# jeuneS2/csolve

Hardware: AMD Instinct MI355X
Metric: constraint propagations/sec + nodes/sec, queens-N, 1/2/4/8 MI355X (higher is better)
Workload: dtype int32

## Files before the change

csolve_amd/_lib.py:

```python
from __future__ import annotations

import ctypes as C
import os
import re

_HERE = os.path.dirname(os.path.abspath(__file__))
LIB_PATH = os.environ.get("CSOLVE_HIP_LIB") or os.path.join(_HERE, "libcsolve_hip.so")
HEADER_PATH = os.path.join(os.path.dirname(_HERE), "include", "csolve_gpu.h")


class CsolveError(RuntimeError):
    def __init__(self, code: int, message: str):
        super().__init__(f"csolve_gpu error {code}: {message}")
        self.code = code


class Val(C.Structure):
    _fields_ = [("lo", C.c_int32), ("hi", C.c_int32)]


class Node(C.Structure):
    _fields_ = [("var", C.c_int32), ("lo", C.c_int32), ("hi", C.c_int32), ("parent", C.c_int32)]


class SearchStats(C.Structure):
    _fields_ = [("nodes", C.c_uint64), ("cuts", C.c_uint64), ("props", C.c_uint64), ("revisions", C.c_uint64),
                ("solutions", C.c_uint64), ("iterations", C.c_uint64), ("restarts", C.c_uint64), ("pool", C.c_int64), ("pool_peak", C.c_int64),
                ("best", C.c_int32), ("done", C.c_int32)]


SHARD_SOLUTION_FN = C.CFUNCTYPE(None, C.c_void_p, C.c_int, C.POINTER(C.c_int32), C.c_int64, C.c_int32)


class ShardOptions(C.Structure):
    _fields_ = [("slice_iterations", C.c_int64), ("poll_iterations", C.c_int64), ("seed_states_per_rank", C.c_int64),
                ("low_water", C.c_int64), ("time_limit", C.c_double), ("on_solution", SHARD_SOLUTION_FN),
                ("user", C.c_void_p)]


class Result(C.Structure):
    _fields_ = [("status", C.c_int32), ("props", C.c_int32), ("revisions", C.c_int32), ("rounds", C.c_int32)]


MANY_DONE, MANY_LIMIT, MANY_BAD_ROOT = 0, 1, 2
MANY_BAD_SLOT = 3


class ManyResult(C.Structure):
    _fields_ = [("status", C.c_int32), ("root_props", C.c_int32), ("nodes", C.c_int64), ("cuts", C.c_int64),
                ("props", C.c_int64), ("solutions", C.c_int64)]


class ManyOptions(C.Structure):
    _fields_ = [("objective", C.c_int32), ("reserved", C.c_int32), ("max_nodes", C.c_int64)]


class ManyUptoOptions(C.Structure):
    _fields_ = [("max_solutions", C.c_int32), ("reserved", C.c_int32), ("max_nodes", C.c_int64)]


MANY_ROTATE_FIRST = 1


class ManyRestartOptions(C.Structure):
    _fields_ = [("max_nodes", C.c_int64), ("restart_base", C.c_int64), ("seed", C.c_uint32), ("flags", C.c_int32)]


MANY_FULL = 4
MANY_SLOT_FRESH = -2


class ManyStream(C.Structure):
    _fields_ = [("d_rows", C.c_void_p), ("d_owner", C.c_void_p), ("d_count", C.c_void_p), ("capacity", C.c_int64)]


def declared_symbols(header: str = HEADER_PATH):
    text = re.sub(r"/\*.*?\*/", "", open(header).read(), flags=re.S)
    return sorted(set(re.findall(r"\b(csgpu_\w+)\s*\(", text)))


PLAN_FAMILIES = ("events", "traced", "rounds", "lds", "bitset", "regs0", "regs1", "regs2", "regs3", "packed",
                 "shave", "shave_trace", "server", "step_shave", "step_packed", "step_import")

_lib = None
_demangler = None


def demangle(symbol: str) -> str:
    global _demangler
    if _demangler is None:
        cxx = C.CDLL("libstdc++.so.6")
        cxx.__cxa_demangle.argtypes = [C.c_char_p, C.c_void_p, C.c_void_p, C.POINTER(C.c_int)]
        cxx.__cxa_demangle.restype = C.c_void_p
        libc = C.CDLL(None)
        libc.free.argtypes = [C.c_void_p]
        _demangler = (cxx.__cxa_demangle, libc.free)
    fn, free = _demangler
    status = C.c_int()
    p = fn(symbol.encode(), None, None, C.byref(status))
    if status.value != 0 or not p:
        raise ValueError(f"cannot demangle {symbol!r}")
    try:
        text = C.string_at(p).decode()
    finally:
        free(p)
    if text.startswith("void "):
        text = text[5:]
    depth = 0
    for i, ch in enumerate(text):
        depth += ch == "<"
        depth -= ch == ">"
        if ch == "(" and depth == 0:
            return text[:i]
    return text


def load_library():
    global _lib
    if _lib is not None:
        return _lib
    if not os.path.exists(LIB_PATH):
        raise ImportError(
            f"{LIB_PATH} is missing: build it with `python -c 'import __graft_entry__ as g; g.build()'` "
            "or `make -C csolve_amd/csrc` (hipcc --offload-arch=gfx950). There is no CPU fallback.")
    try:
        import torch
    except ImportError:
        pass
    L = C.CDLL(LIB_PATH)
    vp, i32, i64 = C.c_void_p, C.c_int32, C.c_int64
    L.csgpu_last_error.restype = C.c_char_p
    L.csgpu_device_count.restype = C.c_int
    L.csgpu_set_device.argtypes = [C.c_int]
    L.csgpu_model_from_text.argtypes = [C.c_char_p, C.c_int, C.POINTER(vp)]
    L.csgpu_model_from_file.argtypes = [C.c_char_p, C.c_int, C.POINTER(vp)]
    L.csgpu_model_from_dump.argtypes = [C.c_char_p, C.POINTER(vp)]
    L.csgpu_model_free.argtypes = [vp]
    L.csgpu_model_free.restype = None
    for f in ("csgpu_model_num_vars", "csgpu_model_num_clauses", "csgpu_model_objective",
              "csgpu_model_objective_var"):
        getattr(L, f).argtypes = [vp]
    L.csgpu_model_var_name.argtypes = [vp, C.c_int]
    L.csgpu_model_var_name.restype = C.c_char_p
    L.csgpu_model_get_domains.argtypes = [vp, vp]
    L.csgpu_model_set_domains.argtypes = [vp, vp]
    L.csgpu_model_device_info.argtypes = [vp, C.POINTER(i64)]
    L.csgpu_model_root_propagate.argtypes = [vp, C.POINTER(i32)]
    L.csgpu_model_finalize.argtypes = [vp]
    L.csgpu_model_normalize.argtypes = [vp]
    L.csgpu_model_specialize.argtypes = [vp, vp, C.POINTER(vp)]
    L.csgpu_model_build_tables.argtypes = [vp]
    L.csgpu_model_eval_clauses_host.argtypes = [vp, vp]
    L.csgpu_model_set_kernel.argtypes = [vp, C.c_int]
    L.csgpu_model_qualifies.argtypes = [vp, C.c_int]
    L.csgpu_set_linear_fast_paths.argtypes = [C.c_int]
    L.csgpu_sets_pack.argtypes = [vp, vp, vp, i64, vp]
    L.csgpu_sets_unpack.argtypes = [vp, vp, vp, i64, vp]
    L.csgpu_propagate_batch_sets.argtypes = [vp, vp, vp, vp, vp, i64, vp]
    L.csgpu_set_linear_fast_paths.restype = None
    L.csgpu_model_get_kernel.argtypes = [vp]
    L.csgpu_propagate_batch.argtypes = [vp, vp, vp, vp, vp, i64, vp]
    L.csgpu_propagate_batch_obj.argtypes = [vp, vp, vp, vp, vp, i64, i32, i32, vp]
    L.csgpu_internal_propagate_objdev.argtypes = [vp, vp, vp, vp, vp, i64, vp, i32, i32, vp, C.c_int, vp]
    L.csgpu_model_forbidden_words.argtypes = [vp]
    L.csgpu_propagate_batch_fb.argtypes = [vp, vp, vp, vp, vp, vp, vp, i64, vp]
    L.csgpu_eval_batch.argtypes = [vp, vp, vp, i64, vp]
    L.csgpu_eval_clauses.argtypes = [vp, vp, vp, vp]
    L.csgpu_search_create.argtypes = [vp, i64, i64, C.POINTER(vp)]
    L.csgpu_search_free.argtypes = [vp]
    L.csgpu_search_free.restype = None
    L.csgpu_search_reset.argtypes = [vp]
    L.csgpu_search_put.argtypes = [vp, vp, i64]
    L.csgpu_search_put_host.argtypes = [vp, vp, i64]
    L.csgpu_search_take.argtypes = [vp, vp, i64, C.POINTER(i64)]
    L.csgpu_search_take_host.argtypes = [vp, vp, i64, C.POINTER(i64)]
    L.csgpu_plan_transfers.argtypes = [vp, C.c_int, i64, i64, vp, C.POINTER(C.c_int)]
    L.csgpu_shard_region_size.argtypes = [C.c_int, C.c_int, i64, C.POINTER(C.c_size_t)]
    L.csgpu_shard_region_init.argtypes = [vp, C.c_size_t, C.c_int, C.c_int, i64]
    L.csgpu_shard_barrier.argtypes = [vp]
    L.csgpu_text_num_vars.argtypes = [C.c_char_p, C.c_int, C.POINTER(C.c_int)]
    L.csgpu_shard_default_options.argtypes = [C.POINTER(ShardOptions)]
    L.csgpu_shard_default_options.restype = None
    L.csgpu_shard_run.argtypes = [vp, vp, C.c_int, vp, C.POINTER(ShardOptions), C.POINTER(SearchStats),
                                  C.POINTER(SearchStats)]
    L.csgpu_search_set_best.argtypes = [vp, i32]
    L.csgpu_model_add_conflict.argtypes = [vp, i32, vp, vp]
    L.csgpu_search_put_cost.argtypes = [vp, C.POINTER(C.c_double), C.POINTER(i64)]
    L.csgpu_objective_better.argtypes = [C.c_int, Val, i32]
    L.csgpu_objective_bound.argtypes = [C.c_int, Val, i32]
    L.csgpu_objective_bound.restype = Val
    L.csgpu_objective_best.argtypes = [C.c_int, Val, i32]
    L.csgpu_objective_best.restype = i32
    L.csgpu_luby_next.argtypes = [C.POINTER(C.c_uint64), C.POINTER(C.c_uint64)]
    L.csgpu_luby_next.restype = None
    L.csgpu_step_check.argtypes = [Val, C.c_uint32]
    L.csgpu_step_val.argtypes = [Val, C.c_uint32, C.c_uint32]
    L.csgpu_step_val.restype = i32
    L.csgpu_search_share_incumbent.argtypes = [vp, vp]
    L.csgpu_search_set_parents.argtypes = [vp, i64]
    L.csgpu_search_set_restart.argtypes = [vp, i64]
    L.csgpu_search_run.argtypes = [vp, i64, C.POINTER(SearchStats)]
    L.csgpu_search_solutions.argtypes = [vp, vp, i64]
    L.csgpu_search_best_solution.argtypes = [vp, vp]
    L.csgpu_search_solutions.restype = i64
    L.csgpu_search_set_solution_stream.argtypes = [vp, i64]
    L.csgpu_search_drain_solutions.argtypes = [vp, vp, i64, C.POINTER(i64)]
    L.csgpu_search_drain_solutions_device.argtypes = [vp, vp, i64, C.POINTER(i64), vp]
    L.csgpu_search_pending_solutions.argtypes = [vp, C.POINTER(i64), C.POINTER(i64)]
    L.csgpu_propagate_one.argtypes = [vp, vp, Node, vp, C.POINTER(Result)]
    L.csgpu_propagate_one_traced.argtypes = [vp, vp, Node, vp, C.POINTER(Result), vp, i32, C.POINTER(i32)]
    L.csgpu_propagate_one_causes.argtypes = [vp, vp, Node, vp, C.POINTER(Result), vp, i32, C.POINTER(i32)]
    L.csgpu_propagate_values.argtypes = [vp, vp, i32, vp, i32, vp, vp]
    L.csgpu_model_root_propagate_limit.argtypes = [vp, i64, C.POINTER(i32), C.POINTER(i32)]
    L.csgpu_propagate_one_chain.argtypes = [vp, vp, Node, C.POINTER(i32), C.POINTER(i32), vp, i32, C.POINTER(i32)]
    L.csgpu_search_set_strategy.argtypes = [vp, C.c_int, C.c_int]
    L.csgpu_search_set_restart_on_improvement.argtypes = [vp, C.c_int]
    L.csgpu_internal_plan_symbol.argtypes = [vp, C.c_int, C.c_char_p, C.c_size_t]
    L.csgpu_solve_many.argtypes = [vp, vp, i64, C.POINTER(ManyOptions), vp, vp, vp]
    L.csgpu_internal_many_symbol.argtypes = [vp, C.c_char_p, C.c_size_t]
    L.csgpu_internal_many_waves.argtypes = [vp, i64]
    L.csgpu_internal_many_waves.restype = i64
    L.csgpu_internal_many_resume_symbol.argtypes = [vp, C.c_char_p, C.c_size_t]
    L.csgpu_many_checkpoint_bytes.argtypes = [vp]
    L.csgpu_many_checkpoint_bytes.restype = C.c_size_t
    L.csgpu_many_checkpoints_create.argtypes = [vp, i64, C.POINTER(vp)]
    L.csgpu_many_checkpoints_reset.argtypes = [vp, vp]
    L.csgpu_many_checkpoints_free.argtypes = [vp]
    L.csgpu_many_checkpoints_free.restype = None
    L.csgpu_solve_many_checkpointed.argtypes = [vp, vp, i64, C.POINTER(ManyOptions), vp, vp, vp, vp, vp]
    L.csgpu_solve_many_resume.argtypes = [vp, i64, C.POINTER(ManyOptions), vp, vp, vp, vp, vp]
    L.csgpu_many_checkpoint_states.argtypes = [vp, C.c_int32, vp, i64, C.POINTER(i64), vp]
    L.csgpu_many_checkpoint_children.argtypes = [vp, vp, i64, vp, vp]
    L.csgpu_many_checkpoint_fanout.argtypes = [vp, vp, i64, vp, vp, vp, i64, vp]
    L.csgpu_many_fold.argtypes = [vp, vp, i64, vp, vp]
    L.csgpu_solve_many_upto.argtypes = [vp, vp, i64, C.POINTER(ManyUptoOptions), vp, vp, vp]
    L.csgpu_solve_many_upto_checkpointed.argtypes = [vp, vp, i64, C.POINTER(ManyUptoOptions), vp, vp, vp, vp, vp]
    L.csgpu_solve_many_upto_resume.argtypes = [vp, i64, C.POINTER(ManyUptoOptions), vp, vp, vp, vp, vp]
    L.csgpu_internal_many_upto_symbol.argtypes = [vp, C.c_char_p, C.c_size_t]
    L.csgpu_model_qualifies_many_allowed.argtypes = [vp]
    L.csgpu_solve_many_allowed.argtypes = [vp, vp, i64, C.POINTER(ManyOptions), vp, vp, vp]
    L.csgpu_solve_many_allowed_upto.argtypes = [vp, vp, i64, C.POINTER(ManyUptoOptions), vp, vp, vp]
    L.csgpu_internal_many_allowed_symbol.argtypes = [vp, C.c_char_p, C.c_size_t]
    L.csgpu_internal_many_allowed_upto_symbol.argtypes = [vp, C.c_char_p, C.c_size_t]
    L.csgpu_solve_many_restarts.argtypes = [vp, vp, vp, i64, C.POINTER(ManyRestartOptions), vp, vp, vp, vp]
    L.csgpu_internal_many_restart_symbol.argtypes = [vp, C.c_char_p, C.c_size_t]
    L.csgpu_solve_many_stream.argtypes = [vp, vp, i64, C.POINTER(ManyOptions), vp, vp, vp, C.POINTER(ManyStream), vp]
    L.csgpu_internal_many_stream_symbol.argtypes = [vp, C.c_char_p, C.c_size_t]
    L.csgpu_solve_many_clauses.argtypes = [vp, vp, i64, C.POINTER(ManyOptions), vp, vp, vp, vp]
    L.csgpu_model_qualifies_many_clauses.argtypes = [vp]
    L.csgpu_internal_many_clauses_symbol.argtypes = [vp, C.c_char_p, C.c_size_t]
    L.csgpu_internal_many_clauses_waves.argtypes = [vp, i64]
    L.csgpu_internal_many_clauses_waves.restype = i64
    L.csgpu_internal_many_clauses_resume_symbol.argtypes = [vp, C.c_char_p, C.c_size_t]
    L.csgpu_many_clause_checkpoint_bytes.argtypes = [vp]
    L.csgpu_many_clause_checkpoint_bytes.restype = C.c_size_t
    L.csgpu_many_clause_checkpoints_create.argtypes = [vp, i64, C.POINTER(vp)]
    L.csgpu_solve_many_clauses_checkpointed.argtypes = [vp, vp, i64, C.POINTER(ManyOptions), vp, vp, vp, vp, vp, vp]
    L.csgpu_solve_many_clauses_resume.argtypes = [vp, i64, C.POINTER(ManyOptions), vp, vp, vp, vp, vp, vp]
    L.csgpu_many_clause_checkpoint_states.argtypes = [vp, C.c_int32, vp, i64, C.POINTER(i64), C.POINTER(C.c_int32),
                                                      C.POINTER(C.c_int32), vp]
    L.csgpu_many_clause_checkpoint_children.argtypes = [vp, vp, i64, vp, vp]
    L.csgpu_many_clause_checkpoint_fanout.argtypes = [vp, vp, i64, vp, vp, vp, i64, vp]
    L.csgpu_solve_many_clauses_upto.argtypes = [vp, vp, i64, C.POINTER(ManyUptoOptions), vp, vp, vp]
    L.csgpu_solve_many_clauses_upto_checkpointed.argtypes = [vp, vp, i64, C.POINTER(ManyUptoOptions), vp, vp, vp, vp, vp]
    L.csgpu_solve_many_clauses_upto_resume.argtypes = [vp, i64, C.POINTER(ManyUptoOptions), vp, vp, vp, vp, vp]
    L.csgpu_internal_many_clauses_upto_symbol.argtypes = [vp, C.c_char_p, C.c_size_t]
    L.csgpu_solve_many_clauses_restarts.argtypes = [vp, vp, vp, i64, C.POINTER(ManyRestartOptions), vp, vp, vp, vp]
    L.csgpu_internal_many_clauses_restart_symbol.argtypes = [vp, C.c_char_p, C.c_size_t]
    L.csgpu_solve_many_clauses_stream.argtypes = [vp, vp, i64, C.POINTER(ManyOptions), vp, vp, vp, C.POINTER(ManyStream), vp]
    L.csgpu_internal_many_clauses_stream_symbol.argtypes = [vp, C.c_char_p, C.c_size_t]
    L.csgpu_solve_many_clauses_from.argtypes = [vp, vp, vp, i64, C.POINTER(ManyOptions), vp, vp, vp, vp, vp, vp]
    L.csgpu_solve_many_clauses_from_resume.argtypes = [vp, i64, C.POINTER(ManyOptions), vp, vp, vp, vp, vp, vp]
    L.csgpu_many_clause_checkpoint_children_obj.argtypes = [vp, vp, i64, C.c_int, vp, vp]
    L.csgpu_many_clause_checkpoint_fanout_obj.argtypes = [vp, vp, i64, C.c_int, vp, vp, vp, vp, vp, i64, vp]
    L.csgpu_many_fold_best.argtypes = [vp, vp, vp, i64, C.c_int, vp, vp]
    L.csgpu_many_best_key.argtypes = [C.c_int, C.c_int32, C.c_uint32]
    L.csgpu_many_best_key.restype = C.c_uint64
    L.csgpu_many_key_decode.argtypes = [C.c_int, C.c_uint64, C.POINTER(C.c_int32), C.POINTER(C.c_uint32)]
    L.csgpu_internal_many_clauses_from_symbol.argtypes = [vp, C.c_char_p, C.c_size_t]
    L.csgpu_many_value.argtypes = [C.c_uint32, C.c_uint32, C.c_int32, Val, C.c_uint32, C.c_int32]
    L.csgpu_many_value.restype = C.c_int32
    L.csgpu_debug_one_timing.argtypes = [vp, C.POINTER(C.c_double), C.POINTER(C.c_uint64), C.POINTER(C.c_uint64)]
    _lib = L
    return L


def check(rc: int):
    if rc < 0:
        raise CsolveError(rc, load_library().csgpu_last_error().decode())
    return rc
```

csolve_amd/csrc/cs_capi.hip:

```cpp
#include <hip/hip_runtime.h>
#include <chrono>

#include <dlfcn.h>
#include <stdarg.h>
#include <stdio.h>
#include <stdlib.h>
#include <string.h>

#include <mutex>

#include "../../include/csolve_gpu.h"
#include "cs_kernels.hip.h"
#include "cs_shave.hip.h"
#include "cs_step.hip.h"
#include "cs_dive.hip.h"
#include "cs_walk.hip.h"
#include "cs_chain.hip.h"
#include "cs_internal.h"

static thread_local char g_err[512] = "";

static int set_err(int code, const char *fmt, ...) {
  va_list ap;
  va_start(ap, fmt);
// ... 980 lines not shown
  const char *force = getenv("CSGPU_K2_ADJ");
  const int want_global = force != NULL && force[0] == 'g';
  if (want_global && 8 * lds_slice <= CS_CU_LDS) {
    m->lds_adj_global = 1;
    waves = 8;
    bytes = 8 * lds_slice;
  }
  { const char *e = getenv("CSGPU_K2_CSZ"); m->k2_csz = e != NULL && atoi(e) >= 1 && atoi(e) <= CS_CHUNK ? atoi(e) : 0; }
  if (!waves) return CSGPU_OK;
  int rc;
  if ((rc = upload(m->img->adj_packed, (size_t)m->img->n_adj * (size_t)m->img->packed_width, (int **)&m->d_adj_packed)))
    return rc;
  if ((rc = plan_kernel(&m->plan.lds, ne_lds_kernel(m->img->packed_width, h->n_vars, m->lds_adj_global), bytes, waves)))
    return rc;
  if (m->plan.lds.per_cu < 1) m->plan.lds.per_cu = 1;
  return CSGPU_OK;
}

static int64_t widest_root_domain(const csgpu_model *m) {
  const cs_model *h = m->host;
  int64_t width = 1;
  for (int32_t v = 0; v < h->n_vars; v++) {
    const int64_t w = (int64_t)h->dom[v].hi - (int64_t)h->dom[v].lo + 1;
    if (w > width) width = w;
  }
  return width;
}

static int forbidden_sets_shape(const csgpu_model *m, int *fw_out, size_t *lds_out) {
  const cs_model *h = m->host;
  if (m->img->sym_width == 0 || m->not_root) return 0;
  const int64_t width = widest_root_domain(m);
  const int fw = width <= 64 ? 1 : (width <= 128 ? 2 : (width <= 256 ? 4 : 0));
  if (!fw) return 0;
  const size_t n_words = ((size_t)h->n_vars + 31) / 32;
  const size_t off_bytes = (((size_t)h->n_vars * 2 * sizeof(int)) + 15) & ~(size_t)15;
  const size_t base_bytes = (((size_t)h->n_vars * sizeof(int)) + 15) & ~(size_t)15;
  const size_t adj_bytes = (((size_t)m->img->sym_n_adj * (size_t)m->img->sym_width) + 15) & ~(size_t)15;
  const size_t sl = ((size_t)h->n_vars * sizeof(cs_val) + (size_t)h->n_vars * fw * 8 + (2 * n_words + 2) * sizeof(unsigned) + 15) &
                    ~(size_t)15;
  int waves = 16;
  for (; waves >= 1; waves--)
    if (off_bytes + base_bytes + adj_bytes + (size_t)waves * sl <= CS_CU_LDS) break;
  if (waves < 1) return 0;
  *fw_out = fw;
  *lds_out = off_bytes + base_bytes + adj_bytes + (size_t)waves * sl;
  return waves;
}

static int plan_forbidden_sets(csgpu_model *m) {
  const cs_model *h = m->host;
  int fw = 0;
  size_t lds = 0;
  const int waves = forbidden_sets_shape(m, &fw, &lds);
  if (!waves) return CSGPU_OK;
  m->fb_words = fw;
  int *lo = (int *)malloc((size_t)(h->n_vars ? h->n_vars : 1) * sizeof(int));
  for (int32_t v = 0; v < h->n_vars; v++) lo[v] = h->dom[v].lo;
  int rc = upload(lo, (size_t)h->n_vars * sizeof(int), &m->d_root_lo);
  free(lo);
  if (rc) return rc;
  if ((rc = upload(m->img->sym_off, ((size_t)h->n_vars + 1) * sizeof(int), &m->d_sym_off))) return rc;
  if ((rc = upload(m->img->sym_packed, (size_t)m->img->sym_n_adj * (size_t)m->img->sym_width, (int **)&m->d_sym_packed)))
    return rc;
  if ((rc = plan_kernel(&m->plan.bitset, ne_bitset_kernel(m->img->sym_width, fw, h->n_vars), lds, waves))) return rc;
  if (m->plan.bitset.per_cu < 1) m->plan.bitset.per_cu = 1;
  return CSGPU_OK;
}

static int dense_table_waves(const csgpu_model *m, size_t *bytes_out) {
  if (m->img->dense_width == 0) return 0;
  const size_t bytes = (size_t)m->host->n_vars * m->img->dense_slots * m->img->dense_cols * m->img->dense_width;
  int best = 0, waves = 0;
  for (int w = 4; w <= 16; w <<= 1)
    if (resident_per_cu(bytes, w) * w > best) { best = resident_per_cu(bytes, w) * w; waves = w; }
  *bytes_out = bytes;
  return waves;
}

static int plan_dense_table(csgpu_model *m) {
  const cs_model *h = m->host;
  if (!m->fb_words) return CSGPU_OK;
  const int n = h->n_vars, width = m->img->dense_width, slots = m->img->dense_slots;
  size_t bytes = 0;
  const int waves = dense_table_waves(m, &bytes);
  if (!waves) return CSGPU_OK;
  m->dense_bytes = bytes;
  int rc;
  if ((rc = upload(m->img->dense_tab, bytes, (int **)&m->d_dense_tab))) return rc;
  for (int variant = 0; variant < 4; variant++)
    if ((rc = plan_kernel(&m->plan.regs[variant], ne_regs_kernel(width, m->fb_words, n, variant & 1, variant >> 1), bytes, waves)))
      return rc;
  m->plan.full = n == cs_dense_strides(n) * CS_WAVE;
  if ((rc = plan_kernel(&m->plan.shave, ne_shave_kernel(width, n, slots, m->plan.full), bytes, waves))) return rc;
  const size_t table = (bytes + 15) & ~(size_t)15;
  if (table + (size_t)waves * 32 <= CS_CU_LDS &&
      (rc = plan_kernel(&m->plan.step_shave, step_shave_kernel(width, n, slots, m->plan.full), table + (size_t)waves * 32, waves)))
    return rc;
  if (table + CS_SHAVE_TRACE_LDS * 16 <= CS_CU_LDS) {
    if ((rc = plan_kernel(&m->plan.shave_trace, ne_shave_trace_kernel(width, n, slots), table + CS_SHAVE_TRACE_LDS * 16, waves)))
      return rc;
    m->plan.server = m->plan.shave_trace;
    m->plan.server.fn = shave_server_kernel(width, n, slots);
  }
  const int64_t widest = widest_root_domain(m);
  for (int family = 0; family < MANY_FAMILIES; family++) {
    const int by_allowed = family == MANY_ALLOWED || family == MANY_ALLOWED_UPTO;
    if (by_allowed && widest > CS_DIVE_ALLOWED_WIDTH) continue;
    if ((rc = plan_kernel(&m->plan.dive[family], dive_kernel(family, width, n, widest <= 32 ? 1 : 4), table, waves))) return rc;
  }
  {
    int *hi = (int *)malloc((size_t)n * sizeof(int));
    if (hi == NULL) return set_err(CSGPU_E_ARG, "out of memory");
    for (int32_t v = 0; v < n; v++) hi[v] = h->dom[v].hi;
    rc = upload(hi, (size_t)n * sizeof(int), &m->d_root_hi);
    free(hi);
    if (rc) return rc;
  }
  HIP_TRY(hipMalloc((void **)&m->d_tickets, (size_t)CS_TICKET_SLOTS * CS_TICKET_SLOT_WORDS * sizeof(unsigned)));
  HIP_TRY(hipMemset(m->d_tickets, 0, (size_t)CS_TICKET_SLOTS * CS_TICKET_SLOT_WORDS * sizeof(unsigned)));
  m->ticket_slots = CS_TICKET_SLOTS;
  m->shave_static = getenv("CSGPU_SHAVE_STATIC") != NULL;
  return CSGPU_OK;
}

static int plan_packed(csgpu_model *m) {
  const cs_model *h = m->host;
  if (m->plan.shave.fn == NULL) return CSGPU_OK;
  const int n = h->n_vars, s3 = m->img->dense_slots == 3;
  m->packed_nw = 1;
  for (int32_t v = 0; v < n; v++)
    if ((int64_t)h->dom[v].hi - (int64_t)h->dom[v].lo + 1 > 32) m->packed_nw = 2;
  m->packed_bias = 0;
  for (int32_t v = 0; v < n; v++)
    if (h->dom[v].lo - m->img->dense_dmin > m->packed_bias) m->packed_bias = h->dom[v].lo - m->img->dense_dmin;
  m->plan.packed_nodes = packed_nodes_per_wave(m->fb_words, n, m->img->dense_width);
  if (!m->plan.packed_nodes) return CSGPU_OK;
  const size_t bytes = m->dense_bytes;
  int rc;
  if ((rc = plan_kernel(&m->plan.packed, ne_packed_kernel(n, m->packed_nw, s3), 2 * bytes, m->plan.regs[0].waves))) return rc;
  m->plan.packed.per_cu = m->plan.regs[0].per_cu;
  const size_t per_row = (size_t)m->img->dense_slots * m->img->dense_cols, total = (size_t)n * per_row;
  uint16_t *rel = (uint16_t *)malloc(total * sizeof(uint16_t));
  const uint8_t *src = (const uint8_t *)m->img->dense_tab;
  for (size_t i = 0; i < total; i++) {
    const int32_t u = (int32_t)(i / per_row);
    rel[i] = src[i] == 0xffu ? (uint16_t)0xffffu : (uint16_t)((int)src[i] - (h->dom[u].lo - m->img->dense_dmin) + m->packed_bias);
  }
  rc = upload(rel, total * sizeof(uint16_t), (int **)&m->d_packed_tab);
  free(rel);
  if (rc) return rc;
  if (step_packed_lds(m, 16) <= 80u * 1024u &&
      ((rc = plan_kernel(&m->plan.step_packed, step_packed_kernel(n, m->packed_nw, s3), step_packed_lds(m, 16), 16)) ||
       (rc = plan_kernel(&m->plan.step_import, step_import_kernel(n, m->packed_nw, s3), (2 * bytes + 15) & ~(size_t)15, 4))))
    return rc;
  m->step_chunk_max = 128;
  { const char *e = getenv("CSGPU_STEP_CHUNK_MAX"); if (e != NULL && atoi(e) > 0) m->step_chunk_max = atoi(e); }
  return CSGPU_OK;
}

static int stage_single_node(csgpu_model *m) {
  int dev = 0;
  hipDeviceProp_t prop;
  HIP_TRY(hipGetDevice(&dev));
  HIP_TRY(hipGetDeviceProperties(&prop, dev));
  m->n_cus = prop.multiProcessorCount;
  const size_t nbytes = (size_t)(m->host->n_vars ? m->host->n_vars : 1) * sizeof(cs_val);
  const size_t part = (nbytes + 63) & ~(size_t)63;
  unsigned char *d = NULL;
  HIP_TRY(hipHostMalloc((void **)&m->h_one, 2 * part + 128, hipHostMallocMapped));
  HIP_TRY(hipHostGetDevicePointer((void **)&d, m->h_one, 0));
  m->d_one_in = (cs_val *)d;
  m->d_one_node = (cs_node_in *)(d + part);
  m->d_one_res = (cs_node_out *)(d + part + 64);
  m->d_one_out = (cs_val *)(d + part + 128);
  return CSGPU_OK;
}

extern "C" int csgpu_model_finalize(csgpu_model *m) {
  if (m == NULL) return set_err(CSGPU_E_ARG, "null argument");
  free_device(m);
  int rc;
  if ((rc = csgpu_model_build_tables(m)) || (rc = drop_entailed_clauses(m)) || (rc = plan_general(m)) ||
      (rc = plan_lds_resident(m)) || (rc = plan_forbidden_sets(m)) || (rc = plan_dense_table(m)) || (rc = plan_packed(m)) ||
      (rc = stage_single_node(m)))
    return rc;
  m->plan.step_kind = m->plan.step_packed.fn != NULL ? 1
                      : (m->plan.step_shave.fn != NULL && m->host->n_vars <= 256 && m->plan.max_width <= 256 ? 2 : 0);
  m->finalized = 1;
  return CSGPU_OK;
}

static int kernel_qualifies(const csgpu_model *m, int which) {
  if (!m->finalized) return 0;
  switch (which) {
  case 1: return 1;
  case 2: return m->plan.lds.fn != NULL;
  case 3: return m->plan.bitset.fn != NULL;
  case 4: return m->plan.regs[0].fn != NULL;
  case 5: return m->plan.packed.fn != NULL;
  case 6: return m->plan.rounds.fn != NULL;
  case 7: return m->plan.shave.fn != NULL;
  default: return 0;
  }
}

extern "C" int csgpu_model_set_kernel(csgpu_model *m, int which) {
  static const char *const kernel_name[8] = {
    NULL, NULL, "the LDS-resident kernel", "the forbidden-set kernel", "the register-resident forbidden-set kernel",
    "the several-nodes-per-wave kernel (at most 32 variables, 64 values)", "the clause-resident kernel (at most 512 clauses)",
    "the interval-only shaving kernel (dense pair table in LDS)" };
  if (m == NULL || which < 0 || which > 7) return set_err(CSGPU_E_ARG, "bad argument");
  if (which >= 2) {
    if (!m->finalized) return set_err(CSGPU_E_STATE, "model is not finalized");
    if (!kernel_qualifies(m, which)) return set_err(CSGPU_E_LIMIT, "model does not qualify for %s", kernel_name[which]);
  }
  m->kernel_choice = which;
  return CSGPU_OK;
}

extern "C" int csgpu_model_qualifies(const csgpu_model *m, int which) { return m != NULL && kernel_qualifies(m, which); }

extern "C" int csgpu_internal_plan_symbol(const csgpu_model *m, int family, char *buf, size_t len) {
  if (m == NULL || buf == NULL || len == 0) return set_err(CSGPU_E_ARG, "null argument");
  if (!m->finalized) return set_err(CSGPU_E_STATE, "model is not finalized");
  const cs_kernel_plan *p = &m->plan;
  const cs_planned *fam[] = { &p->events, &p->traced, &p->rounds, &p->lds, &p->bitset, &p->regs[0], &p->regs[1],
                              &p->regs[2], &p->regs[3], &p->packed, &p->shave, &p->shave_trace, &p->server,
                              &p->step_shave, &p->step_packed, &p->step_import };
  if (family < 0 || family >= (int)(sizeof fam / sizeof fam[0])) return set_err(CSGPU_E_ARG, "no plan family %d", family);
  buf[0] = '\0';
  const void *fn = fam[family]->fn;
  if (fn == NULL) return CSGPU_OK;
  Dl_info info;
  if (dladdr(fn, &info) == 0 || info.dli_sname == NULL || info.dli_saddr != fn)
    return set_err(CSGPU_E_STATE, "plan family %d: the kernel handle has no dynamic symbol", family);
  if (strlen(info.dli_sname) >= len) return set_err(CSGPU_E_LIMIT, "plan family %d: symbol longer than the buffer", family);
  strcpy(buf, info.dli_sname);
  return CSGPU_OK;
}

static int many_symbol(const csgpu_model *m, int family, char *buf, size_t len) {
  if (m == NULL || buf == NULL || len == 0) return set_err(CSGPU_E_ARG, "null argument");
  if (!m->finalized) return set_err(CSGPU_E_STATE, "model is not finalized");
  buf[0] = '\0';
  const void *fn = m->plan.dive[family].fn;
  const char *name = many_kernel_name[family];
  if (fn == NULL) return CSGPU_OK;
  Dl_info info;
  if (dladdr(fn, &info) == 0 || info.dli_sname == NULL || info.dli_saddr != fn)
    return set_err(CSGPU_E_STATE, "%s: the kernel handle has no dynamic symbol", name);
  if (strlen(info.dli_sname) >= len) return set_err(CSGPU_E_LIMIT, "%s: symbol longer than the buffer", name);
  strcpy(buf, info.dli_sname);
  return CSGPU_OK;
}

extern "C" int csgpu_internal_many_symbol(const csgpu_model *m, char *buf, size_t len) { return many_symbol(m, MANY_PLAIN, buf, len); }
extern "C" int csgpu_internal_many_resume_symbol(const csgpu_model *m, char *buf, size_t len) { return many_symbol(m, MANY_CK, buf, len); }
extern "C" int csgpu_internal_many_upto_symbol(const csgpu_model *m, char *buf, size_t len) { return many_symbol(m, MANY_UPTO, buf, len); }
extern "C" int csgpu_internal_many_restart_symbol(const csgpu_model *m, char *buf, size_t len) { return many_symbol(m, MANY_RESTART, buf, len); }
extern "C" int csgpu_internal_many_stream_symbol(const csgpu_model *m, char *buf, size_t len) { return many_symbol(m, MANY_STREAM, buf, len); }
extern "C" int csgpu_internal_many_allowed_symbol(const csgpu_model *m, char *buf, size_t len) { return many_symbol(m, MANY_ALLOWED, buf, len); }
extern "C" int csgpu_internal_many_allowed_upto_symbol(const csgpu_model *m, char *buf, size_t len) { return many_symbol(m, MANY_ALLOWED_UPTO, buf, len); }

extern "C" void csgpu_internal_engine_ref(const csgpu_model *m, int delta) {
  if (m != NULL) const_cast<csgpu_model *>(m)->engines += delta;
}

extern "C" const int32_t *csgpu_internal_root_lo(const csgpu_model *m) {
  return m != NULL && m->finalized && m->fb_words ? m->d_root_lo : NULL;
}

extern "C" int csgpu_model_forbidden_words(const csgpu_model *m) { return m && m->finalized ? m->fb_words : 0; }

extern "C" int csgpu_internal_step_kind(const csgpu_model *m) { return m == NULL || !m->finalized ? 0 : m->plan.step_kind; }

static int64_t step_shave_waves(const csgpu_model *m, int64_t stage_rows) {
  const cs_planned *k = &m->plan.step_shave;
  int64_t waves = (int64_t)m->n_cus * (int64_t)k->per_cu * k->waves;
  const int64_t by_stage = stage_rows / (4 * (int64_t)m->plan.max_width);
  if (waves > by_stage) waves = by_stage / k->waves * k->waves;
  return waves;
}

extern "C" int64_t csgpu_internal_step_parents_limit(const csgpu_model *m, int64_t stage_rows) {
  const int kind = csgpu_internal_step_kind(m);
  if (kind == 1) return 0x3fffffff;
  if (kind != 2) return 0;
  const int maxw = m->plan.max_width;
  const int64_t waves = step_shave_waves(m, stage_rows);
  if (waves < 1) return 0;
  return (stage_rows - waves * 2 * maxw) / maxw;
}

extern "C" int64_t csgpu_internal_step_stage_rows(const csgpu_model *m) {
  if (csgpu_internal_step_kind(m) != 2) return 0;
  return (int64_t)m->n_cus * 32 * 4 * m->plan.max_width;
}

extern "C" int64_t csgpu_internal_step_waves(const csgpu_model *m) { return m == NULL ? 0 : (int64_t)m->n_cus * 32; }

static int launch_step_shave(const csgpu_model *m, const csgpu_step_launch *L, void *stream) {
  const cs_planned *k = &m->plan.step_shave;
  const int n = m->host->n_vars, maxw = m->plan.max_width;
  int64_t waves = step_shave_waves(m, L->stage_rows);
  if (waves < k->waves || (int64_t)L->parents > csgpu_internal_step_parents_limit(m, L->stage_rows))
    return set_err(CSGPU_E_LIMIT, "step kernel: staging buffer too small for the frontier");
  const int64_t by_parents = ((int64_t)L->parents + k->waves - 1) / k->waves * k->waves;
  if (waves > by_parents) waves = by_parents;
  const int64_t grid = waves / k->waves;
  const int64_t K = L->stage_rows / waves;
  cs_step_io io;
  io.pool = (const uint2 *)L->pool;
  io.first_row = (long long)L->first_row;
  io.parents = L->parents;
  io.chunk = 1;
  io.maxw = maxw;
  io.stage = (uint2 *)L->stage;
  io.K = (int)(K > 0x7fffffff ? 0x7fffffff : K);
  io.fill = L->fill;
  io.wstat = (unsigned long long *)L->wstat;
  io.ticket = L->ticket;
  io.solutions = L->solutions;
  io.stored = (unsigned long long *)L->stored;
  io.max_solutions = (long long)L->max_solutions;
  io.store_open = L->store_open;
  io.stream_on = L->stream != NULL;
  int nn = n, slots = m->img->dense_slots, dmin_d = m->img->dense_dmin;
  const void *tab_d = m->d_dense_tab;
  const int *root_lo_d = m->d_root_lo, *sym_off = m->d_sym_off;
  size_t tab_bytes = m->dense_bytes;
  void *args[] = { &nn, &tab_d, &slots, &dmin_d, &root_lo_d, &sym_off, &tab_bytes, &io };
  HIP_TRY(hipLaunchKernel(k->fn, dim3((unsigned)grid), dim3((unsigned)(k->waves * CS_WAVE)), args, k->lds, (hipStream_t)stream));
  hipLaunchKernelGGL(cs_collect, dim3((unsigned)waves), dim3(256), 0, (hipStream_t)stream, (const unsigned *)L->fill, (int)waves,
                     (const uint2 *)L->stage, io.K, n, (uint2 *)L->pool, (long long)L->first_row, (int)L->parents,
                     0 , (const unsigned *)L->ticket, (const unsigned long long *)L->wstat,
                     (unsigned long long *)L->out, (const unsigned long long *)L->stored,
                     L->stream, (long long)L->stream_base, (long long)L->stream_limit, (long long)L->stream_cap,
                     (unsigned long long *)L->stream_err);
  HIP_TRY(hipGetLastError());
  return CSGPU_OK;
}

extern "C" int csgpu_internal_step(const csgpu_model *m, const csgpu_step_launch *L, void *stream) {
  const int kind = csgpu_internal_step_kind(m);
  if (kind == 0 || L == NULL || L->parents < 1) return set_err(CSGPU_E_ARG, "bad argument");
  if (kind == 2) return launch_step_shave(m, L, stream);
  const int n = m->host->n_vars;
  const int G = m->plan.packed_nodes, maxw = m->plan.max_width;
  if (G * maxw > CS_STEP_QN) return set_err(CSGPU_E_LIMIT, "step kernel: interval too wide for the child queue");
  int64_t waves = (int64_t)m->n_cus * 32;
  const int64_t by_stage = L->stage_rows / (2 * (int64_t)G * maxw);
  if (waves > by_stage) waves = by_stage;
  const int64_t by_parents = ((int64_t)L->parents + G - 1) / G;
  if (waves > by_parents) waves = by_parents;
  if (waves < 1) return set_err(CSGPU_E_LIMIT, "step kernel: staging buffer too small");
  int wg_waves = 16;
  while (wg_waves > waves) wg_waves >>= 1;
  const int64_t grid = waves / wg_waves;
  waves = grid * wg_waves;
  const int64_t K = L->stage_rows / waves;
  int64_t chunk = (int64_t)L->parents / (waves * 8);
  if (chunk > m->step_chunk_max) chunk = m->step_chunk_max;
  if (chunk * maxw > K / 2) chunk = K / (2 * maxw);
  chunk = chunk / G * G;
  if (chunk < G) chunk = G;
  cs_step_io io;
  io.pool = (const uint2 *)L->pool;
  io.first_row = (long long)L->first_row;
  io.parents = L->parents;
  io.chunk = (int)chunk;
  io.maxw = maxw;
  io.stage = (uint2 *)L->stage;
  io.K = (int)(K > 0x7fffffff ? 0x7fffffff : K);
  io.fill = L->fill;
  io.wstat = (unsigned long long *)L->wstat;
  io.ticket = L->ticket;
  io.solutions = L->solutions;
  io.stored = (unsigned long long *)L->stored;
  io.max_solutions = (long long)L->max_solutions;
  io.store_open = L->store_open;
  io.stream_on = L->stream != NULL;
  int nn = n, slots = m->img->dense_slots, bias = m->packed_bias;
  const void *tab_d = m->d_packed_tab;
  const int *root_lo_d = m->d_root_lo, *sym_off = m->d_sym_off;
  size_t tab_bytes = 2 * m->dense_bytes;
  void *args[] = { &nn, &tab_d, &slots, &root_lo_d, &sym_off, &bias, &tab_bytes, &io };
  HIP_TRY(hipLaunchKernel(m->plan.step_packed.fn, dim3((unsigned)grid), dim3((unsigned)(wg_waves * CS_WAVE)), args,
                          step_packed_lds(m, wg_waves), (hipStream_t)stream));
  hipLaunchKernelGGL(cs_collect, dim3((unsigned)waves), dim3(256), 0, (hipStream_t)stream, (const unsigned *)L->fill, (int)waves,
                     (const uint2 *)L->stage, io.K, n, (uint2 *)L->pool, (long long)L->first_row, (int)L->parents,
                     (int)chunk, (const unsigned *)L->ticket, (const unsigned long long *)L->wstat,
                     (unsigned long long *)L->out, (const unsigned long long *)L->stored,
                     L->stream, (long long)L->stream_base, (long long)L->stream_limit, (long long)L->stream_cap,
                     (unsigned long long *)L->stream_err);
  HIP_TRY(hipGetLastError());
  return CSGPU_OK;
}

extern "C" int csgpu_internal_step_import(const csgpu_model *m, csgpu_val *d_rows, int64_t first_row, int64_t count,
                                          void *stream) {
  const int kind = csgpu_internal_step_kind(m);
  if (kind == 2) return CSGPU_OK;
  if (kind != 1 || d_rows == NULL || count < 0) return set_err(CSGPU_E_ARG, "bad argument");
  if (count == 0) return CSGPU_OK;
  const cs_planned *k = &m->plan.step_import;
  const int n = m->host->n_vars, G = m->plan.packed_nodes;
  int nn = n, slots = m->img->dense_slots, bias = m->packed_bias;
  const void *tab_d = m->d_packed_tab;
  const int *root_lo_d = m->d_root_lo;
  size_t tab_bytes = 2 * m->dense_bytes;
  long long fr = first_row, cnt = count;
  int64_t grid = (count + (int64_t)G * k->waves - 1) / ((int64_t)G * k->waves);
  if (grid > (int64_t)m->n_cus * 8) grid = (int64_t)m->n_cus * 8;
  void *args[] = { &nn, &tab_d, &slots, &root_lo_d, &bias, &tab_bytes, &d_rows, &fr, &cnt };
  HIP_TRY(hipLaunchKernel(k->fn, dim3((unsigned)grid), dim3((unsigned)(k->waves * CS_WAVE)), args, k->lds, (hipStream_t)stream));
  return CSGPU_OK;
}

extern "C" int csgpu_internal_step_export(const csgpu_model *m, csgpu_val *d_rows, int64_t first_row, int64_t count,
                                          void *stream) {
  const int kind = csgpu_internal_step_kind(m);
  if (kind == 2) return CSGPU_OK;
  if (kind != 1 || d_rows == NULL || count < 0) return set_err(CSGPU_E_ARG, "bad argument");
  if (count == 0) return CSGPU_OK;
  const int n = m->host->n_vars;
  const long long elements = (long long)count * n;
  uint2 *rows = (uint2 *)d_rows + (size_t)first_row * n;
  const unsigned grid = (unsigned)((elements + 255) / 256);
  if (m->packed_nw == 1)
    hipLaunchKernelGGL(cs_step_export<1>, dim3(grid), dim3(256), 0, (hipStream_t)stream, n, (const int *)m->d_root_lo, rows, elements);
  else
    hipLaunchKernelGGL(cs_step_export<2>, dim3(grid), dim3(256), 0, (hipStream_t)stream, n, (const int *)m->d_root_lo, rows, elements);
  HIP_TRY(hipGetLastError());
  return CSGPU_OK;
}

static int launch_regs(const csgpu_model *m, const csgpu_val *d_states_in, const uint64_t *d_forb_in,
                       const csgpu_node *d_nodes, csgpu_val *d_states_out, uint64_t *d_forb_out, csgpu_result *d_results,
                       int64_t batch, const uint64_t *d_batch, int sets_only, int flags, void *stream) {
  int csz = shrink_chunk(CS_CHUNK, batch, (int64_t)m->n_cus * 32);
  int n = m->host->n_vars, slots = m->img->dense_slots, dmin_d = m->img->dense_dmin;
  const void *tab_d = m->d_dense_tab;
  const int *root_lo_d = m->d_root_lo, *sym_off = m->d_sym_off;
  long long nb_d = (long long)batch;
  void *args_d[] = { &n, &tab_d, &slots, &dmin_d, &root_lo_d, &sym_off, &d_states_in, &d_forb_in, &d_nodes,
                     &d_states_out, &d_forb_out, &d_results, &nb_d, &d_batch, &csz, &flags };
  if (!sets_only && m->kernel_choice != 4 && kernel_qualifies(m, 5)) {
    const cs_planned *k = &m->plan.packed;
    const int64_t groups = (batch + m->plan.packed_nodes - 1) / m->plan.packed_nodes;
    int64_t gp = (int64_t)m->n_cus * (int64_t)k->per_cu * 2;
    const int64_t need_gp = (groups + k->waves - 1) / k->waves;
    if (gp > need_gp) gp = need_gp;
    csz = m->packed_bias;
    tab_d = m->d_packed_tab;
    HIP_TRY(hipLaunchKernel(k->fn, dim3((unsigned)gp), dim3((unsigned)(k->waves * CS_WAVE)), args_d, k->lds, (hipStream_t)stream));
    return CSGPU_OK;
  }
  const int fast = m->plan.full && d_forb_in != NULL && d_forb_out != NULL && flags == 0;
  const cs_planned *k = &m->plan.regs[fast | sets_only << 1];
  const int64_t chunks = (batch + csz - 1) / csz;
  int64_t g = (int64_t)m->n_cus * (int64_t)k->per_cu;
  const int64_t need_wg = (chunks + k->waves - 1) / k->waves;
  g *= 2;
  if (g > need_wg) g = need_wg;
  HIP_TRY(hipLaunchKernel(k->fn, dim3((unsigned)g), dim3((unsigned)(k->waves * CS_WAVE)), args_d, k->lds, (hipStream_t)stream));
  return CSGPU_OK;
}

static std::mutex g_ticket_mutex;

static unsigned *ticket_slot(csgpu_model *m, void *stream) {
  if (m->d_tickets == NULL) return NULL;
  std::lock_guard<std::mutex> lock(g_ticket_mutex);
  hipStreamCaptureStatus cap = hipStreamCaptureStatusNone;
  if (stream != NULL && hipStreamIsCapturing((hipStream_t)stream, &cap) != hipSuccess) cap = hipStreamCaptureStatusNone;
  int slot = -1;
  if (cap == hipStreamCaptureStatusActive) {
    if (m->ticket_reserved < m->ticket_slots - CS_TICKET_STREAMS) slot = m->ticket_slots - 1 - m->ticket_reserved++;
  } else {
    for (int i = 0; i < m->ticket_streams; i++)
      if (m->ticket_stream[i] == stream) slot = i;
    if (slot < 0 && m->ticket_streams < CS_TICKET_STREAMS) {
      slot = m->ticket_streams++;
      m->ticket_stream[slot] = stream;
    }
  }
  return slot < 0 ? NULL : m->d_tickets + (size_t)slot * CS_TICKET_SLOT_WORDS;
}

static int launch_shave(const csgpu_model *m, const csgpu_val *d_states_in, const csgpu_node *d_nodes,
                        csgpu_val *d_states_out, csgpu_result *d_results, int64_t batch, const uint64_t *d_batch,
                        void *stream) {
  const cs_planned *k = &m->plan.shave;
  int csz = shrink_chunk(m->host->n_vars <= CS_WAVE ? 2 * CS_SHAVE_CHUNK : CS_SHAVE_CHUNK, batch, 4 * (int64_t)m->n_cus * 32);
  const int64_t chunks = (batch + csz - 1) / csz;
  int64_t g = (int64_t)m->n_cus * (int64_t)k->per_cu;
  const int64_t need_wg = (chunks + k->waves - 1) / k->waves;
  if (g > need_wg) g = need_wg;
  int n = m->host->n_vars, slots = m->img->dense_slots, dmin_d = m->img->dense_dmin;
  const void *tab_d = m->d_dense_tab;
  const int *root_lo_d = m->d_root_lo, *sym_off = m->d_sym_off;
  long long nb_d = (long long)batch;
  unsigned *tickets = m->shave_static ? NULL : ticket_slot((csgpu_model *)m, stream);
  int4 *no_trace = NULL;
  unsigned *no_trace_n = NULL;
  unsigned no_trace_cap = 0u;
  void *args[] = { &n, &tab_d, &slots, &dmin_d, &root_lo_d, &sym_off, &d_states_in, &d_nodes, &d_states_out, &d_results,
                   &nb_d, &d_batch, &csz, &tickets, &no_trace, &no_trace_n, &no_trace_cap };
  HIP_TRY(hipLaunchKernel(k->fn, dim3((unsigned)g), dim3((unsigned)(k->waves * CS_WAVE)), args, k->lds, (hipStream_t)stream));
  return CSGPU_OK;
}


static_assert(sizeof(csgpu_many_result) == sizeof(cs_dive_result) && sizeof(csgpu_many_result) == 40, "csgpu_many_result layout");
static_assert(sizeof(csgpu_many_restart_options) == 24, "csgpu_many_restart_options layout");

#define MANY_NOT_QUALIFIED "model does not qualify for the interval-only shaving kernel"

struct csgpu_many_checkpoints {
  const csgpu_model *m;
  int64_t capacity;
  size_t slot_bytes;
  cs_val *d_pool;
  unsigned long long *d_next;
  int counted;
  int kind;
  int *d_zero;
};
enum { MANY_POOL_DIVE, MANY_POOL_WALK };
#define MANY_POOL_KIND "the checkpoint pool is of the other kind: csgpu_many_checkpoints_create makes the pools of csgpu_solve_many, " \
                       "csgpu_many_clause_checkpoints_create those of csgpu_solve_many_clauses"

extern "C" int64_t csgpu_internal_many_waves(const csgpu_model *m, int64_t count) {
  if (m == NULL || !m->finalized || m->plan.dive[MANY_PLAIN].fn == NULL || count < 1) return 0;
  const cs_planned *k = &m->plan.dive[MANY_PLAIN];
  int64_t grid = (int64_t)m->n_cus * k->per_cu;
  const int64_t by_count = (count + k->waves - 1) / k->waves;
  if (grid > by_count) grid = by_count;
  return grid * k->waves;
}

static int many_workspace(csgpu_model *mm, int64_t waves, int frames) {
  const int n = mm->host->n_vars;
  const size_t bytes = (size_t)waves * (size_t)frames * ((size_t)n + 1) * sizeof(cs_val);
  if (mm->d_many_tickets == NULL) {
    quiesce_servers();
    HIP_TRY(hipMalloc((void **)&mm->d_many_tickets, (size_t)CS_DIVE_SHARDS * CS_DIVE_TICKET_STRIDE * sizeof(unsigned)));
    HIP_TRY(hipMemset(mm->d_many_tickets, 0, (size_t)CS_DIVE_SHARDS * CS_DIVE_TICKET_STRIDE * sizeof(unsigned)));
  }
  if (mm->many_stack_bytes < bytes) {
    quiesce_servers();
    if (mm->d_many_stack != NULL) (void)hipFree(mm->d_many_stack);
    mm->d_many_stack = NULL;
    mm->many_stack_bytes = 0;
    HIP_TRY(hipMalloc(&mm->d_many_stack, bytes));
    mm->many_stack_bytes = bytes;
  }
  return CSGPU_OK;
}

static int many_check_head(int null_arg, int64_t count, int64_t max_nodes, const char *budgeted) {
  if (null_arg) return set_err(CSGPU_E_ARG, "null argument");
  if (count < 0) return set_err(CSGPU_E_ARG, "negative instance count");
  if (max_nodes <= 0) return set_err(CSGPU_E_ARG, "max_nodes must be positive: every %s has a budget", budgeted);
  return CSGPU_OK;
}

static int many_check_objective(int objective) {
  if (objective == CS_OBJ_MIN || objective == CS_OBJ_MAX)
    return set_err(CSGPU_E_LIMIT, "csgpu_solve_many searches with ANY or ALL: MIN / MAX are not supported");
  if (objective != CS_OBJ_ANY && objective != CS_OBJ_ALL) return set_err(CSGPU_E_ARG, "no objective %d", objective);
  return CSGPU_OK;
}

static int many_check_tail(const csgpu_model *m, int family, const csgpu_many_checkpoints *ck, int64_t count) {
  if (!m->finalized) return set_err(CSGPU_E_STATE, "model is not finalized");
  if (m->plan.dive[family].fn == NULL)
    return set_err(CSGPU_E_LIMIT, MANY_NOT_QUALIFIED " (a pure != network of at most 256 variables whose dense pair table "
                                                     "fits LDS), which csgpu_solve_many is built on");
  if (ck != NULL && ck->m != m) return set_err(CSGPU_E_ARG, "the checkpoint pool was created for another model");
  if (ck != NULL && ck->kind != MANY_POOL_DIVE) return set_err(CSGPU_E_ARG, MANY_POOL_KIND);
  if (count > 0x7fffffff - CS_DIVE_SHARDS) return set_err(CSGPU_E_LIMIT, "more than 2^31 - 65 instances in one call");
  return CSGPU_OK;
}

static int many_launch(const csgpu_model *m, int family, const csgpu_val *d_roots, int64_t count, int64_t max_nodes, int all,
                       csgpu_many_result *d_results, int32_t *d_solutions, int resume, void *stream, void *tail0, void *tail1) {
  if (count == 0) return CSGPU_OK;
  csgpu_model *mm = const_cast<csgpu_model *>(m);
  const cs_planned *k = &m->plan.dive[family];
  const int n = m->host->n_vars;
  const int64_t waves = csgpu_internal_many_waves(m, count);
  const int frames = n;
  int rc;
  if ((rc = many_workspace(mm, resume ? 0 : waves, frames))) return rc;
  cs_dive_io io;
  io.roots = (const cs_val *)d_roots;
  io.count = (int)count;
  io.all = all;
  io.max_nodes = (long long)max_nodes;
  io.results = (cs_dive_result *)d_results;
  io.solutions = d_solutions;
  io.stack = resume ? NULL : (cs_val *)mm->d_many_stack;
  io.frames = frames;
  io.tickets = mm->d_many_tickets;
  int nn = n, slots = m->img->dense_slots, dmin_d = m->img->dense_dmin;
  const void *tab_d = m->d_dense_tab;
  const int *root_lo_d = m->d_root_lo, *root_hi_d = m->d_root_hi, *sym_off = m->d_sym_off;
  size_t tab_bytes = m->dense_bytes;
  void *args[] = { &nn, &tab_d, &slots, &dmin_d, &root_lo_d, &root_hi_d, &sym_off, &tab_bytes, &io, tail0, tail1 };
  HIP_TRY(hipLaunchKernel(k->fn, dim3((unsigned)(waves / k->waves)), dim3((unsigned)(k->waves * CS_WAVE)), args, k->lds, (hipStream_t)stream));
  return CSGPU_OK;
}

static cs_dive_ck many_ck_arg(const csgpu_many_checkpoints *ck, int32_t *d_slots, int resume) {
  cs_dive_ck dk;
  dk.pool = ck != NULL ? ck->d_pool : NULL;
  dk.next = ck != NULL ? ck->d_next : NULL;
  dk.capacity = ck != NULL ? (int)ck->capacity : 0;
  dk.resume = resume;
  dk.slots = ck != NULL ? d_slots : NULL;
  return dk;
}

extern "C" int csgpu_solve_many(const csgpu_model *m, const csgpu_val *d_roots, int64_t count, const csgpu_many_options *options,
                                csgpu_many_result *d_results, int32_t *d_solutions, void *stream) {
  const int null_arg = m == NULL || d_roots == NULL || d_results == NULL || options == NULL;
  int rc;
  if ((rc = many_check_head(null_arg, count, null_arg ? 0 : options->max_nodes, "instance")) ||
      (rc = many_check_objective(options->objective)) || (rc = many_check_tail(m, MANY_PLAIN, NULL, count)))
    return rc;
  return many_launch(m, MANY_PLAIN, d_roots, count, options->max_nodes, options->objective == CS_OBJ_ALL, d_results, d_solutions,
                     0, stream, NULL, NULL);
}


static int many_qualifies(const csgpu_model *m) {
  if (m->finalized) return m->plan.dive[MANY_PLAIN].fn != NULL;
  if (m->img == NULL) return 0;
  int fw = 0;
  size_t bytes = 0;
  return forbidden_sets_shape(m, &fw, &bytes) > 0 && dense_table_waves(m, &bytes) > 0 && ((bytes + 15) & ~(size_t)15) <= CS_CU_LDS;
}

extern "C" size_t csgpu_many_checkpoint_bytes(const csgpu_model *m) {
  if (m == NULL || !many_qualifies(m)) return 0;
  const size_t n = (size_t)m->host->n_vars;
  return (n + 1) * (n + 1) * sizeof(cs_val);
}

static int many_pool_create(const csgpu_model *m, int64_t capacity, int kind, int qualifies, const char *limit, size_t slot_bytes,
                            csgpu_many_checkpoints **out) {
  if (m == NULL || out == NULL) return set_err(CSGPU_E_ARG, "null argument");
  if (capacity < 1) return set_err(CSGPU_E_ARG, "a checkpoint pool has at least one slot");
  if (!m->finalized) return set_err(CSGPU_E_STATE, "model is not finalized");
  if (!qualifies) return set_err(CSGPU_E_LIMIT, "%s", limit);
  if (capacity > 0x7fffffff) return set_err(CSGPU_E_LIMIT, "more than 2^31 - 1 slots");
  csgpu_many_checkpoints *ck = (csgpu_many_checkpoints *)calloc(1, sizeof *ck);
  if (ck == NULL) return set_err(CSGPU_E_LIMIT, "out of memory");
  ck->m = m;
  ck->capacity = capacity;
  ck->slot_bytes = slot_bytes;
  ck->kind = kind;
  const size_t zero_bytes = (size_t)m->host->n_vars * sizeof(int);
  hipError_t e;
  if ((e = hipMalloc((void **)&ck->d_pool, (size_t)capacity * ck->slot_bytes)) != hipSuccess ||
      (e = hipMalloc((void **)&ck->d_next, sizeof *ck->d_next)) != hipSuccess ||
      (e = hipMemset(ck->d_pool, 0, (size_t)capacity * ck->slot_bytes)) != hipSuccess ||
      (e = hipMemset(ck->d_next, 0, sizeof *ck->d_next)) != hipSuccess ||
      (kind == MANY_POOL_WALK && ((e = hipMalloc((void **)&ck->d_zero, zero_bytes)) != hipSuccess ||
                                  (e = hipMemset(ck->d_zero, 0, zero_bytes)) != hipSuccess))) {
    csgpu_many_checkpoints_free(ck);
    return set_err(CSGPU_E_HIP, "checkpoint pool of %lld slots: %s", (long long)capacity, hipGetErrorString(e));
  }
  csgpu_internal_engine_ref(m, 1);
  ck->counted = 1;
  *out = ck;
  return CSGPU_OK;
}

extern "C" int csgpu_many_checkpoints_create(const csgpu_model *m, int64_t capacity, csgpu_many_checkpoints **out) {
  return many_pool_create(m, capacity, MANY_POOL_DIVE, m != NULL && m->finalized && m->plan.dive[MANY_CK].fn != NULL,
                          MANY_NOT_QUALIFIED ", which csgpu_solve_many is built on", csgpu_many_checkpoint_bytes(m), out);
}

extern "C" int csgpu_many_checkpoints_reset(csgpu_many_checkpoints *ck, void *stream) {
  if (ck == NULL) return set_err(CSGPU_E_ARG, "null argument");
  HIP_TRY(hipMemsetAsync(ck->d_next, 0, sizeof *ck->d_next, (hipStream_t)stream));
  return CSGPU_OK;
}

extern "C" void csgpu_many_checkpoints_free(csgpu_many_checkpoints *ck) {
  if (ck == NULL) return;
  if (ck->counted) csgpu_internal_engine_ref(ck->m, -1);
  (void)hipFree(ck->d_pool);
  (void)hipFree(ck->d_next);
  (void)hipFree(ck->d_zero);
  free(ck);
// ... 1245 lines not shown
```

csolve_amd/csrc/cs_internal.h:

```cpp
#ifndef CS_INTERNAL_H
#define CS_INTERNAL_H

#include "../../include/csolve_gpu.h"
#include "cs_model.h"

#ifdef __cplusplus
extern "C" {
#endif

int csgpu_model_from_host(cs_model *host, int lists_final, int domains_are_root, csgpu_model **out);
cs_model *csgpu_model_host(csgpu_model *m);

int csgpu_internal_propagate_fb(const csgpu_model *m, const csgpu_val *d_states_in, const uint64_t *d_forb_in,
                                const csgpu_node *d_nodes, csgpu_val *d_states_out, uint64_t *d_forb_out,
                                csgpu_result *d_results, int64_t batch, const uint64_t *d_batch, void *stream);
int csgpu_internal_propagate_obj(const csgpu_model *m, const csgpu_val *d_states_in, const csgpu_node *d_nodes,
                                 csgpu_val *d_states_out, csgpu_result *d_results, int64_t batch,
                                 const uint64_t *d_batch, int32_t obj_lo, int32_t obj_hi, void *stream);

int csgpu_internal_propagate_objdev(const csgpu_model *m, const csgpu_val *d_states_in, const csgpu_node *d_nodes,
                                    csgpu_val *d_states_out, csgpu_result *d_results, int64_t batch,
                                    const uint64_t *d_batch, int32_t obj_lo, int32_t obj_hi, const int32_t *d_best,
                                    int sense, void *stream);
const int32_t *csgpu_internal_root_lo(const csgpu_model *m);
void csgpu_internal_engine_ref(const csgpu_model *m, int delta);
int csgpu_internal_eval_list(const csgpu_model *m, const csgpu_val *d_states, const int32_t *d_list,
                             const uint64_t *d_count, int64_t bound, int32_t *d_truth, void *stream);

int csgpu_internal_set_error(int code, const char *msg);
int csgpu_internal_search_info(const csgpu_search *s, int *objective, int *obj_var, int *n_vars, int *restarts,
                               int64_t *stream_rows);

int csgpu_internal_server_warm(csgpu_model *m);

int csgpu_internal_plan_symbol(const csgpu_model *m, int family, char *buf, size_t len);
int csgpu_internal_many_symbol(const csgpu_model *m, char *buf, size_t len);
int csgpu_internal_many_resume_symbol(const csgpu_model *m, char *buf, size_t len);
int csgpu_internal_many_upto_symbol(const csgpu_model *m, char *buf, size_t len);
int csgpu_internal_many_restart_symbol(const csgpu_model *m, char *buf, size_t len);
int csgpu_internal_many_stream_symbol(const csgpu_model *m, char *buf, size_t len);
int csgpu_internal_many_allowed_symbol(const csgpu_model *m, char *buf, size_t len);
int csgpu_internal_many_allowed_upto_symbol(const csgpu_model *m, char *buf, size_t len);
int64_t csgpu_internal_many_waves(const csgpu_model *m, int64_t count);
int csgpu_internal_many_clauses_symbol(const csgpu_model *m, char *buf, size_t len);
int64_t csgpu_internal_many_clauses_waves(const csgpu_model *m, int64_t count);
int csgpu_internal_many_clauses_resume_symbol(const csgpu_model *m, char *buf, size_t len);
int csgpu_internal_many_clauses_upto_symbol(const csgpu_model *m, char *buf, size_t len);
int csgpu_internal_many_clauses_restart_symbol(const csgpu_model *m, char *buf, size_t len);
int csgpu_internal_many_clauses_stream_symbol(const csgpu_model *m, char *buf, size_t len);
int csgpu_internal_many_clauses_from_symbol(const csgpu_model *m, char *buf, size_t len);

typedef struct csgpu_step_launch {
  const csgpu_val *pool;
  int64_t first_row;
  int32_t parents;
  csgpu_val *stage;
  int64_t stage_rows;
  uint32_t *fill;
  uint64_t *wstat;
  uint32_t *ticket;
  uint64_t *out;
  int32_t *solutions;
  uint64_t *stored;
  int64_t max_solutions;
  int32_t store_open;
  int32_t *stream;
  int64_t stream_base;
  int64_t stream_limit;
  int64_t stream_cap;
  uint64_t *stream_err;
} csgpu_step_launch;
int csgpu_internal_step_kind(const csgpu_model *m);
int64_t csgpu_internal_step_parents_limit(const csgpu_model *m, int64_t stage_rows);
int64_t csgpu_internal_step_stage_rows(const csgpu_model *m);
int64_t csgpu_internal_step_waves(const csgpu_model *m);
int csgpu_internal_step(const csgpu_model *m, const csgpu_step_launch *L, void *stream);
int csgpu_internal_step_import(const csgpu_model *m, csgpu_val *d_rows, int64_t first_row, int64_t count, void *stream);
int csgpu_internal_step_export(const csgpu_model *m, csgpu_val *d_rows, int64_t first_row, int64_t count, void *stream);

#ifdef __cplusplus
}
#endif
#endif
```

csolve_amd/csrc/cs_search.hip:

```cpp
#include <hip/hip_runtime.h>
#include <chrono>
#include <type_traits>

#include <stdint.h>
#include <stdio.h>
#include <stdlib.h>
#include <string.h>

#include "../../include/csolve_gpu.h"
#include "cs_arith.h"
#include "cs_frontend.h"
#include "cs_internal.h"

#include "cs_search_kernels.hip.h"

struct cs_search_switches {
  int burst_off;
  int graph_off;
  int burst_split;
  int eval_always;
  int holes_off;
  int sets_off;
  int fused_off;
  int trace;
  int64_t parents_max;
  int64_t backlog_div;
  int64_t stage_mult;
};

static int env_is(const char *name, char c) {
  const char *e = getenv(name);
  return e != NULL && e[0] == c;
}
static int64_t env_count(const char *name, int64_t otherwise) {
  const char *e = getenv(name);
  return e != NULL && atoll(e) >= 1 ? atoll(e) : otherwise;
}

static cs_search_switches read_switches(void) {
  cs_search_switches w;
  w.burst_off = env_is("CSGPU_SEARCH_BURST", '0');
  w.graph_off = env_is("CSGPU_SEARCH_GRAPH", '0');
  w.burst_split = !env_is("CSGPU_SEARCH_BURST_SPLIT", '0');
  w.eval_always = env_is("CSGPU_SEARCH_EVAL", '1');
  w.holes_off = env_is("CSGPU_SEARCH_HOLES", '0');
  w.sets_off = env_is("CSGPU_SEARCH_SETS", '0');
  w.fused_off = env_is("CSGPU_SEARCH_FUSED", '0');
  w.trace = getenv("CSGPU_SEARCH_TRACE") != NULL;
  w.parents_max = env_count("CSGPU_SEARCH_PARENTS_MAX", 8192);
  w.backlog_div = env_count("CSGPU_SEARCH_BACKLOG_DIV", 4);
  w.stage_mult = env_count("CSGPU_STEP_STAGE_MULT", 2);
  return w;
}

enum cs_path {
  PATH_LEVELS,
  PATH_HOST,
  PATH_BURST_ONE,
  PATH_BURST_SPLIT,
};

struct csgpu_search {
  const csgpu_model *m;
  int n, objective, obj_var;
  int64_t cap, max_children, max_parents, max_width, parents_limit;
  int64_t parents_max;
  double avg_children;
  cs_val *pool;
  int64_t top, peak;
  int fw;
  unsigned long long *pool_forb, *d_child_forb;
  csgpu_node *d_rebuild_nodes;
  cs_choice *d_choice;
  int *d_child_off , *d_block_sum, *d_block_skip;
  csgpu_node *d_nodes;
  cs_val *d_child_states, *d_complete_states;
  csgpu_result *d_results;
  int *d_dest , *d_complete_list, *d_truth;
  int *d_block_surv, *d_block_comp, *d_block_cuts, *d_block_props, *d_block_revs, *d_surv_off, *d_comp_off;
  unsigned long long *d_counters;
  int *d_best;
  int64_t pending_complete;
  int32_t *d_solutions;
  int32_t *d_best_solution;
  int have_best_solution;
  int32_t best_solution_value;
  csgpu_search *lender;
  int borrowers, free_pending;
  double put_seconds;
  int64_t put_states;
  int device;
  int64_t max_solutions;
  csgpu_search_stats st;
  cs_val *seed;
  int64_t seed_count, seed_cap, restart_base, since_restart;
  uint64_t luby_threshold, luby_counter;
  unsigned long long *d_burst, *h_burst;
  hipStream_t burst_stream;
  hipGraphExec_t burst_exec;
  int64_t burst_limit;
  cs_holes holes;
  int counted;
  int64_t stage_rows;
  uint32_t *d_fill, *d_ticket;
  uint64_t *d_wstat, *d_step_out, *h_step_out;
  double surv_per_parent;
  uint64_t stored_seen;
  int order, prefer_failing, restart_on_improvement, fail_var_known;
  int *d_prio;
  int burst_no_eval;
  cs_search_switches sw;
  cs_path path;
  int32_t *d_stream;
  int64_t stream_cap, stream_rows, stream_head;
  int stream_failed;
};

extern "C" int csgpu_internal_set_error(int code, const char *msg);
static int fail(int code, const char *msg) { return csgpu_internal_set_error(code, msg); }
static int flush_accept_results(csgpu_search *s);

#define HIP_OK(expr)                                                           \
  do {                                                                         \
    hipError_t e_ = (expr);                                                    \
    if (e_ != hipSuccess) return fail(CSGPU_E_HIP, hipGetErrorString(e_));     \
  } while (0)
#define TRY(expr)                                                              \
  do {                                                                         \
    const int rc_ = (expr);                                                    \
    if (rc_ != CSGPU_OK) return rc_;                                           \
  } while (0)

static cs_path plan_path(const csgpu_search *s) {
  const int default_rule = s->order == 1 && !s->prefer_failing;
  if (s->objective == CS_OBJ_ALL)
    return csgpu_internal_step_kind(s->m) != 0 && !s->sw.fused_off && !s->sw.eval_always && default_rule ? PATH_LEVELS
                                                                                                          : PATH_HOST;
  const int split = s->sw.burst_split && s->objective != CS_OBJ_ANY;
  const int64_t most = split ? BURST_PARENTS_MAX : SMALL_PARENTS;
  if (s->sw.burst_off || s->parents_max > most || s->parents_max * s->max_width > s->max_children) return PATH_HOST;
  return split ? PATH_BURST_SPLIT : PATH_BURST_ONE;
}

static int burst_path(const csgpu_search *s) { return s->path == PATH_BURST_ONE || s->path == PATH_BURST_SPLIT; }

static int objective_sense(int objective) { return objective == CS_OBJ_MIN ? 1 : (objective == CS_OBJ_MAX ? 2 : 0); }

static int64_t pool_reserve(const csgpu_search *s) { return (int64_t)s->n * s->max_width; }
static int64_t pool_room_limit(const csgpu_search *s) { return s->cap > pool_reserve(s) ? s->cap - pool_reserve(s) : s->cap; }

static int scatter_cpb(int n, int64_t children) {
  int cpb = 4096 / n;
  cpb = cpb < 4 ? 4 : (cpb > SB ? SB : cpb);
  while (cpb > 4 && children / cpb < 2048) cpb >>= 1;
  return cpb;
}

template <typename F> static void launch_seg(int n, F launch) {
  if (n <= 16) launch(std::integral_constant<int, 16>());
  else if (n <= 32) launch(std::integral_constant<int, 32>());
  else launch(std::integral_constant<int, 64>());
}

static void drop_burst_graph(csgpu_search *s) {
  if (s->burst_exec != NULL) (void)hipGraphExecDestroy(s->burst_exec);
  s->burst_exec = NULL;
}

extern "C" void csgpu_search_free(csgpu_search *s) {
  if (s == NULL) return;
  if (s->borrowers > 0) {
    s->free_pending = 1;
    return;
  }
  if (s->lender != NULL) {
    csgpu_search *l = s->lender;
    s->lender = NULL;
    if (--l->borrowers == 0 && l->free_pending) csgpu_search_free(l);
  }
  (void)hipSetDevice(s->device);
  if (s->counted) csgpu_internal_engine_ref(s->m, -1);
  (void)hipFree(s->pool_forb); (void)hipFree(s->d_child_forb); (void)hipFree(s->d_rebuild_nodes);
  (void)hipFree(s->pool); (void)hipFree(s->d_choice); (void)hipFree(s->d_child_off); (void)hipFree(s->d_block_sum); (void)hipFree(s->d_block_skip);
  (void)hipFree(s->d_nodes); (void)hipFree(s->d_child_states); (void)hipFree(s->d_complete_states);
  (void)hipFree(s->d_results); (void)hipFree(s->d_dest); (void)hipFree(s->d_complete_list); (void)hipFree(s->d_truth);
  (void)hipFree(s->d_block_surv); (void)hipFree(s->d_block_comp); (void)hipFree(s->d_surv_off); (void)hipFree(s->d_comp_off);
  (void)hipFree(s->d_block_cuts); (void)hipFree(s->d_block_props); (void)hipFree(s->d_block_revs);
  (void)hipFree(s->d_counters); (void)hipFree(s->d_solutions);
  (void)hipFree(s->seed);
  (void)hipFree(s->d_best_solution);
  (void)hipFree(s->d_burst);
  (void)hipFree(s->d_prio);
  (void)hipFree(s->d_stream);
  (void)hipFree(s->d_fill); (void)hipFree(s->d_ticket); (void)hipFree(s->d_wstat); (void)hipFree(s->d_step_out);
  if (s->h_step_out) (void)hipHostFree(s->h_step_out);
  if (s->h_burst) (void)hipHostFree(s->h_burst);
  drop_burst_graph(s);
  if (s->burst_stream) (void)hipStreamDestroy(s->burst_stream);
  free(s);
}

static int search_init(csgpu_search *s) {
  const csgpu_model *m = s->m;
  const int n = s->n;
  const int64_t max_children = s->max_children;
  s->sw = read_switches();
  s->objective = csgpu_model_objective(m);
  s->obj_var = csgpu_model_objective_var(m);
  s->max_parents = max_children / s->max_width;
  s->avg_children = (double)s->max_width;
  s->parents_limit = s->objective == CS_OBJ_ALL ? s->max_parents : 64;
  if (s->parents_limit > s->max_parents) s->parents_limit = s->max_parents;
  s->parents_max = s->parents_limit;
  if (s->objective == CS_OBJ_MIN || s->objective == CS_OBJ_MAX) {
    int64_t want = s->sw.parents_max;
    const int64_t most = s->sw.burst_split ? BURST_PARENTS_MAX : SMALL_PARENTS;
    if (want > most) want = most;
    s->parents_max = want < s->max_parents ? want : s->max_parents;
    if (s->parents_max < s->parents_limit) s->parents_max = s->parents_limit;
  }
  s->max_solutions = 1024;
  s->restart_base = s->objective == CS_OBJ_ANY ? 64 : 0;
  s->order = 1;
  s->holes.order = 1;
  s->holes.prio = NULL;
  s->holes.pool_forb = NULL;
  s->holes.root_lo = csgpu_internal_root_lo(m);
  s->path = plan_path(s);
  const int levels = s->path == PATH_LEVELS;
  const size_t row = (size_t)n * sizeof(cs_val);
#define ALLOC(ptr, bytes) HIP_OK(hipMalloc((void **)&(ptr), (bytes)))
  ALLOC(s->pool, row * (size_t)s->cap);
  s->fw = s->obj_var < 0 && !s->sw.sets_off && !levels ? csgpu_model_forbidden_words(m) : 0;
  s->stage_rows = max_children;
  if (levels) {
    s->stage_rows = max_children * s->sw.stage_mult;
    if (s->stage_rows < csgpu_internal_step_stage_rows(m)) s->stage_rows = csgpu_internal_step_stage_rows(m);
    if (s->stage_rows > s->cap) s->stage_rows = s->cap;
  }
  if (levels) {
    const int64_t waves = csgpu_internal_step_waves(m);
    ALLOC(s->d_fill, sizeof(uint32_t) * (size_t)waves);
    ALLOC(s->d_wstat, sizeof(uint64_t) * 8 * (size_t)waves);
    ALLOC(s->d_ticket, 1024);
    ALLOC(s->d_step_out, sizeof(uint64_t) * 8);
    HIP_OK(hipHostMalloc((void **)&s->h_step_out, sizeof(uint64_t) * 8, 0));
  }
  if (s->fw > 0) {
    ALLOC(s->pool_forb, (size_t)n * s->fw * 8 * (size_t)s->cap);
    ALLOC(s->d_child_forb, (size_t)n * s->fw * 8 * (size_t)max_children);
    ALLOC(s->d_rebuild_nodes, sizeof(csgpu_node) * (size_t)max_children);
  }
  ALLOC(s->d_choice, sizeof(cs_choice) * (size_t)max_children);
  ALLOC(s->d_child_off, sizeof(int) * ((size_t)max_children + 1));
  ALLOC(s->d_block_sum, sizeof(int) * ((size_t)max_children + 1));
  ALLOC(s->d_block_skip, sizeof(int) * ((size_t)max_children + 1));
  ALLOC(s->d_nodes, sizeof(csgpu_node) * (size_t)max_children);
  ALLOC(s->d_child_states, row * (size_t)(levels ? s->stage_rows : max_children));
  if (!levels) ALLOC(s->d_complete_states, row * (size_t)max_children);
  ALLOC(s->d_results, sizeof(csgpu_result) * (size_t)max_children);
  ALLOC(s->d_dest, sizeof(int) * (size_t)max_children);
  ALLOC(s->d_complete_list, sizeof(int) * (size_t)max_children);
  ALLOC(s->d_truth, sizeof(int) * (size_t)max_children);
  {
    size_t blocks = ((size_t)max_children + SB - 1) / SB + 1;
    if (blocks < BURST_CLASS_WGS) blocks = BURST_CLASS_WGS;
    ALLOC(s->d_block_surv, sizeof(int) * blocks);
    ALLOC(s->d_block_comp, sizeof(int) * blocks);
    ALLOC(s->d_block_cuts, sizeof(int) * blocks);
    ALLOC(s->d_block_props, sizeof(int) * blocks);
    ALLOC(s->d_block_revs, sizeof(int) * blocks);
    ALLOC(s->d_surv_off, sizeof(int) * (blocks + 1));
    ALLOC(s->d_comp_off, sizeof(int) * (blocks + 1));
  }
  ALLOC(s->d_counters, sizeof(unsigned long long) * C_COUNT);
  s->d_best = (int *)(s->d_counters + C_BEST);
  ALLOC(s->d_solutions, sizeof(int32_t) * (size_t)n * (size_t)s->max_solutions);
  ALLOC(s->d_best_solution, sizeof(int32_t) * (size_t)n);
  if (s->fw == 1 && s->holes.root_lo != NULL && !s->sw.holes_off) s->holes.pool_forb = s->pool_forb;
  ALLOC(s->d_burst, sizeof(unsigned long long) * B_COUNT);
#undef ALLOC
  HIP_OK(hipHostMalloc((void **)&s->h_burst, sizeof(unsigned long long) * (B_COUNT + C_COUNT + 1), 0));
  HIP_OK(hipStreamCreate(&s->burst_stream));
  int64_t info[8];
  s->burst_no_eval = !s->sw.eval_always && csgpu_model_device_info(m, info) == CSGPU_OK && info[2] == 0;
  return csgpu_search_reset(s);
}

extern "C" int csgpu_search_create(const csgpu_model *m, int64_t pool_capacity, int64_t max_children,
                                   csgpu_search **out) {
  if (m == NULL || out == NULL || pool_capacity < 1 || max_children < 1) return fail(CSGPU_E_ARG, "bad argument");
  const int n = csgpu_model_num_vars(m);
  if (n <= 0) return fail(CSGPU_E_ARG, "model without variables");
  int device = 0;
  if (hipGetDevice(&device) != hipSuccess) return fail(CSGPU_E_HIP, "hipGetDevice");
  csgpu_val *dom = (csgpu_val *)malloc((size_t)n * sizeof *dom);
  if (dom == NULL) return fail(CSGPU_E_LIMIT, "out of memory");
  csgpu_model_get_domains(m, dom);
  int64_t max_width = 2;
  for (int v = 0; v < n; v++) {
    int64_t w = (int64_t)dom[v].hi - (int64_t)dom[v].lo + 1;
    if (w > SPLIT_WIDTH) w = SPLIT_WIDTH;
    if (w > max_width) max_width = w;
  }
  free(dom);
  if (max_children < max_width) max_children = max_width;
  if (max_children > 0x3fffffff) return fail(CSGPU_E_LIMIT, "max_children too large");
  if (pool_capacity < max_children + 1) pool_capacity = max_children + 1;
  if (pool_capacity > 0x7fffffff) return fail(CSGPU_E_LIMIT, "pool_capacity too large");
  csgpu_search *s = (csgpu_search *)calloc(1, sizeof *s);
  if (s == NULL) return fail(CSGPU_E_LIMIT, "out of memory");
  s->m = m;
  s->n = n;
  s->device = device;
  s->max_width = max_width;
  s->max_children = max_children;
  s->cap = pool_capacity;
  csgpu_internal_engine_ref(m, 1);
  s->counted = 1;
  const int rc = search_init(s);
  if (rc != CSGPU_OK) {
    csgpu_search_free(s);
    return rc;
  }
  *out = s;
  return CSGPU_OK;
}

static int search_put(csgpu_search *s, const csgpu_val *d_states, int64_t count);

extern "C" int csgpu_search_put(csgpu_search *s, const csgpu_val *d_states, int64_t count) {
  if (s == NULL || (count > 0 && d_states == NULL) || count < 0) return fail(CSGPU_E_ARG, "bad argument");
  if (hipSetDevice(s->device) != hipSuccess) return fail(CSGPU_E_HIP, "hipSetDevice");
  const auto t0 = std::chrono::steady_clock::now();
  int rc = search_put(s, d_states, count);
  if (rc == CSGPU_OK && count > 0) {
    HIP_OK(hipDeviceSynchronize());
    s->put_seconds += std::chrono::duration<double>(std::chrono::steady_clock::now() - t0).count();
    s->put_states += count;
  }
  return rc;
}

extern "C" int csgpu_search_put_cost(const csgpu_search *s, double *seconds, int64_t *states) {
  if (s == NULL || seconds == NULL || states == NULL) return fail(CSGPU_E_ARG, "bad argument");
  *seconds = s->put_seconds;
  *states = s->put_states;
  return CSGPU_OK;
}

static int search_put(csgpu_search *s, const csgpu_val *d_states, int64_t count) {
  if (s->top + count > s->cap) return fail(CSGPU_E_LIMIT, "state pool is full");
  if (count > 0)
    HIP_OK(hipMemcpy(s->pool + (size_t)s->top * s->n, d_states, (size_t)count * s->n * sizeof(cs_val),
                     hipMemcpyDeviceToDevice));
  if (count > 0 && s->path == PATH_LEVELS)
    TRY(csgpu_internal_step_import(s->m, (csgpu_val *)s->pool, s->top, count, NULL));
  if (count > 0 && s->fw > 0) {
    for (int64_t done = 0; done < count; done += s->max_children) {
      const int64_t k = count - done < s->max_children ? count - done : s->max_children;
      hipLaunchKernelGGL(cs_fill_rebuild, dim3((unsigned)((k + 255) / 256)), dim3(256), 0, 0, s->d_rebuild_nodes,
                         (long long)(s->top + done), (int)k);
      TRY(csgpu_propagate_batch_fb(s->m, (const csgpu_val *)s->pool, NULL, s->d_rebuild_nodes,
                                   (csgpu_val *)s->d_child_states, (uint64_t *)s->d_child_forb, s->d_results, k,
                                   NULL));
      HIP_OK(hipMemcpy(s->pool_forb + (size_t)(s->top + done) * s->n * s->fw, s->d_child_forb,
                       (size_t)k * s->n * s->fw * 8, hipMemcpyDeviceToDevice));
    }
  }
  if (count > 0 && (s->restart_base > 0 || s->restart_on_improvement) && !s->st.iterations) {
    if (s->seed_count + count > s->seed_cap) {
      const int64_t cap = (s->seed_count + count) * 2;
      cs_val *grown = NULL;
      HIP_OK(hipMalloc((void **)&grown, (size_t)cap * s->n * sizeof(cs_val)));
      if (s->seed_count > 0)
        HIP_OK(hipMemcpy(grown, s->seed, (size_t)s->seed_count * s->n * sizeof(cs_val), hipMemcpyDeviceToDevice));
      (void)hipFree(s->seed);
      s->seed = grown;
      s->seed_cap = cap;
    }
    HIP_OK(hipMemcpy(s->seed + (size_t)s->seed_count * s->n, d_states, (size_t)count * s->n * sizeof(cs_val),
                     hipMemcpyDeviceToDevice));
    s->seed_count += count;
  }
  s->top += count;
  if (s->top > s->peak) s->peak = s->top;
  return CSGPU_OK;
}

extern "C" int csgpu_search_reset(csgpu_search *s) {
  if (s == NULL) return fail(CSGPU_E_ARG, "bad argument");
  if (hipSetDevice(s->device) != hipSuccess) return fail(CSGPU_E_HIP, "hipSetDevice");
  s->top = 0;
  s->peak = 0;
  memset(&s->st, 0, sizeof s->st);
  s->st.best = s->objective == CS_OBJ_MIN ? CS_DOM_MAX : (s->objective == CS_OBJ_MAX ? CS_DOM_MIN : 0);
  s->seed_count = 0;
  s->since_restart = 0;
  s->luby_threshold = 1;
  s->luby_counter = 1;
  s->put_seconds = 0.0;
  s->put_states = 0;
  s->have_best_solution = 0;
  s->pending_complete = 0;
  s->surv_per_parent = (double)s->max_width;
  s->stored_seen = 0;
  s->stream_rows = 0;
  s->stream_head = 0;
  s->stream_failed = 0;
  if (s->d_prio != NULL) HIP_OK(hipMemset(s->d_prio, 0, sizeof(int) * (size_t)s->n));
  HIP_OK(hipMemset(s->d_counters, 0, sizeof(unsigned long long) * C_COUNT));
  HIP_OK(hipMemcpy(s->d_best, &s->st.best, sizeof(int), hipMemcpyHostToDevice));
  return CSGPU_OK;
}

extern "C" int csgpu_search_put_host(csgpu_search *s, const csgpu_val *states, int64_t count) {
  if (s == NULL || (count > 0 && states == NULL) || count < 0) return fail(CSGPU_E_ARG, "bad argument");
  if (hipSetDevice(s->device) != hipSuccess) return fail(CSGPU_E_HIP, "hipSetDevice");
  if (count == 0) return CSGPU_OK;
  cs_val *tmp = NULL;
  const size_t bytes = (size_t)count * s->n * sizeof(cs_val);
  HIP_OK(hipMalloc((void **)&tmp, bytes));
  hipError_t e = hipMemcpy(tmp, states, bytes, hipMemcpyHostToDevice);
  int rc = e == hipSuccess ? csgpu_search_put(s, (const csgpu_val *)tmp, count) : fail(CSGPU_E_HIP, hipGetErrorString(e));
  (void)hipFree(tmp);
  return rc;
}

extern "C" int csgpu_search_set_restart(csgpu_search *s, int64_t iterations) {
  if (s == NULL || iterations < 0) return fail(CSGPU_E_ARG, "bad argument");
  s->restart_base = s->objective == CS_OBJ_ANY ? iterations : 0;
  return CSGPU_OK;
}

extern "C" int csgpu_search_set_strategy(csgpu_search *s, int order, int prefer_failing) {
  if (s == NULL || order < 0 || order > 4) return fail(CSGPU_E_ARG, "bad argument");
  if (hipSetDevice(s->device) != hipSuccess) return fail(CSGPU_E_HIP, "hipSetDevice");
  if (s->top != 0 || s->st.iterations != 0) return fail(CSGPU_E_STATE, "the strategy is set before the first state is put");
  const int is_default = order == 1 && !prefer_failing;
  if (!is_default) {
    s->fw = 0;
    s->holes.pool_forb = NULL;
  }
  s->order = order;
  s->prefer_failing = prefer_failing != 0;
  s->path = plan_path(s);
  s->holes.order = order;
  s->holes.prio = NULL;
  if (s->prefer_failing) {
    if (s->d_prio == NULL) HIP_OK(hipMalloc((void **)&s->d_prio, sizeof(int) * (size_t)s->n));
    HIP_OK(hipMemset(s->d_prio, 0, sizeof(int) * (size_t)s->n));
    s->holes.prio = s->d_prio;
    const int k = csgpu_model_get_kernel(s->m);
    s->fail_var_known = k == 1 || k == 6 || k == 7;
  }
  drop_burst_graph(s);
  return CSGPU_OK;
}

extern "C" int csgpu_search_set_restart_on_improvement(csgpu_search *s, int on) {
  if (s == NULL) return fail(CSGPU_E_ARG, "bad argument");
  if (s->top != 0 || s->st.iterations != 0) return fail(CSGPU_E_STATE, "set before the first state is put");
  s->restart_on_improvement = on != 0 && (s->objective == CS_OBJ_MIN || s->objective == CS_OBJ_MAX);
  return CSGPU_OK;
}

extern "C" int csgpu_search_take(csgpu_search *s, csgpu_val *d_states, int64_t max, int64_t *count) {
  if (s == NULL || d_states == NULL || count == NULL || max < 0) return fail(CSGPU_E_ARG, "bad argument");
  if (hipSetDevice(s->device) != hipSuccess) return fail(CSGPU_E_HIP, "hipSetDevice");
  int64_t k = max < s->top ? max : s->top;
  *count = k;
  if (k == 0) return CSGPU_OK;
  HIP_OK(hipMemcpy(d_states, s->pool, (size_t)k * s->n * sizeof(cs_val), hipMemcpyDeviceToDevice));
  if (s->path == PATH_LEVELS) {
    TRY(csgpu_internal_step_export(s->m, d_states, 0, k, NULL));
    HIP_OK(hipDeviceSynchronize());
  }
  const int64_t rest = s->top - k, mv = rest < k ? rest : k;
  if (mv > 0) {
    hipLaunchKernelGGL(cs_move_rows, dim3((unsigned)((mv + 3) / 4)), dim3(SB), 0, 0, (unsigned long long *)s->pool,
                       (long long)(s->top - mv), 0ll, (int)mv, s->n);
    if (s->fw > 0)
      hipLaunchKernelGGL(cs_move_rows, dim3((unsigned)((mv + 3) / 4)), dim3(SB), 0, 0, s->pool_forb,
                         (long long)(s->top - mv), 0ll, (int)mv, s->n * s->fw);
    HIP_OK(hipGetLastError());
    HIP_OK(hipDeviceSynchronize());
  }
  s->top -= k;
  return CSGPU_OK;
}

extern "C" int csgpu_search_take_host(csgpu_search *s, csgpu_val *states, int64_t max, int64_t *count) {
  if (s == NULL || states == NULL || count == NULL || max < 0) return fail(CSGPU_E_ARG, "bad argument");
  if (hipSetDevice(s->device) != hipSuccess) return fail(CSGPU_E_HIP, "hipSetDevice");
  const int64_t k = max < s->top ? max : s->top;
  *count = 0;
  if (k == 0) return CSGPU_OK;
  cs_val *tmp = NULL;
  const size_t bytes = (size_t)k * s->n * sizeof(cs_val);
  HIP_OK(hipMalloc((void **)&tmp, bytes));
  int64_t got = 0;
  int rc = csgpu_search_take(s, (csgpu_val *)tmp, k, &got);
  if (rc == CSGPU_OK) {
    const hipError_t e = hipMemcpy(states, tmp, (size_t)got * s->n * sizeof(cs_val), hipMemcpyDeviceToHost);
    if (e == hipSuccess) *count = got;
    else rc = fail(CSGPU_E_HIP, hipGetErrorString(e));
  }
  (void)hipFree(tmp);
  return rc;
}

extern "C" int csgpu_internal_search_info(const csgpu_search *s, int *objective, int *obj_var, int *n_vars,
                                          int *restarts, int64_t *stream_rows) {
  if (s == NULL) return CSGPU_E_ARG;
  if (objective != NULL) *objective = s->objective;
  if (obj_var != NULL) *obj_var = s->obj_var;
  if (n_vars != NULL) *n_vars = s->n;
  if (restarts != NULL) *restarts = s->restart_base > 0 || s->restart_on_improvement;
  if (stream_rows != NULL) *stream_rows = s->d_stream != NULL ? s->stream_cap : 0;
  return CSGPU_OK;
}

extern "C" int csgpu_search_set_parents(csgpu_search *s, int64_t parents_per_iteration) {
  if (s == NULL || parents_per_iteration < 1) return fail(CSGPU_E_ARG, "bad argument");
  const int64_t limit = parents_per_iteration < s->max_parents ? parents_per_iteration : s->max_parents;
  if ((s->lender != NULL || s->borrowers > 0) && (limit > SMALL_PARENTS || limit * s->max_width > s->max_children))
    return fail(CSGPU_E_STATE, "engines that share an incumbent run device-driven iterations: at most 1,024 parents per iteration");
  s->parents_limit = limit;
  s->parents_max = s->parents_limit;
  s->path = plan_path(s);
  return CSGPU_OK;
}

extern "C" int csgpu_search_set_best(csgpu_search *s, int32_t best) {
  if (s == NULL) return fail(CSGPU_E_ARG, "bad argument");
  if (hipSetDevice(s->device) != hipSuccess) return fail(CSGPU_E_HIP, "hipSetDevice");
  TRY(flush_accept_results(s));
  int better = (s->objective == CS_OBJ_MIN && best < s->st.best) || (s->objective == CS_OBJ_MAX && best > s->st.best);
  if (better) {
    s->st.best = best;
    HIP_OK(hipMemcpy(s->d_best, &best, sizeof(int), hipMemcpyHostToDevice));
  }
  return CSGPU_OK;
}

extern "C" int csgpu_search_set_solution_stream(csgpu_search *s, int64_t rows) {
  if (s == NULL) return fail(CSGPU_E_ARG, "bad argument");
  if (hipSetDevice(s->device) != hipSuccess) return fail(CSGPU_E_HIP, "hipSetDevice");
  if (s->top != 0 || s->st.iterations != 0) return fail(CSGPU_E_STATE, "the solution stream is set before the first state is put");
  if (s->lender != NULL || s->borrowers > 0)
    return fail(CSGPU_E_STATE, "an engine that shares its incumbent has no solution stream");
  if (rows < s->max_width || rows > 0x7fffffff) return fail(CSGPU_E_ARG, "solution stream rows out of range");
  if (s->d_stream != NULL && s->stream_cap != rows) {
    (void)hipFree(s->d_stream);
    s->d_stream = NULL;
  }
  if (s->d_stream == NULL) HIP_OK(hipMalloc((void **)&s->d_stream, (size_t)rows * s->n * sizeof(int32_t)));
  s->stream_cap = rows;
  s->stream_rows = 0;
  s->stream_head = 0;
  s->stream_failed = 0;
  HIP_OK(hipMemset(s->d_counters + C_STREAM, 0, sizeof(unsigned long long) * 3));
  drop_burst_graph(s);
  return CSGPU_OK;
}

static int64_t stream_room(const csgpu_search *s) {
  const int64_t pending = s->objective == CS_OBJ_ALL ? s->pending_complete : (s->pending_complete > 0 ? 1 : 0);
  return s->stream_cap - s->stream_rows - pending;
}

extern "C" int csgpu_search_share_incumbent(csgpu_search *s, csgpu_search *with) {
  if (s == NULL || with == NULL || s->objective != with->objective || s->obj_var != with->obj_var)
    return fail(CSGPU_E_ARG, "bad argument");
  if (hipSetDevice(s->device) != hipSuccess) return fail(CSGPU_E_HIP, "hipSetDevice");
  if (s->d_stream != NULL || with->d_stream != NULL)
    return fail(CSGPU_E_STATE, "an engine with a solution stream does not share its incumbent");
  if (s->objective != CS_OBJ_MIN && s->objective != CS_OBJ_MAX) return CSGPU_OK;
  if (!burst_path(s) || !burst_path(with))
    return fail(CSGPU_E_STATE, "a shared incumbent needs the device-driven iterations");
  TRY(flush_accept_results(s));
  int mine = 0, theirs = 0;
  HIP_OK(hipMemcpy(&mine, s->d_best, sizeof(int), hipMemcpyDeviceToHost));
  HIP_OK(hipMemcpy(&theirs, with->d_best, sizeof(int), hipMemcpyDeviceToHost));
  const int best = s->objective == CS_OBJ_MIN ? (mine < theirs ? mine : theirs) : (mine > theirs ? mine : theirs);
  HIP_OK(hipMemcpy(with->d_best, &best, sizeof(int), hipMemcpyHostToDevice));
  if (s == with || s->lender == with) return CSGPU_OK;
  if (s->borrowers > 0) return fail(CSGPU_E_STATE, "an engine whose incumbent word is shared by others cannot borrow one itself");
  csgpu_search *owner = with->lender != NULL ? with->lender : with;
  if (s->lender != NULL && --s->lender->borrowers == 0 && s->lender->free_pending) csgpu_search_free(s->lender);
  s->lender = owner;
  owner->borrowers++;
  s->d_best = owner->d_best;
  s->st.best = best;
  s->path = plan_path(s);
  drop_burst_graph(s);
  return CSGPU_OK;
}

static int apply_accept_results(csgpu_search *s, unsigned long long solutions_total, int best) {
  if (s->pending_complete == 0) return CSGPU_OK;
  const int improved = (s->objective == CS_OBJ_MIN || s->objective == CS_OBJ_MAX) && solutions_total > s->st.solutions &&
                       best != s->st.best;
  if (s->d_stream != NULL && (s->objective == CS_OBJ_ALL || s->objective == CS_OBJ_ANY))
    s->stream_rows += (int64_t)(solutions_total - s->st.solutions);
  s->st.solutions = solutions_total;
  if (improved) {
    hipLaunchKernelGGL(cs_pick_best, dim3(1), dim3(64), 0, 0, s->d_complete_states, s->d_truth, (int)s->pending_complete,
                       s->n, s->objective, s->obj_var, best, s->d_best_solution, s->d_stream, (long long)s->stream_cap,
                       s->d_counters);
    if (s->d_stream != NULL) s->stream_rows++;
    s->have_best_solution = 1;
    s->best_solution_value = best;
  }
  if (s->objective == CS_OBJ_MIN || s->objective == CS_OBJ_MAX) s->st.best = best;
  s->pending_complete = 0;
  HIP_OK(hipGetLastError());
  return CSGPU_OK;
}

static int flush_accept_results(csgpu_search *s) {
  if (s->pending_complete == 0) return CSGPU_OK;
  unsigned long long tail[C_COUNT - C_SOLUTIONS];
  HIP_OK(hipMemcpy(tail, s->d_counters + C_SOLUTIONS, sizeof tail, hipMemcpyDeviceToHost));
  return apply_accept_results(s, tail[0], (int)(unsigned)tail[C_BEST - C_SOLUTIONS]);
}

static int one_iteration_fused(csgpu_search *s) {
  const int64_t reserve = pool_reserve(s);
  const double spp = s->surv_per_parent < 0.25 ? 0.25 : s->surv_per_parent;
  int64_t parents = s->top;
  const int64_t by_stage = (int64_t)((double)s->stage_rows / (2.0 * spp));
  if (parents > by_stage) parents = by_stage;
  const int64_t room = s->cap - s->top - reserve;
  const int64_t by_pool = room > 0 ? (int64_t)((double)room / (spp * (double)s->n)) : 0;
  if (parents > by_pool) parents = by_pool;
  if (parents > 0x3fffffff) parents = 0x3fffffff;
  if (parents < 1) parents = 1;
  if (s->d_stream != NULL && parents > stream_room(s) / s->max_width) parents = stream_room(s) / s->max_width;
  if (s->top - 1 + s->max_width > s->cap) return fail(CSGPU_E_LIMIT, "state pool is full");
  csgpu_step_launch L;
  L.pool = (const csgpu_val *)s->pool;
  L.first_row = s->top - parents;
  L.parents = (int32_t)parents;
  L.stage = (csgpu_val *)s->d_child_states;
  L.stage_rows = s->stage_rows;
  if (L.stage_rows > s->cap - s->top) L.stage_rows = s->cap - s->top;
  {
    const int64_t limit = csgpu_internal_step_parents_limit(s->m, L.stage_rows);
    if (limit < 1) return fail(CSGPU_E_LIMIT, "state pool is full");
    if (parents > limit) {
      parents = limit;
      L.first_row = s->top - parents;
      L.parents = (int32_t)parents;
    }
  }
  L.fill = s->d_fill;
  L.wstat = s->d_wstat;
  L.ticket = s->d_ticket;
  L.out = s->d_step_out;
  L.solutions = s->d_solutions;
  L.stored = (uint64_t *)(s->d_counters + C_STORED);
  L.max_solutions = s->max_solutions;
  L.store_open = s->stored_seen < (uint64_t)s->max_solutions;
  L.stream = s->d_stream;
  L.stream_base = s->stream_head + s->stream_rows;
  L.stream_limit = s->stream_head + s->stream_cap;
  L.stream_cap = s->stream_cap;
  L.stream_err = (uint64_t *)(s->d_counters + C_STREAM_ERR);
  HIP_OK(hipMemsetAsync(s->d_ticket, 0, 1024, 0));
  TRY(csgpu_internal_step(s->m, &L, NULL));
  HIP_OK(hipMemcpyAsync(s->h_step_out, s->d_step_out, sizeof(uint64_t) * 8, hipMemcpyDeviceToHost, 0));
  HIP_OK(hipStreamSynchronize(0));
  const uint64_t *h = s->h_step_out;
  const int64_t consumed = (int64_t)h[0], survivors = (int64_t)h[1];
  if (consumed < 1) return fail(CSGPU_E_LIMIT, "internal: a frontier of the fused search consumed no parent");
  s->top += survivors - consumed;
  if (s->top > s->peak) s->peak = s->top;
  s->st.iterations++;
  s->st.nodes += h[2];
  s->st.cuts += h[3];
  s->st.props += h[4];
  s->st.revisions += h[5];
  s->st.solutions += h[6];
  if (s->d_stream != NULL) s->stream_rows += (int64_t)h[6];
  s->stored_seen = h[7];
  s->surv_per_parent = 0.5 * s->surv_per_parent + 0.5 * ((double)survivors / (double)consumed);
  if (s->sw.trace)
    fprintf(stderr, "fused: parents %lld consumed %lld survivors %lld top %lld nodes %llu cuts %llu solutions %llu\n",
            (long long)parents, (long long)consumed, (long long)survivors, (long long)s->top, (unsigned long long)h[2],
            (unsigned long long)h[3], (unsigned long long)h[6]);
  return CSGPU_OK;
}

static int one_iteration(csgpu_search *s) {
  if (s->path == PATH_LEVELS) return one_iteration_fused(s);
  const int n = s->n;
  int64_t parents = s->top < s->parents_limit ? s->top : s->parents_limit;
  const int64_t room_limit = pool_room_limit(s);
  const int adaptive = s->objective == CS_OBJ_ALL && s->parents_limit == s->max_parents;
  if (adaptive) {
    int64_t guess = (int64_t)((double)s->max_children / (s->avg_children * 1.25));
    if (guess > s->max_children / 2) guess = s->max_children / 2;
    const double per_parent = s->avg_children > 1.5 ? s->avg_children - 1.0 : 0.5;
    const int64_t room = (int64_t)((double)(room_limit - s->top) / (per_parent * 1.25));
    if (guess > room) guess = room;
    if (guess > parents) parents = guess < s->top ? guess : s->top;
  }
  if (!adaptive || parents <= s->max_parents) {
    if (s->top - parents + parents * s->max_width > room_limit) {
      const int64_t fit = s->max_width > 1 ? (room_limit - s->top) / (s->max_width - 1) : parents;
      parents = s->top < 1 ? 0 : (fit < 1 ? 1 : (fit < parents ? fit : parents));
      if (s->top - parents + parents * s->max_width > s->cap) return fail(CSGPU_E_LIMIT, "state pool is full");
    }
  }
  if (s->d_stream != NULL && s->objective == CS_OBJ_ALL && parents > stream_room(s) / s->max_width)
    parents = stream_room(s) / s->max_width;
  long long first_row = s->top - parents;
  if (parents == 0) return CSGPU_OK;
  const int small = parents <= SMALL_PARENTS && parents <= s->max_parents;
  const int low_last = s->objective == CS_OBJ_MAX ? 0 : 1;
  const unsigned scramble =
      s->objective == CS_OBJ_ANY ? (unsigned)(s->st.iterations * 2654435761ull + 0x9e3779b9u) | 1u : 0u;
  unsigned long long skipped_now = 0;
  int64_t children;
  const uint64_t *d_children;
  if (small) {
    hipLaunchKernelGGL(cs_expand_small, dim3(1), dim3(1024), 0, 0, s->pool, first_row, (int)parents, n, s->d_nodes,
                       s->d_counters, low_last, scramble, s->holes);
    children = parents * s->max_width;
    d_children = (const uint64_t *)(s->d_counters + C_TOTAL_CHILDREN);
  } else {
    unsigned pb;
    for (;;) {
      HIP_OK(hipMemsetAsync(s->d_counters, 0, sizeof(unsigned long long) * C_PER_ITERATION, 0));
      launch_seg(n, [&](auto S) {
        constexpr int ppb = SB / decltype(S)::value;
        pb = (unsigned)((parents + ppb - 1) / ppb);
        hipLaunchKernelGGL(cs_branch<decltype(S)::value>, dim3(pb), dim3(SB), 0, 0, s->pool, first_row, (int)parents, n,
                           s->d_choice, s->d_block_sum, s->holes, s->d_block_skip);
      });
      hipLaunchKernelGGL(cs_scan, dim3(1), dim3(1024), 0, 0, s->d_block_sum, (int)pb, s->d_child_off, s->d_counters,
                         (int)C_TOTAL_CHILDREN, (const int *)s->d_block_skip, (int)C_SKIPPED);
      unsigned long long head[C_COUNT - C_TOTAL_CHILDREN];
      HIP_OK(hipMemcpy(head, s->d_counters + C_TOTAL_CHILDREN, sizeof head, hipMemcpyDeviceToHost));
      children = (int64_t)head[0];
      skipped_now = head[C_SKIPPED - C_TOTAL_CHILDREN];
      TRY(apply_accept_results(s, head[C_SOLUTIONS - C_TOTAL_CHILDREN], (int)(unsigned)head[C_BEST - C_TOTAL_CHILDREN]));
      if (adaptive) s->avg_children = 0.5 * s->avg_children + 0.5 * ((double)children / (double)parents);
      const int fits = children <= s->max_children &&
                       (s->top - parents + children <= room_limit || (parents == 1 && s->top - 1 + children <= s->cap));
      if (fits) break;
      if (parents == 1) return fail(CSGPU_E_LIMIT, "state pool is full");
      parents = parents / 2 > 0 ? parents / 2 : 1;
      first_row = s->top - parents;
    }
    d_children = NULL;
    if (children > s->max_children) return fail(CSGPU_E_LIMIT, "internal: more children than the batch buffers hold");
    launch_seg(n, [&](auto S) {
      hipLaunchKernelGGL(cs_emit<decltype(S)::value>, dim3(pb), dim3(SB), 0, 0, first_row, (int)parents,
                         (const cs_choice *)s->d_choice, (const int *)s->d_child_off, s->d_nodes, low_last, scramble);
    });
  }
  s->top -= parents;
  s->st.iterations++;
  if (children == 0) {
    s->st.nodes += skipped_now;
    s->st.cuts += skipped_now;
    return CSGPU_OK;
  }

  const cs_val lim = cs_objective_bound(objective_sense(s->objective), cs_interval(CS_DOM_MIN, CS_DOM_MAX), s->st.best);
  if (s->fw > 0)
    TRY(csgpu_internal_propagate_fb(s->m, (const csgpu_val *)s->pool, (const uint64_t *)s->pool_forb, s->d_nodes,
                                    (csgpu_val *)s->d_child_states, (uint64_t *)s->d_child_forb, s->d_results, children,
                                    d_children, NULL));
  else
    TRY(csgpu_internal_propagate_obj(s->m, (const csgpu_val *)s->pool, s->d_nodes, (csgpu_val *)s->d_child_states,
                                     s->d_results, children, d_children, lim.lo, lim.hi, NULL));
  const unsigned cb = (unsigned)((children + SB - 1) / SB);
  if (s->prefer_failing)
    hipLaunchKernelGGL(cs_prio_update, dim3(cb), dim3(SB), 0, 0, (const csgpu_result *)s->d_results, (const csgpu_node *)s->d_nodes,
                       (int)children, (const unsigned long long *)d_children, n, s->fail_var_known, s->d_prio);
  if (small) {
    hipLaunchKernelGGL(cs_classify_small, dim3(1), dim3(1024), 0, 0, s->d_results, s->d_dest, s->d_complete_list,
                       s->d_counters, (unsigned long long *)NULL);
  } else {
    hipLaunchKernelGGL(cs_classify_count, dim3(cb), dim3(SB), 0, 0, s->d_results, (int)children, s->d_block_surv,
                       s->d_block_comp, s->d_block_cuts, s->d_block_props, s->d_block_revs);
    hipLaunchKernelGGL(cs_scan_classes, dim3(1), dim3(1024), 0, 0, s->d_block_surv, s->d_block_comp, s->d_block_cuts,
                       s->d_block_props, s->d_block_revs, (int)cb, s->d_surv_off, s->d_comp_off, s->d_counters);
    hipLaunchKernelGGL(cs_classify_assign, dim3(cb), dim3(SB), 0, 0, s->d_results, (int)children, s->d_surv_off,
                       s->d_comp_off, s->d_dest, s->d_complete_list);
  }
  {
    const int cpb = scatter_cpb(n, children);
    hipLaunchKernelGGL(cs_scatter, dim3((unsigned)((children + cpb - 1) / cpb)), dim3(SB), 0, 0, s->d_child_states, s->d_dest,
                       s->d_counters, (long long)s->top, n, s->pool, s->d_child_forb, s->pool_forb, s->fw, cpb,
                       (const unsigned long long *)NULL);
  }
  unsigned long long c[C_COUNT];
  HIP_OK(hipMemcpy(c, s->d_counters, sizeof c, hipMemcpyDeviceToHost));
  if (small) {
    children = (int64_t)c[C_TOTAL_CHILDREN];
    TRY(apply_accept_results(s, c[C_SOLUTIONS], (int)(unsigned)c[C_BEST]));
  }
  s->top += (int64_t)c[C_SURVIVORS];
  if (s->top > s->peak) s->peak = s->top;
  s->st.nodes += (uint64_t)children + c[C_SKIPPED];
  s->st.cuts += c[C_CUTS] + c[C_SKIPPED];
  s->st.props += c[C_PROPS];
  s->st.revisions += c[C_REVS];

  const int64_t complete = (int64_t)c[C_COMPLETE];
  if (complete > 0) {
    if (s->objective == CS_OBJ_ALL) {
      const int *truth = s->fw > 0 && !s->sw.eval_always ? (const int *)NULL : (const int *)s->d_truth;
      if (truth != NULL)
        TRY(csgpu_internal_eval_list(s->m, (const csgpu_val *)s->d_child_states, s->d_complete_list,
                                     (const uint64_t *)(s->d_counters + C_COMPLETE), complete, s->d_truth, NULL));
      hipLaunchKernelGGL(cs_accept, dim3((unsigned)((complete + SB - 1) / SB)), dim3(SB), 0, 0, s->d_child_states,
                         truth, (int)complete, n, s->objective, s->obj_var, s->d_counters, s->d_solutions,
                         (long long)s->max_solutions, (const int *)s->d_complete_list, s->d_stream, (long long)s->stream_cap);
    } else {
      const unsigned gw = (unsigned)((complete + 3) / 4);
      hipLaunchKernelGGL(cs_gather_complete, dim3(gw), dim3(SB), 0, 0, s->d_child_states, s->d_complete_list,
                         (int)complete, n, s->d_complete_states);
      TRY(csgpu_eval_batch(s->m, (const csgpu_val *)s->d_complete_states, s->d_truth, complete, NULL));
      hipLaunchKernelGGL(cs_accept, dim3((unsigned)((complete + SB - 1) / SB)), dim3(SB), 0, 0, s->d_complete_states,
                         s->d_truth, (int)complete, n, s->objective, s->obj_var, s->d_counters, s->d_solutions,
                         (long long)s->max_solutions, (const int *)NULL,
                         s->objective == CS_OBJ_ANY ? s->d_stream : (int32_t *)NULL, (long long)s->stream_cap);
    }
    s->pending_complete = complete;
    if (s->objective == CS_OBJ_ANY) TRY(flush_accept_results(s));
  }
  HIP_OK(hipGetLastError());
  return CSGPU_OK;
}


static int enqueue_burst(csgpu_search *s, hipStream_t st) {
  const int n = s->n;
  const int64_t bound = s->parents_max * s->max_width;
  const long long room_limit = pool_room_limit(s);
  const uint64_t *d_children = (const uint64_t *)(s->d_counters + C_TOTAL_CHILDREN);
  const int sense = objective_sense(s->objective);
  const int cpb = scatter_cpb(n, bound);
  const int split = s->path == PATH_BURST_SPLIT;
  const unsigned burst_wgs = (unsigned)((s->parents_max + BURST_PPW - 1) / BURST_PPW);
  const int *truth = s->burst_no_eval ? (const int *)NULL : (const int *)s->d_truth;
  for (int it = 0; it < BURST_ITERATIONS; it++) {
    if (split) {
      hipLaunchKernelGGL(cs_burst_branch, dim3(burst_wgs), dim3(1024), 0, st, s->pool, n, s->d_counters, s->d_burst,
                         s->objective, (long long)s->max_width, (long long)s->cap, room_limit, s->holes, s->d_choice,
                         s->d_block_sum, s->d_block_skip, (const cs_val *)s->d_child_states,
                         (const int *)s->d_complete_list, truth, s->obj_var, s->d_solutions,
                         (long long)s->max_solutions, s->d_best_solution, s->d_best, s->d_stream, (long long)s->stream_cap);
      hipLaunchKernelGGL(cs_burst_emit, dim3(burst_wgs), dim3(1024), 0, st, s->d_nodes, s->d_counters, s->d_burst,
                         s->objective, (const cs_choice *)s->d_choice, (const int *)s->d_block_sum,
                         (const int *)s->d_block_skip);
    } else
      hipLaunchKernelGGL(cs_expand_burst, dim3(1), dim3(1024), 0, st, s->pool, n, s->d_nodes, s->d_counters, s->d_burst,
                         s->objective, (long long)s->max_width, (long long)s->cap, room_limit, s->holes,
                         (const cs_val *)s->d_child_states, (const int *)s->d_complete_list, truth,
                         s->obj_var, s->d_solutions, (long long)s->max_solutions, s->d_best_solution, s->d_best,
                         s->d_stream, (long long)s->stream_cap);
    if (s->fw > 0)
      TRY(csgpu_internal_propagate_fb(s->m, (const csgpu_val *)s->pool, (const uint64_t *)s->pool_forb, s->d_nodes,
                                      (csgpu_val *)s->d_child_states, (uint64_t *)s->d_child_forb, s->d_results, bound,
                                      d_children, st));
    else
      TRY(csgpu_internal_propagate_objdev(s->m, (const csgpu_val *)s->pool, s->d_nodes, (csgpu_val *)s->d_child_states,
                                          s->d_results, bound, d_children, CS_DOM_MIN, CS_DOM_MAX,
                                          sense ? (const int32_t *)s->d_best : NULL, sense, st));
    if (s->prefer_failing)
      hipLaunchKernelGGL(cs_prio_update, dim3((unsigned)((bound + SB - 1) / SB)), dim3(SB), 0, st, (const csgpu_result *)s->d_results,
                         (const csgpu_node *)s->d_nodes, (int)bound, (const unsigned long long *)d_children, n, s->fail_var_known,
                         s->d_prio);
    if (split) {
      hipLaunchKernelGGL(cs_burst_count, dim3(BURST_CLASS_WGS), dim3(1024), 0, st, (const csgpu_result *)s->d_results,
                         (const unsigned long long *)s->d_counters, s->d_block_surv, s->d_block_comp, s->d_block_cuts,
                         s->d_block_props, s->d_block_revs);
      hipLaunchKernelGGL(cs_burst_assign, dim3(BURST_CLASS_WGS), dim3(1024), 0, st, (const csgpu_result *)s->d_results,
                         s->d_dest, s->d_complete_list, s->d_counters, s->d_burst, (const int *)s->d_block_surv,
                         (const int *)s->d_block_comp, (const int *)s->d_block_cuts, (const int *)s->d_block_props,
                         (const int *)s->d_block_revs, (const cs_val *)s->d_child_states, s->pool, n,
                         (const unsigned long long *)s->d_child_forb, s->pool_forb, s->fw);
    } else {
      hipLaunchKernelGGL(cs_classify_small, dim3(1), dim3(1024), 0, st, s->d_results, s->d_dest, s->d_complete_list,
                         s->d_counters, s->d_burst);
      hipLaunchKernelGGL(cs_scatter, dim3((unsigned)((bound + cpb - 1) / cpb)), dim3(SB), 0, st, s->d_child_states, s->d_dest,
                         s->d_counters, 0ll, n, s->pool, s->d_child_forb, s->pool_forb, s->fw, cpb,
                         (const unsigned long long *)(s->d_burst + B_SCATTER_BASE));
    }
    if (truth != NULL)
      TRY(csgpu_internal_eval_list(s->m, (const csgpu_val *)s->d_child_states, s->d_complete_list,
                                   (const uint64_t *)(s->d_counters + C_COMPLETE), bound, s->d_truth, st));
  }
  hipLaunchKernelGGL(cs_accept_burst, dim3(1), dim3(256), 0, st, s->d_child_states, s->d_complete_list, truth, n,
                     s->objective, s->obj_var, s->d_counters, s->d_burst, s->d_solutions, (long long)s->max_solutions,
                     s->d_best_solution, s->d_best, s->d_stream, (long long)s->stream_cap);
  HIP_OK(hipGetLastError());
  return CSGPU_OK;
}

static int run_burst(csgpu_search *s, int64_t budget, int64_t *done) {
  TRY(flush_accept_results(s));
  if (!s->sw.graph_off && (s->burst_exec == NULL || s->burst_limit != s->parents_max)) {
    drop_burst_graph(s);
    hipGraph_t graph = NULL;
    if (hipStreamBeginCapture(s->burst_stream, hipStreamCaptureModeThreadLocal) == hipSuccess) {
      const int rc = enqueue_burst(s, s->burst_stream);
      const hipError_t e = hipStreamEndCapture(s->burst_stream, &graph);
      if (rc != CSGPU_OK) {
        if (graph != NULL) (void)hipGraphDestroy(graph);
        return rc;
      }
      if (e == hipSuccess && graph != NULL && hipGraphInstantiate(&s->burst_exec, graph, NULL, NULL, 0) != hipSuccess)
        s->burst_exec = NULL;
      if (graph != NULL) (void)hipGraphDestroy(graph);
    }
    (void)hipGetLastError();
    s->burst_limit = s->parents_max;
  }
  unsigned long long *h = s->h_burst;
  memset(h, 0, sizeof(unsigned long long) * B_COUNT);
  h[B_TOP] = (unsigned long long)s->top;
  h[B_BUDGET] = (unsigned long long)(budget < BURST_ITERATIONS ? budget : BURST_ITERATIONS);
  h[B_LIMIT] = (unsigned long long)s->parents_limit;
  h[B_LIMIT_MAX] = (unsigned long long)s->parents_max;
  h[B_BACKLOG_DIV] = (unsigned long long)s->sw.backlog_div;
  h[B_ITER_BASE] = (unsigned long long)s->st.iterations;
  h[B_PEAK] = (unsigned long long)s->peak;
  HIP_OK(hipMemcpyAsync(s->d_burst, h, sizeof(unsigned long long) * B_COUNT, hipMemcpyHostToDevice, s->burst_stream));
  if (s->burst_exec != NULL)
    HIP_OK(hipGraphLaunch(s->burst_exec, s->burst_stream));
  else
    TRY(enqueue_burst(s, s->burst_stream));
  HIP_OK(hipMemcpyAsync(h, s->d_burst, sizeof(unsigned long long) * B_COUNT, hipMemcpyDeviceToHost, s->burst_stream));
  HIP_OK(hipMemcpyAsync(h + B_COUNT, s->d_counters, sizeof(unsigned long long) * C_COUNT, hipMemcpyDeviceToHost,
                        s->burst_stream));
  HIP_OK(hipMemcpyAsync(h + B_COUNT + C_COUNT, s->d_best, sizeof(int), hipMemcpyDeviceToHost, s->burst_stream));
  HIP_OK(hipStreamSynchronize(s->burst_stream));
  if (s->sw.trace)
    fprintf(stderr, "burst: iters %llu top %llu nodes %llu cuts %llu | surv %llu complete %llu children %llu solutions %llu stored %llu best %d\n",
            h[B_ITERS], h[B_TOP], h[B_NODES], h[B_CUTS], h[B_COUNT + C_SURVIVORS], h[B_COUNT + C_COMPLETE],
            h[B_COUNT + C_TOTAL_CHILDREN], h[B_COUNT + C_SOLUTIONS], h[B_COUNT + C_STORED], (int)(unsigned)h[B_COUNT + C_BEST]);
  if (h[B_ERROR] != 0ull) return fail(CSGPU_E_LIMIT, "state pool is full");
  *done = (int64_t)h[B_ITERS];
  s->top = (int64_t)h[B_TOP];
  s->peak = (int64_t)h[B_PEAK];
  s->st.iterations += h[B_ITERS];
  s->st.nodes += h[B_NODES];
  s->st.cuts += h[B_CUTS];
  s->st.props += h[B_PROPS];
  s->st.revisions += h[B_REVS];
  s->st.solutions = h[B_COUNT + C_SOLUTIONS];
  if (s->d_stream != NULL) s->stream_rows = (int64_t)h[B_COUNT + C_STREAM] - s->stream_head;
  if (s->objective == CS_OBJ_MIN || s->objective == CS_OBJ_MAX) s->st.best = *(const int *)(h + B_COUNT + C_COUNT);
  if (h[B_IMPROVED] != 0ull) {
    s->have_best_solution = 1;
    s->best_solution_value = (int32_t)(uint32_t)h[B_IMPROVED];
  }
  return CSGPU_OK;
}

static int restart_from_seeds(csgpu_search *s) {
  s->st.restarts++;
  s->top = 0;
  const int keep_flag = s->restart_on_improvement;
  const int64_t keep = s->restart_base;
  s->restart_on_improvement = 0;
  s->restart_base = 0;
  const int rc = csgpu_search_put(s, (const csgpu_val *)s->seed, s->seed_count);
  s->restart_base = keep;
  s->restart_on_improvement = keep_flag;
  return rc;
}

extern "C" int csgpu_search_run(csgpu_search *s, int64_t max_iterations, csgpu_search_stats *stats) {
  if (s == NULL || stats == NULL) return fail(CSGPU_E_ARG, "bad argument");
  if (hipSetDevice(s->device) != hipSuccess) return fail(CSGPU_E_HIP, "hipSetDevice");
  if (s->stream_failed) return fail(CSGPU_E_STATE, "the solution stream overflowed: reset the engine");
  for (int64_t it = 0; it < max_iterations; it++) {
    if (s->top == 0) break;
    if (s->objective == CS_OBJ_ANY && s->st.solutions > 0) break;
    if (s->d_stream != NULL && stream_room(s) < (s->objective == CS_OBJ_ALL ? s->max_width : 1)) break;
    int64_t steps = 1;
    const int32_t best_before = s->st.best;
    const int restarts_on = s->restart_base > 0 && s->seed_count > 0 && s->st.solutions == 0;
    if (burst_path(s)) {
      int64_t budget = max_iterations - it;
      if (s->d_stream != NULL && budget > stream_room(s)) budget = stream_room(s);
      if (restarts_on) {
        const int64_t until = (int64_t)s->luby_threshold * s->restart_base + 1 - s->since_restart;
        if (until < budget) budget = until < 1 ? 1 : until;
      }
      TRY(run_burst(s, budget, &steps));
      if (steps == 0) break;
      it += steps - 1;
    } else {
      TRY(one_iteration(s));
    }
    if (s->restart_on_improvement && s->seed_count > 0 && s->top > 0) {
      TRY(flush_accept_results(s));
      if (s->st.best != best_before) TRY(restart_from_seeds(s));
    }
    if (restarts_on && s->st.solutions == 0 &&
        (s->since_restart += steps) > (int64_t)s->luby_threshold * s->restart_base) {
      s->since_restart = 0;
      cs_luby_next(&s->luby_threshold, &s->luby_counter);
      TRY(restart_from_seeds(s));
    }
  }
  TRY(flush_accept_results(s));
  if (s->d_stream != NULL) {
    unsigned long long err = 0ull;
    HIP_OK(hipMemcpy(&err, s->d_counters + C_STREAM_ERR, sizeof err, hipMemcpyDeviceToHost));
    if (err != 0ull) {
      s->stream_failed = 1;
      return fail(CSGPU_E_LIMIT, "solution stream overflow");
    }
  }
  s->st.pool = s->top;
  s->st.pool_peak = s->peak;
  s->st.done = s->top == 0 || (s->objective == CS_OBJ_ANY && s->st.solutions > 0);
  *stats = s->st;
  return CSGPU_OK;
}

extern "C" int64_t csgpu_search_solutions(const csgpu_search *s, int32_t *values, int64_t max) {
  if (s == NULL || values == NULL || max < 0) return CSGPU_E_ARG;
  if (hipSetDevice(s->device) != hipSuccess) return fail(CSGPU_E_HIP, "hipSetDevice");
  unsigned long long stored = 0;
  if (hipMemcpy(&stored, s->d_counters + C_STORED, sizeof stored, hipMemcpyDeviceToHost) != hipSuccess) return CSGPU_E_HIP;
  int64_t k = (int64_t)stored;
  if (k > s->max_solutions) k = s->max_solutions;
  if (k > max) k = max;
  if (k > 0 && hipMemcpy(values, s->d_solutions, (size_t)k * s->n * sizeof(int32_t), hipMemcpyDeviceToHost) != hipSuccess)
    return CSGPU_E_HIP;
  return k;
}

extern "C" int csgpu_search_best_solution(const csgpu_search *s, int32_t *values) {
  if (s == NULL || values == NULL) return CSGPU_E_ARG;
  if (hipSetDevice(s->device) != hipSuccess) return fail(CSGPU_E_HIP, "hipSetDevice");
  if (!s->have_best_solution || s->best_solution_value != s->st.best) return 0;
  if (hipMemcpy(values, s->d_best_solution, (size_t)s->n * sizeof(int32_t), hipMemcpyDeviceToHost) != hipSuccess)
    return CSGPU_E_HIP;
  return 1;
}

static int stream_drain(csgpu_search *s, int32_t *values, int64_t max, int64_t *count, hipMemcpyKind kind, hipStream_t st) {
  if (s == NULL || values == NULL || count == NULL || max < 0) return fail(CSGPU_E_ARG, "bad argument");
  if (hipSetDevice(s->device) != hipSuccess) return fail(CSGPU_E_HIP, "hipSetDevice");
  if (s->d_stream == NULL) return fail(CSGPU_E_STATE, "no solution stream");
  if (s->stream_failed) return fail(CSGPU_E_STATE, "the solution stream overflowed: reset the engine");
  TRY(flush_accept_results(s));
  *count = 0;
  const int64_t k = max < s->stream_rows ? max : s->stream_rows;
  if (k == 0) return CSGPU_OK;
  HIP_OK(hipDeviceSynchronize());
  const size_t row = (size_t)s->n * sizeof(int32_t);
  const int64_t first = s->stream_head % s->stream_cap, part = k < s->stream_cap - first ? k : s->stream_cap - first;
  HIP_OK(hipMemcpyAsync(values, s->d_stream + (size_t)first * s->n, (size_t)part * row, kind, st));
  if (k > part) HIP_OK(hipMemcpyAsync(values + (size_t)part * s->n, s->d_stream, (size_t)(k - part) * row, kind, st));
  HIP_OK(hipStreamSynchronize(st));
  s->stream_head += k;
  s->stream_rows -= k;
  const unsigned long long head = (unsigned long long)s->stream_head;
  HIP_OK(hipMemcpy(s->d_counters + C_STREAM_HEAD, &head, sizeof head, hipMemcpyHostToDevice));
  *count = k;
  return CSGPU_OK;
}

extern "C" int csgpu_search_drain_solutions(csgpu_search *s, int32_t *values, int64_t max, int64_t *count) {
  return stream_drain(s, values, max, count, hipMemcpyDeviceToHost, (hipStream_t)0);
}

extern "C" int csgpu_search_drain_solutions_device(csgpu_search *s, int32_t *d_values, int64_t max, int64_t *count,
                                                   void *stream) {
  return stream_drain(s, d_values, max, count, hipMemcpyDeviceToDevice, (hipStream_t)stream);
}

extern "C" int csgpu_search_pending_solutions(const csgpu_search *s, int64_t *rows, int64_t *room) {
  if (s == NULL || rows == NULL || room == NULL) return fail(CSGPU_E_ARG, "bad argument");
  if (s->d_stream == NULL) return fail(CSGPU_E_STATE, "no solution stream");
  if (s->stream_failed) return fail(CSGPU_E_STATE, "the solution stream overflowed: reset the engine");
  *rows = s->stream_rows;
  *room = s->stream_cap - s->stream_rows;
  return CSGPU_OK;
}
```

csolve_amd/csrc/cs_step.hip.h:

```cpp
#ifndef CS_STEP_HIP_H
#define CS_STEP_HIP_H

#include "cs_kernels.hip.h"
#include "cs_shave.hip.h"

#define CS_STEP_QN 256
#define CS_STEP_SHARDS 16
#define CS_STEP_STATS 8

struct cs_step_io {
  const uint2 *pool;
  long long first_row;
  int parents;
  int chunk;
  int maxw;
  uint2 *stage;
  int K;
  unsigned *fill;
  unsigned long long *wstat;
  unsigned *ticket;
  int32_t *solutions;
  unsigned long long *stored;
  long long max_solutions;
  int store_open;
  int stream_on;
};

template <int S>
__device__ __forceinline__ unsigned cs_seg_bcast(unsigned x, int src, int lane) {
  return (unsigned)__builtin_amdgcn_ds_bpermute(((lane & ~(S - 1)) + src) << 2, (int)x);
}

template <int G, int NW, bool S3>
struct cs_packed {
  static constexpr int S = CS_WAVE / G;
  static constexpr int W = CS_WAVE;
  static constexpr unsigned KEY_VALUE = (1u << 26) - 1u;
  const unsigned short *s_tab;
  int n, slots, v, row_stride;
  unsigned key_base;
  __device__ __forceinline__ void push_pending(bool &pending, int rl, unsigned *fb) const {
    while (__ballot(pending) != 0ull) {
      const unsigned key = cs_segment_min<S>(pending ? key_base + (unsigned)rl : 0xffffffffu);
      const int ul = (int)(key >> 26);
      const int cd = (int)(key & KEY_VALUE);
      pending = pending && v != ul;
      const int ulc = ul < n ? ul : n - 1;
      const unsigned char *row = (const unsigned char *)s_tab + ulc * row_stride + v * 2;
      if (S3) {
        const int e0 = (int)*(const unsigned short *)(row), e1 = (int)*(const unsigned short *)(row + W * 2),
                  e2 = (int)*(const unsigned short *)(row + 2 * W * 2);
        const unsigned b0_ = (unsigned)(cd - e0), b1_ = (unsigned)(cd - e1), b2_ = (unsigned)(cd - e2);
        fb[0] |= (b0_ < 32u ? 1u << b0_ : 0u) | (b1_ < 32u ? 1u << b1_ : 0u) | (b2_ < 32u ? 1u << b2_ : 0u);
        if (NW == 2)
          fb[1] |= ((b0_ >> 5) == 1u ? 1u << (b0_ & 31u) : 0u) | ((b1_ >> 5) == 1u ? 1u << (b1_ & 31u) : 0u) |
                   ((b2_ >> 5) == 1u ? 1u << (b2_ & 31u) : 0u);
      } else {
        for (int k = 0; k < slots; k++) {
          const unsigned bit = (unsigned)(cd - (int)*(const unsigned short *)(row + (size_t)k * W * 2));
          fb[0] |= bit < 32u ? 1u << bit : 0u;
          if (NW == 2) fb[1] |= (bit >> 5) == 1u ? 1u << (bit & 31u) : 0u;
        }
      }
    }
  }
  __device__ __forceinline__ void decode(uint2 e, bool live, int &rl, int &rh, unsigned *fb) const {
    if (NW == 1) {
      fb[0] = live ? e.x : 0xfffffffeu;
      fb[1] = 0xffffffffu;
      rl = live ? (int)(e.y & 0xffu) : 0;
      rh = live ? (int)((e.y >> 8) & 0xffu) : 0;
    } else {
      fb[0] = live ? e.x : 0xfffffffeu;
      fb[1] = live ? e.y : 0xffffffffu;
      cs_set_bounds_all<2>(fb, &rl, &rh);
      rl = rl > 63 ? 0 : rl;
      rh = rh < 0 ? 0 : rh;
    }
  }
  __device__ __forceinline__ uint2 encode(int rl, int rh, unsigned *fb) const {
    if (NW == 1) return make_uint2(fb[0], (unsigned)rl | ((unsigned)rh << 8));
    cs_set_restrict<2>(fb, rl, rh);
    return make_uint2(fb[0], fb[1]);
  }
};

template <int G, int NW, bool S3>
__global__ __launch_bounds__(1024, 8) void cs_step_packed(int n, const unsigned short *__restrict__ tab_g, int slots,
                                                          const int *__restrict__ root_lo, const int *__restrict__ sym_off,
                                                          int bias, size_t tab_bytes, cs_step_io io) {
  extern __shared__ __attribute__((aligned(16))) unsigned char cs_lds[];
  typedef unsigned long long u64;
  constexpr int S = CS_WAVE / G;
  constexpr int W = CS_WAVE;
  constexpr int LOG_S = G == 4 ? 4 : 5;
  constexpr int WORDS = 1 + NW;
  const int lane = threadIdx.x & (CS_WAVE - 1);
  const int wave_in_block = __builtin_amdgcn_readfirstlane(threadIdx.x >> 6);
  const int waves_per_block = blockDim.x >> 6;
  const int wave_global = (int)blockIdx.x * waves_per_block + wave_in_block;
  {
    const int vecs = (int)(tab_bytes / 16);
    const uint4 *src = (const uint4 *)tab_g;
    uint4 *dst = (uint4 *)cs_lds;
    for (int i = threadIdx.x; i < vecs; i += blockDim.x) dst[i] = src[i];
  }
  unsigned *s_wave = (unsigned *)(cs_lds + ((tab_bytes + 15) & ~(size_t)15)) + (size_t)wave_in_block * (WORDS * 256 + CS_STEP_QN);
  unsigned *s_prl = s_wave;
  unsigned *s_pf = s_wave + 256;
  unsigned *s_q = s_wave + WORDS * 256;
  __syncthreads();

  const int g = lane >> LOG_S, v = lane & (S - 1);
  const bool live = v < n;
  const int vcl = live ? v : n - 1;
  const int b0 = live ? root_lo[vcl] : 0;
  const int deg = live ? sym_off[vcl + 1] - sym_off[vcl] : 0;
  cs_packed<G, NW, S3> P;
  P.s_tab = (const unsigned short *)cs_lds;
  P.n = n; P.slots = slots; P.v = v; P.row_stride = slots * W * 2;
  P.key_base = ((unsigned)v << 26) + (unsigned)bias;

  int c_cur = 0, c_end = 0;
  int exhausted = 0;
  int tk_pending = 0;
  unsigned tk_v = 0u;
  int qhead = 0, qlen = 0;
  int grp_tail = 0;
  int fill = 0;
  int sfill = 0;
  int store_open = io.store_open;
  int acc_fail = 0, acc_sol = 0, acc_parents = 0;
  int acc_nodes = 0, acc_skip = 0, acc_props = 0, acc_revs = 0;
  const size_t region = (size_t)wave_global * (size_t)io.K;
  uint2 pre = make_uint2(0u, 0u);

  auto load_group = [&](int first, int end) -> uint2 {
    const int pidx = first + g < end ? first + g : end - 1;
    const long long prow = io.first_row + (long long)io.parents - 1 - (long long)pidx;
    return io.pool[(size_t)prow * n + vcl];
  };
#define CS_STEP_ASK_TICKET()                                                                                        \
  do {                                                                                                              \
    if (!exhausted && !tk_pending) {                                                                                \
      if (fill + sfill + qlen + (c_end - c_cur + io.chunk) * io.maxw <= io.K) {                                     \
        tk_v = 0u;                                                                                                  \
        if (lane == 0) tk_v = __hip_atomic_fetch_add(io.ticket, 1u, __ATOMIC_RELAXED, __HIP_MEMORY_SCOPE_AGENT);    \
        tk_pending = 1;                                                                                             \
      } else {                                                                                                      \
        exhausted = 1;                           \
      }                                                                                                             \
    }                                                                                                               \
  } while (0)
  CS_STEP_ASK_TICKET();

  for (;;) {
    c_cur = __builtin_amdgcn_readfirstlane(c_cur);
    c_end = __builtin_amdgcn_readfirstlane(c_end);
    exhausted = __builtin_amdgcn_readfirstlane(exhausted);
    tk_pending = __builtin_amdgcn_readfirstlane(tk_pending);
    qhead = __builtin_amdgcn_readfirstlane(qhead);
    qlen = __builtin_amdgcn_readfirstlane(qlen);
    grp_tail = __builtin_amdgcn_readfirstlane(grp_tail);
    fill = __builtin_amdgcn_readfirstlane(fill);
    sfill = __builtin_amdgcn_readfirstlane(sfill);
    store_open = __builtin_amdgcn_readfirstlane(store_open);
    acc_fail = __builtin_amdgcn_readfirstlane(acc_fail);
    acc_sol = __builtin_amdgcn_readfirstlane(acc_sol);
    acc_parents = __builtin_amdgcn_readfirstlane(acc_parents);
    int grp_live = 0;
    if (qlen > 0) {
      const unsigned d0 = s_q[qhead];
      const int grp_head = (int)((__builtin_amdgcn_readfirstlane((int)d0) & 0xff) >> (G == 4 ? 2 : 1));
      grp_live = (grp_tail - grp_head) & 3;
      if (grp_live == 0) grp_live = 4;
    }
    if (grp_live < 4 && qlen + G * io.maxw <= CS_STEP_QN) {
      if (c_cur == c_end && tk_pending) {
        tk_pending = 0;
        const long long first = (long long)__builtin_amdgcn_readfirstlane((int)tk_v) * io.chunk;
        if (first < (long long)io.parents) {
          c_cur = (int)first;
          c_end = first + io.chunk < (long long)io.parents ? (int)first + io.chunk : io.parents;
          pre = load_group(c_cur, c_end);
        } else {
          exhausted = 1;
        }
      }
      if (c_cur < c_end) {
        const bool pvalid = c_cur + g < c_end;
        const int had = c_end - c_cur < G ? c_end - c_cur : G;
        const uint2 e = pre;
        c_cur += had;
        acc_parents += had;
        if (c_cur < c_end) pre = load_group(c_cur, c_end);
        else CS_STEP_ASK_TICKET();
        int rl, rh;
        unsigned fb[2];
        P.decode(e, live, rl, rh, fb);
        const bool open = live && pvalid && rl != rh;
        const unsigned kmin = cs_segment_min<S>(open ? ((unsigned)(rh - rl) << 8) | (unsigned)v : 0xffffffffu);
        const int bv = (int)(kmin & 0xffu);
        const bool any_open = kmin != 0xffffffffu;
        const unsigned prl = (unsigned)rl | ((unsigned)rh << 8);
        const unsigned prl_b = cs_seg_bcast<S>(prl, bv & (S - 1), lane);
        const unsigned f0_b = cs_seg_bcast<S>(fb[0], bv & (S - 1), lane);
        const unsigned f1_b = NW == 2 ? cs_seg_bcast<S>(fb[1], bv & (S - 1), lane) : 0u;
        const int rlb = (int)(prl_b & 0xffu), rhb = (int)((prl_b >> 8) & 0xffu);
        unsigned a0, a1 = 0u;
        if (NW == 1) {
          a0 = ~f0_b & (~0u << rlb) & (~0u >> (31 - rhb));
        } else {
          const unsigned lo_m0 = rlb < 32 ? ~0u << rlb : 0u, lo_m1 = rlb < 32 ? ~0u : ~0u << (rlb - 32);
          const unsigned hi_m0 = rhb < 32 ? ~0u >> (31 - rhb) : ~0u, hi_m1 = rhb < 32 ? 0u : ~0u >> (63 - rhb);
          a0 = ~f0_b & lo_m0 & hi_m0;
          a1 = ~f1_b & lo_m1 & hi_m1;
        }
        if (!any_open) { a0 = 0u; a1 = 0u; }
        const int width = any_open ? rhb - rlb + 1 : 0;
        const int cnt = __popc(a0) + (NW == 2 ? __popc(a1) : 0);
        if (v == 0) { acc_nodes += width; acc_skip += width - cnt; }
        const int slot_lane = grp_tail * 64 + lane;
        s_prl[slot_lane] = prl;
        s_pf[slot_lane] = fb[0];
        if (NW == 2) s_pf[256 + slot_lane] = fb[1];
        int off = 0, total = 0;
#pragma unroll
        for (int gg = 0; gg < G; gg++) {
          const int c = __builtin_amdgcn_readlane(cnt, gg * S);
          off += g > gg ? c : 0;
          total += c;
        }
        const unsigned desc_base = (unsigned)(grp_tail * G + g) | ((unsigned)bv << 8);
        const int qbase = qhead + qlen + off;
#pragma unroll
        for (int p = 0; p < (32 * NW) / S; p++) {
          const int bit = v + p * S;
          const unsigned word = (NW == 2 && bit >= 32) ? a1 : a0;
          const int b5 = bit & 31;
          if ((word >> b5) & 1u) {
            int rank = __popc(word & ((1u << b5) - 1u));
            if (NW == 2 && bit >= 32) rank += __popc(a0);
            s_q[(qbase + rank) & (CS_STEP_QN - 1)] = desc_base | ((unsigned)bit << 16);
          }
        }
        if (total > 0) {
          qlen += total;
          grp_tail = (grp_tail + 1) & 3;
        }
        continue;
      }
    }
    if (qlen == 0) break;

    const int take = qlen < G ? qlen : G;
    const bool valid = g < take;
    const unsigned d = s_q[(qhead + (valid ? g : 0)) & (CS_STEP_QN - 1)];
    qhead = (qhead + take) & (CS_STEP_QN - 1);
    qlen -= take;
    const int slot = (int)(d & 0xffu), nvar = (int)((d >> 8) & 0xffu), nval = (int)(d >> 16);
    const int src = slot * S + v;
    const unsigned prl = s_prl[src];
    unsigned fb[2];
    fb[0] = s_pf[src];
    fb[1] = NW == 2 ? s_pf[256 + src] : 0xffffffffu;
    int rl = (int)(prl & 0xffu), rh = (int)((prl >> 8) & 0xffu);
    const bool mine = v == nvar;
    if (mine) { rl = nval; rh = nval; }
    const int rl0 = rl, rh0 = rh;
    bool pending = mine && valid;
    const unsigned valid_lo = G == 2 ? 0xffffffffu : (take >= 2 ? 0xffffffffu : 0x0000ffffu);
    const unsigned valid_hi = G == 2 ? (take >= 2 ? 0xffffffffu : 0u) : (take >= 4 ? 0xffffffffu : (take == 3 ? 0x0000ffffu : 0u));
    const u64 validm = ((u64)valid_hi << 32) | (u64)valid_lo;
    u64 failedm = 0ull, pushedm = __ballot(pending);
    for (;;) {
      P.push_pending(pending, rl, fb);
      int first, last;
      bool bad;
      if (NW == 1) {
        const unsigned a = ~fb[0] & (~0u << rl) & (~0u >> (31 - rh));
        bad = a == 0u;
        first = __builtin_ctz(a | 0x80000000u);
        last = 31 - __builtin_clz(a | 1u);
      } else {
        cs_set_bounds<2>(fb, rl, rh, &first, &last);
        bad = last < 0;
      }
      const bool newly = !bad && first == last && rl != rh;
      rl = bad ? rl : first;
      rh = bad ? rh : last;
      const u64 badm = __ballot(bad);
      if (badm != 0ull) failedm |= cs_segments_any<G>(badm);
      const u64 newm = __ballot(newly) & ~failedm & validm;
      if (newm == 0ull) break;
      pending = __builtin_amdgcn_inverse_ballot_w64(newm);
      pushedm |= newm;
    }
    failedm &= validm;
    const u64 openm = cs_segments_any<G>(__ballot(live && rl != rh)) & validm;
    const u64 survm = openm & ~failedm, complm = validm & ~failedm & ~openm;
    acc_fail += __popcll(failedm) >> LOG_S;
    acc_props += __builtin_amdgcn_inverse_ballot_w64(validm & ~failedm) ? (rl - rl0) + (rh0 - rh) : 0;
    acc_revs += __builtin_amdgcn_inverse_ballot_w64(pushedm) ? deg : 0;
    if (survm != 0ull) {
      const int rank = (int)__builtin_amdgcn_mbcnt_hi((unsigned)(survm >> 32), __builtin_amdgcn_mbcnt_lo((unsigned)survm, 0u)) >> LOG_S;
      const uint2 e = P.encode(rl, rh, fb);
      if (__builtin_amdgcn_inverse_ballot_w64(survm) && live) io.stage[(region + (size_t)(fill + rank)) * n + v] = e;
      fill += __popcll(survm) >> LOG_S;
    }
    if (complm != 0ull) {
      const int ns = __popcll(complm) >> LOG_S;
      acc_sol += ns;
      if (io.stream_on) {
        const int rank = (int)__builtin_amdgcn_mbcnt_hi((unsigned)(complm >> 32), __builtin_amdgcn_mbcnt_lo((unsigned)complm, 0u)) >> LOG_S;
        if (__builtin_amdgcn_inverse_ballot_w64(complm) && live)
          io.stage[(region + (size_t)(io.K - 1 - (sfill + rank))) * n + v] = make_uint2((unsigned)(b0 + rl), 0u);
        sfill += ns;
      }
      if (store_open) {
        unsigned long long s0 = 0ull;
        if (lane == 0) s0 = atomicAdd(io.stored, (unsigned long long)ns);
        const long long slot0 = (long long)(((u64)(unsigned)__builtin_amdgcn_readfirstlane((int)(s0 >> 32)) << 32) |
                                            (u64)(unsigned)__builtin_amdgcn_readfirstlane((int)s0));
        const int rank = (int)__builtin_amdgcn_mbcnt_hi((unsigned)(complm >> 32), __builtin_amdgcn_mbcnt_lo((unsigned)complm, 0u)) >> LOG_S;
        if (__builtin_amdgcn_inverse_ballot_w64(complm) && live && slot0 + rank < io.max_solutions)
          io.solutions[(size_t)(slot0 + rank) * n + v] = b0 + rl;
        if (slot0 + ns >= io.max_solutions) store_open = 0;
      }
    }
  }
  const int nodes = cs_wave_sum(acc_nodes), skip = cs_wave_sum(acc_skip), props = cs_wave_sum(acc_props),
            revs = cs_wave_sum(acc_revs);
  if (lane == 0) {
    io.fill[wave_global] = (unsigned)fill;
    unsigned long long *st = io.wstat + (size_t)wave_global * CS_STEP_STATS;
    st[0] = (unsigned long long)nodes;
    st[1] = (unsigned long long)(skip + acc_fail);
    st[2] = (unsigned long long)props;
    st[3] = (unsigned long long)revs;
    st[4] = (unsigned long long)acc_sol;
    st[5] = (unsigned long long)acc_parents;
  }
#undef CS_STEP_ASK_TICKET
}

template <int G, int NW, bool S3>
__global__ __launch_bounds__(256) void cs_step_import(int n, const unsigned short *__restrict__ tab_g, int slots,
                                                      const int *__restrict__ root_lo, int bias, size_t tab_bytes,
                                                      uint2 *__restrict__ rows, long long first_row, long long count) {
  extern __shared__ __attribute__((aligned(16))) unsigned char cs_lds[];
  constexpr int S = CS_WAVE / G;
  constexpr int TOP = 32 * NW - 1;
  {
    const int vecs = (int)(tab_bytes / 16);
    const uint4 *src = (const uint4 *)tab_g;
    uint4 *dst = (uint4 *)cs_lds;
    for (int i = threadIdx.x; i < vecs; i += blockDim.x) dst[i] = src[i];
  }
  __syncthreads();
  const int lane = threadIdx.x & (CS_WAVE - 1);
  const int v = lane & (S - 1);
  const bool live = v < n;
  const int vcl = live ? v : n - 1;
  const int b0 = live ? root_lo[vcl] : 0;
  cs_packed<G, NW, S3> P;
  P.s_tab = (const unsigned short *)cs_lds;
  P.n = n; P.slots = slots; P.v = v; P.row_stride = slots * CS_WAVE * 2;
  P.key_base = ((unsigned)v << 26) + (unsigned)bias;
  const long long segs = (long long)gridDim.x * (blockDim.x / S);
  const long long groups = (count + G - 1) / G;
  for (long long q = (long long)blockIdx.x * (blockDim.x >> 6) + (threadIdx.x >> 6); q < groups; q += segs / G) {
    const long long r = q * G + lane / S;
    const bool valid = r < count;
    const size_t at = (size_t)(first_row + (valid ? r : count - 1)) * n + vcl;
    const cs_val d = ((const cs_val *)rows)[at];
    int rl = live ? d.lo - b0 : 0, rh = live ? d.hi - b0 : 0;
    rl = rl < 0 ? 0 : (rl > TOP ? TOP : rl);
    rh = rh < 0 ? 0 : (rh > TOP ? TOP : rh);
    unsigned fb[2];
    fb[0] = live ? 0u : 0xfffffffeu;
    fb[1] = live ? 0u : 0xffffffffu;
    bool pending = live && valid && rl == rh;
    P.push_pending(pending, rl, fb);
    const uint2 e = P.encode(rl, rh, fb);
    if (valid && live) rows[at] = e;
  }
}

template <int NW>
__global__ __launch_bounds__(256) void cs_step_export(int n, const int *__restrict__ root_lo, uint2 *__restrict__ rows,
                                                      long long elements) {
  const long long i = (long long)blockIdx.x * blockDim.x + threadIdx.x;
  if (i >= elements) return;
  const uint2 e = rows[i];
  const int b0 = root_lo[(int)(i % n)];
  int rl, rh;
  if (NW == 1) {
    rl = (int)(e.y & 0xffu);
    rh = (int)((e.y >> 8) & 0xffu);
  } else {
    unsigned fb[2] = { e.x, e.y };
    cs_set_bounds_all<2>(fb, &rl, &rh);
  }
  ((cs_val *)rows)[i] = cs_interval(b0 + rl, b0 + rh);
}

__device__ __forceinline__ unsigned cs_wave_min_u32(unsigned x) {
  unsigned y;
  y = (unsigned)__builtin_amdgcn_update_dpp((int)0xffffffffu, (int)x, 0x111, 0xf, 0xf, false); x = y < x ? y : x;
  y = (unsigned)__builtin_amdgcn_update_dpp((int)0xffffffffu, (int)x, 0x112, 0xf, 0xf, false); x = y < x ? y : x;
  y = (unsigned)__builtin_amdgcn_update_dpp((int)0xffffffffu, (int)x, 0x114, 0xf, 0xf, false); x = y < x ? y : x;
  y = (unsigned)__builtin_amdgcn_update_dpp((int)0xffffffffu, (int)x, 0x118, 0xf, 0xf, false); x = y < x ? y : x;
  y = (unsigned)__builtin_amdgcn_update_dpp((int)0xffffffffu, (int)x, 0x142, 0xa, 0xf, false); x = y < x ? y : x;
  y = (unsigned)__builtin_amdgcn_update_dpp((int)0xffffffffu, (int)x, 0x143, 0xc, 0xf, false); x = y < x ? y : x;
  return (unsigned)__builtin_amdgcn_readlane((int)x, 63);
}

template <typename E, int R, int SL, bool FULL>
__global__ __launch_bounds__(1024, (R <= 2 ? 8 : 4)) void cs_step_shave(int n, const E *__restrict__ tab_g, int slots, int dmin,
                                                                        const int *__restrict__ root_lo,
                                                                        const int *__restrict__ sym_off, size_t tab_bytes,
                                                                        cs_step_io io) {
  extern __shared__ __attribute__((aligned(16))) unsigned char cs_lds[];
  typedef unsigned long long u64;
  const int lane = threadIdx.x & (CS_WAVE - 1);
  const int wave_in_block = __builtin_amdgcn_readfirstlane(threadIdx.x >> 6);
  const int waves_per_block = blockDim.x >> 6;
  const int wave_global = (int)blockIdx.x * waves_per_block + wave_in_block;
  if (SL != 0) slots = SL;
  {
    const int vecs = (int)(tab_bytes / 16);
    const uint4 *src = (const uint4 *)tab_g;
    uint4 *dst = (uint4 *)cs_lds;
    for (int i = threadIdx.x; i < vecs; i += blockDim.x) dst[i] = src[i];
  }
  unsigned *s_mask = (unsigned *)(cs_lds + ((tab_bytes + 15) & ~(size_t)15)) + (size_t)wave_in_block * 8;
  __syncthreads();
  const cs_val *pool = (const cs_val *)io.pool;
  cs_val *stage = (cs_val *)io.stage;

  cs_shave_core<E, R, SL, false> C;
  C.s_tab = (const E *)cs_lds; C.slots = slots; C.lane = lane; C.s_trace = nullptr; C.tcount = 0u;
  int b0[R], vcl[R];
  bool live[R];
#pragma unroll
  for (int r = 0; r < R; r++) {
    const int v = lane + r * CS_WAVE;
    live[r] = FULL || v < n;
    vcl[r] = live[r] ? v : n - 1;
    b0[r] = live[r] ? root_lo[vcl[r]] : 0;
    C.b0[r] = b0[r];
    C.kb[r] = b0[r] - dmin;
    C.deg[r] = live[r] ? sym_off[vcl[r] + 1] - sym_off[vcl[r]] : 0;
    C.livemask[r] = FULL ? ~0ull : __ballot(live[r]);
  }
  constexpr int W = CS_WAVE * R;

  int fill = 0, sfill = 0 , store_open = io.store_open;
  int acc_nodes = 0, acc_cuts = 0, acc_sol = 0, acc_parents = 0, acc_revs = 0;
  int acc_props = 0;
  const size_t region = (size_t)wave_global * (size_t)io.K;
  int shard = wave_global % CS_STEP_SHARDS, tried = 0;

#define CS_STEP_DRAW(OUT)                                                                                            \
  do {                                                                                                               \
    (OUT) = -1;                                                                                                      \
    while (tried < CS_STEP_SHARDS) {                                                                                 \
      const int count_s_ = (io.parents - shard + CS_STEP_SHARDS - 1) / CS_STEP_SHARDS;                               \
      unsigned t_ = 0u;                                                                                              \
      if (count_s_ > 0) {                                                                                            \
        if (lane == 0) t_ = __hip_atomic_fetch_add(io.ticket + shard * 16, 1u, __ATOMIC_RELAXED, __HIP_MEMORY_SCOPE_AGENT); \
        t_ = (unsigned)__builtin_amdgcn_readfirstlane((int)t_);                                                      \
      }                                                                                                              \
      if (count_s_ > 0 && t_ < (unsigned)count_s_) { (OUT) = (int)t_ * CS_STEP_SHARDS + shard; break; }              \
      shard = (shard + 1) % CS_STEP_SHARDS;                                                                          \
      tried++;                                                                                                       \
    }                                                                                                                \
  } while (0)
  auto load_parent = [&](int p, cs_val *pd) {
    const size_t prow = (size_t)(io.first_row + (long long)io.parents - 1 - (long long)p) * n;
#pragma unroll
    for (int r = 0; r < R; r++) pd[r] = pool[prow + vcl[r]];
  };

  int p_cur = -1;
  if (io.maxw <= io.K) CS_STEP_DRAW(p_cur);
  cs_val pd[R];
  if (p_cur >= 0) load_parent(p_cur, pd);
  while (p_cur >= 0) {
    p_cur = __builtin_amdgcn_readfirstlane(p_cur);
    fill = __builtin_amdgcn_readfirstlane(fill);
    sfill = __builtin_amdgcn_readfirstlane(sfill);
    shard = __builtin_amdgcn_readfirstlane(shard);
    tried = __builtin_amdgcn_readfirstlane(tried);
    store_open = __builtin_amdgcn_readfirstlane(store_open);
    int plo[R], phi[R];
#pragma unroll
    for (int r = 0; r < R; r++) {
      plo[r] = live[r] ? pd[r].lo - b0[r] : 0;
      phi[r] = live[r] ? pd[r].hi - b0[r] : 0;
    }
    acc_parents++;
    int p_next = -1;
    if (fill + sfill + 2 * io.maxw <= io.K) CS_STEP_DRAW(p_next);
    if (p_next >= 0) load_parent(p_next, pd);
    u64 pval[R];
    unsigned key = 0xffffffffu;
#pragma unroll
    for (int r = R - 1; r >= 0; r--) {
      pval[r] = __ballot(plo[r] == phi[r]) & C.livemask[r];
      const bool open = live[r] && plo[r] != phi[r];
      const unsigned k = ((unsigned)(phi[r] - plo[r]) << 8) | (unsigned)(lane + r * CS_WAVE);
      key = open && k < key ? k : key;
    }
    const unsigned kmin = cs_wave_min_u32(key);
    if (kmin != 0xffffffffu) {
      const int bv = (int)(kmin & 0xffu), br = bv >> 6, bl = bv & 63;
      int blo = 0, bhi = 0, kbw = 0;
#pragma unroll
      for (int r = 0; r < R; r++)
        if (r == br) {
          blo = __builtin_amdgcn_readlane(plo[r], bl);
          bhi = __builtin_amdgcn_readlane(phi[r], bl);
          kbw = __builtin_amdgcn_readlane(C.kb[r], bl);
        }
      const int width = bhi - blo + 1;
      if (lane < 8) s_mask[lane] = 0u;
      {
        const E *row = (const E *)cs_lds + (size_t)bv * slots * W + lane;
        for (int k = 0; k < slots; k++) {
#pragma unroll
          for (int r2 = 0; r2 < R; r2++) {
            const int c = (int)row[k * W + r2 * CS_WAVE] + plo[r2] - kbw - blo;
            if (__builtin_amdgcn_inverse_ballot_w64(pval[r2]) && c >= 0 && c < width) atomicOr(&s_mask[c >> 5], 1u << (c & 31));
          }
        }
      }
      acc_nodes += width;
      for (int wd = 0; wd * 32 < width; wd++) {
        unsigned m = (unsigned)__builtin_amdgcn_readfirstlane((int)s_mask[wd]);
        const int bits = width - wd * 32 < 32 ? width - wd * 32 : 32;
        unsigned todo = ~m & (bits == 32 ? 0xffffffffu : (1u << bits) - 1u);
        acc_cuts += bits - __builtin_popcount(todo);
        while (todo != 0u) {
          const int j = __builtin_ctz(todo);
          todo &= todo - 1u;
          const int value = blo + wd * 32 + j;
          int rlo[R], rhi[R], lo0[R], hi0[R];
          u64 pushed[R], push[R], dl[R], dh[R], val[R];
#pragma unroll
          for (int r = 0; r < R; r++) {
            rlo[r] = plo[r]; rhi[r] = phi[r];
            pushed[r] = pval[r] | ~C.livemask[r];
            push[r] = 0ull; dl[r] = 0ull; dh[r] = 0ull;
            val[r] = pval[r];
            if (r == br) {
              if (lane == bl) { rlo[r] = value; rhi[r] = value; }
              push[r] = 1ull << bl;
              val[r] |= push[r];
            }
            lo0[r] = rlo[r]; hi0[r] = rhi[r];
          }
          int rounds = 0, revisions = 0;
          const int fail_var = C.fixpoint(rlo, rhi, pushed, push, dl, dh, val, rounds, revisions);
          if (rounds != 0) __builtin_amdgcn_s_setprio(0);
          acc_revs += revisions;
          int open_vars = 0;
#pragma unroll
          for (int r = 0; r < R; r++) {
            open_vars += __popcll(__ballot(rlo[r] != rhi[r]));
            if (fail_var < 0) acc_props += (rlo[r] - lo0[r]) + (hi0[r] - rhi[r]);
          }
          if (fail_var >= 0) {
            acc_cuts++;
          } else if (open_vars > 0) {
            const size_t orow = (region + (size_t)fill) * n;
#pragma unroll
            for (int r = 0; r < R; r++)
              if (live[r]) stage[orow + lane + r * CS_WAVE] = cs_interval(rlo[r] + b0[r], rhi[r] + b0[r]);
            fill++;
          } else {
            acc_sol++;
            if (io.stream_on) {
              const size_t orow = (region + (size_t)(io.K - 1 - sfill)) * n;
#pragma unroll
              for (int r = 0; r < R; r++)
                if (live[r]) stage[orow + lane + r * CS_WAVE] = cs_value(rlo[r] + b0[r]);
              sfill++;
            }
            if (store_open) {
              unsigned long long s0 = 0ull;
              if (lane == 0) s0 = atomicAdd(io.stored, 1ull);
              const long long slot0 = (long long)(((u64)(unsigned)__builtin_amdgcn_readfirstlane((int)(s0 >> 32)) << 32) |
                                                  (u64)(unsigned)__builtin_amdgcn_readfirstlane((int)s0));
              if (slot0 < io.max_solutions) {
#pragma unroll
                for (int r = 0; r < R; r++)
                  if (live[r]) io.solutions[(size_t)slot0 * n + lane + r * CS_WAVE] = rlo[r] + b0[r];
              }
              if (slot0 + 1 >= io.max_solutions) store_open = 0;
            }
          }
        }
      }
    }
    p_cur = p_next;
  }
  const int props = cs_wave_sum(acc_props);
  if (lane == 0) {
    io.fill[wave_global] = (unsigned)fill;
    unsigned long long *st = io.wstat + (size_t)wave_global * CS_STEP_STATS;
    st[0] = (unsigned long long)acc_nodes;
    st[1] = (unsigned long long)acc_cuts;
    st[2] = (unsigned long long)props;
    st[3] = (unsigned long long)acc_revs;
    st[4] = (unsigned long long)acc_sol;
    st[5] = (unsigned long long)acc_parents;
  }
#undef CS_STEP_DRAW
}

__global__ __launch_bounds__(256) void cs_collect(const unsigned *__restrict__ fill, int waves, const uint2 *__restrict__ stage,
                                                  int K, int n, uint2 *__restrict__ pool, long long first_row, int parents,
                                                  int chunk, const unsigned *__restrict__ ticket,
                                                  const unsigned long long *__restrict__ wstat,
                                                  unsigned long long *__restrict__ out,
                                                  const unsigned long long *__restrict__ stored,
                                                  int32_t *__restrict__ stream, long long stream_base, long long stream_limit,
                                                  long long stream_cap, unsigned long long *__restrict__ stream_err) {
  __shared__ unsigned long long s_red[256];
  const int w = blockIdx.x, t = threadIdx.x;
  const unsigned long long drawn = chunk == 0 ? (unsigned long long)parents : (unsigned long long)*ticket * (unsigned long long)chunk;
  const long long consumed = drawn < (unsigned long long)parents ? (long long)drawn : (long long)parents;
  unsigned long long before = 0ull;
  for (int i = t; i < w; i += 256) before += fill[i];
  s_red[t] = before;
  __syncthreads();
  for (int d = 128; d > 0; d >>= 1) {
    if (t < d) s_red[t] += s_red[t + d];
    __syncthreads();
  }
  before = s_red[0];
  __syncthreads();
  const size_t count = (size_t)fill[w] * n;
  const uint2 *src = stage + (size_t)w * K * n;
  uint2 *dst = pool + (size_t)(first_row + parents - consumed + (long long)before) * n;
  size_t e = t;
  for (; e + 768 < count; e += 1024) {
    const uint2 a = src[e], b = src[e + 256], c = src[e + 512], d = src[e + 768];
    dst[e] = a; dst[e + 256] = b; dst[e + 512] = c; dst[e + 768] = d;
  }
  for (; e < count; e += 256) dst[e] = src[e];
  if (stream != nullptr) {
    unsigned long long sb = 0ull;
    for (int i = t; i < w; i += 256) sb += wstat[(size_t)i * CS_STEP_STATS + 4];
    __syncthreads();
    s_red[t] = sb;
    __syncthreads();
    for (int d = 128; d > 0; d >>= 1) {
      if (t < d) s_red[t] += s_red[t + d];
      __syncthreads();
    }
    const long long sbefore = (long long)s_red[0];
    __syncthreads();
    const int rows = (int)wstat[(size_t)w * CS_STEP_STATS + 4];
    const long long at = stream_base + sbefore;
    if (rows > 0 && at + rows > stream_limit) {
      if (t == 0) *stream_err = 1ull;
    } else {
      const uint2 *rsrc = stage + (size_t)w * K * n;
      const long long r0 = at % stream_cap;
      const int total = rows * n;
      for (int f = t; f < total; f += 256) {
        const int j = f / n, v = f - j * n;
        long long r = r0 + j;
        r = r >= stream_cap ? r - stream_cap : r;
        stream[(size_t)r * n + v] = (int32_t)rsrc[(size_t)(K - 1 - j) * n + v].x;
      }
    }
  }
  if (w == 0) {
    for (int k = 0; k < 6; k++) {
      unsigned long long x = 0ull;
      for (int i = t; i < waves; i += 256) x += k < 5 ? wstat[(size_t)i * CS_STEP_STATS + k] : (unsigned long long)fill[i];
      s_red[t] = x;
      __syncthreads();
      for (int d = 128; d > 0; d >>= 1) {
        if (t < d) s_red[t] += s_red[t + d];
        __syncthreads();
      }
      if (t == 0) out[k < 5 ? 2 + k : 1] = s_red[0];
      __syncthreads();
    }
    if (t == 0) {
      out[0] = (unsigned long long)consumed;
      out[7] = *stored;
    }
  }
}

#endif
```

csolve_amd/solver.py:

```python
from __future__ import annotations

import contextlib
import ctypes as C

import numpy as np
import torch

from ._lib import (MANY_ROTATE_FIRST, MANY_SLOT_FRESH, PLAN_FAMILIES, CsolveError, ManyOptions, ManyRestartOptions, ManyResult,
                   ManyStream, ManyUptoOptions, Node, Result, SearchStats, Val, check, demangle, load_library)

STATUS_FAIL = -1


def _stream_ptr(stream) -> int:
    if stream is None:
        stream = torch.cuda.current_stream()
    return int(stream.cuda_stream)


class Model:

    def __init__(self, handle):
        self._h = handle
        self.finalized = False
# ... 950 lines not shown
                            if p is not None:
                                p.close()
        assert obj == 1, "solve_many_clauses_spread walks under ALL, or under the model's MIN / MAX"
        family = dict(solve=self.solve_many_clauses, resume=self.resume_many_clauses, children=self.clause_checkpoint_children,
                      fanout=self.clause_checkpoint_fanout, make_pool=self.many_clause_checkpoints,
                      slot_bytes=self.clause_checkpoint_bytes(), qualifies=self.qualifies_many_clauses())
        return self._spread_call(family, roots, budgets, max_rounds, max_rows, solutions, stream, pool_bytes, pools)

    def _solve_many_clauses_spread_best(self, roots, obj, budgets, max_rounds, max_rows, solutions, stream, pool_bytes, pools,
                                        own_pools) -> dict:
        slot_bytes = max(self.clause_checkpoint_bytes(), 1)
        minimise = obj == 2

        def pool_for(rnd, batch):
            k = rnd % 2
            need = max(1, min(batch, pool_bytes // slot_bytes))
            if own_pools and (pools[k] is None or pools[k].capacity < need):
                if pools[k] is not None:
                    pools[k].close()
                pools[k] = self.many_clause_checkpoints(need)
            else:
                pools[k].reset(stream)
            return pools[k]

        def budget(rnd):
            return budgets[min(rnd, len(budgets) - 1)]

        if not self.qualifies_many_clauses() or self.objective != obj:
            self.solve_many_clauses(roots, obj, max_nodes=budget(0), solutions=solutions, stream=stream)
        pool = pool_for(0, int(roots.shape[0]))
        main = self.solve_many_clauses(roots, obj, max_nodes=budget(0), solutions=solutions, stream=stream, checkpoints=pool)
        K = main["status"].shape[0]
        dev = main["status"].device
        limited = torch.zeros((max(K, 1),), dtype=torch.int32, device=dev)
        has = None
        batch, owner = main, None
        rounds, round_rows = 1, []

        def owners_of(index):
            return index if owner is None else owner.long()[index]

        def leave(last):
            nonlocal has
            T = batch["status"].shape[0]
            rows = torch.arange(T, dtype=torch.int64, device=dev)
            stopped = batch["status"] == 1
            if not last:
                stopped = stopped & (batch["slot"] < 0)
            stopped = stopped | (batch["status"] == 3)
            limited.index_add_(0, owners_of(rows), stopped.to(torch.int32))
            if owner is None:
                has = batch["solutions"] > 0
                return
            self.fold_many(batch, owner, main, stream)
            found, value, row = self.fold_many_best(batch, owner, K, obj, stream)
            mine = main["best"]
            take = found & (~has | (value < mine if minimise else value > mine))
            if solutions:
                main["first"].copy_(torch.where(take[:, None], batch["first"][row.clamp(max=max(T - 1, 0))], main["first"]))
            mine.copy_(torch.where(take, value, mine))
            has = has | found

        while rounds < max_rounds and K > 0:
            index = torch.nonzero((batch["status"] == 1) & (batch["slot"] >= 0)).flatten()
            S = int(index.shape[0])
            if S == 0:
                break
            slots = batch["slot"][index].contiguous()
            children = self.clause_checkpoint_children(pool, slots, stream, objective=obj)
            offsets = torch.zeros((S + 1,), dtype=torch.int64, device=dev)
            torch.cumsum(children.clamp(min=0), 0, out=offsets[1:])
            total = int(offsets[-1].item())
            if total > max_rows:
                self.resume_many_clauses(batch, max_nodes=budget(rounds), stream=stream, own_solutions=owner is not None)
                round_rows.append(0)
                rounds += 1
                continue
            limited.index_add_(0, owners_of(index), (children < 0).to(torch.int32))
            if total == 0:
                break
            leave(False)
            whose = owners_of(index)
            owner_start = torch.stack([main["best"][whose], has[whose].to(torch.int32)], 1).contiguous()
            rows, came_from, start = self.clause_checkpoint_fanout(pool, slots, offsets, total, stream=stream, objective=obj,
                                                                   owner_start=owner_start)
            owner = whose[came_from.long()].to(torch.int32).contiguous()
            pool = pool_for(rounds, total)
            batch = self.solve_many_clauses(rows, obj, max_nodes=budget(rounds), solutions=solutions, stream=stream,
                                            checkpoints=pool, start=start)
            round_rows.append(total)
            rounds += 1
        leave(True)
        status = main["status"]
        status.copy_(torch.where(status == 2, status, (limited[:K] > 0).to(status.dtype)))
        if own_pools:
            torch.cuda.current_stream().synchronize()
        out = {k: v for k, v in main.items() if not k.startswith("_") and k != "slot"}
        out["rounds"], out["sub_instances"], out["round_rows"] = rounds, sum(round_rows), round_rows
        return out

    def _many_symbol(self, export: str):
        buf = C.create_string_buffer(1024)
        check(getattr(load_library(), export)(self._h, buf, len(buf)))
        return demangle(buf.value.decode()) if buf.value else None

    def many_kernel(self):
        return self._many_symbol("csgpu_internal_many_symbol")

    def many_resume_kernel(self):
        return self._many_symbol("csgpu_internal_many_resume_symbol")

    def many_upto_kernel(self):
        return self._many_symbol("csgpu_internal_many_upto_symbol")

    def many_allowed_kernel(self):
        return self._many_symbol("csgpu_internal_many_allowed_symbol")

    def many_allowed_upto_kernel(self):
        return self._many_symbol("csgpu_internal_many_allowed_upto_symbol")

    def many_restart_kernel(self):
        return self._many_symbol("csgpu_internal_many_restart_symbol")

    def many_waves(self, count: int) -> int:
        return int(load_library().csgpu_internal_many_waves(self._h, int(count)))

    def forbidden_words(self) -> int:
        return load_library().csgpu_model_forbidden_words(self._h)

    def propagate_fb(self, states_in, nodes, forb_in=None, states_out=None, forb_out=None, results=None,
                     want_forb=True, stream=None):
        n, fw = self.n_vars, self.forbidden_words()
        assert fw > 0, "model does not qualify for the forbidden-set kernel"
        assert states_in.is_cuda and states_in.dtype == torch.int32 and states_in.is_contiguous()
        assert nodes.is_cuda and nodes.dtype == torch.int32 and nodes.is_contiguous()
        B = nodes.shape[0]
        if states_out is None:
            states_out = torch.empty((B, n, 2), dtype=torch.int32, device=nodes.device)
        if results is None:
            results = torch.empty((B, 4), dtype=torch.int32, device=nodes.device)
        if forb_out is None and want_forb:
            forb_out = torch.empty((B, n, fw), dtype=torch.int64, device=nodes.device)
        if forb_in is not None:
            assert forb_in.dtype == torch.int64 and forb_in.is_contiguous() and forb_in.shape[-2:] == (n, fw)
            assert forb_in.shape[0] == states_in.shape[0]
        check(load_library().csgpu_propagate_batch_fb(
            self._h, states_in.data_ptr(), 0 if forb_in is None else forb_in.data_ptr(), nodes.data_ptr(),
            states_out.data_ptr(), 0 if forb_out is None else forb_out.data_ptr(), results.data_ptr(), B,
            _stream_ptr(stream)))
        return states_out, forb_out, results

    def pack_sets(self, states: torch.Tensor, stream=None) -> torch.Tensor:
        n, fw = self.n_vars, self.forbidden_words()
        assert states.is_cuda and states.dtype == torch.int32 and states.is_contiguous() and states.shape[-2:] == (n, 2)
        sets = torch.empty((states.shape[0], n, fw), dtype=torch.int64, device=states.device)
        check(load_library().csgpu_sets_pack(self._h, states.data_ptr(), sets.data_ptr(), states.shape[0], _stream_ptr(stream)))
        return sets

    def unpack_sets(self, sets: torch.Tensor, stream=None) -> torch.Tensor:
        n, fw = self.n_vars, self.forbidden_words()
        assert sets.is_cuda and sets.dtype == torch.int64 and sets.is_contiguous() and sets.shape[-2:] == (n, fw)
        states = torch.empty((sets.shape[0], n, 2), dtype=torch.int32, device=sets.device)
        check(load_library().csgpu_sets_unpack(self._h, sets.data_ptr(), states.data_ptr(), sets.shape[0], _stream_ptr(stream)))
        return states

    def propagate_sets(self, sets_in: torch.Tensor, nodes: torch.Tensor, sets_out: torch.Tensor = None,
                       results: torch.Tensor = None, stream=None):
        n, fw = self.n_vars, self.forbidden_words()
        assert sets_in.is_cuda and sets_in.dtype == torch.int64 and sets_in.is_contiguous() and sets_in.shape[-2:] == (n, fw)
        assert nodes.is_cuda and nodes.dtype == torch.int32 and nodes.is_contiguous() and nodes.shape[-1] == 4
        B = nodes.shape[0]
        if sets_out is None:
            sets_out = torch.empty((B, n, fw), dtype=torch.int64, device=nodes.device)
        if results is None:
            results = torch.empty((B, 4), dtype=torch.int32, device=nodes.device)
        check(load_library().csgpu_propagate_batch_sets(self._h, sets_in.data_ptr(), nodes.data_ptr(), sets_out.data_ptr(),
                                                        results.data_ptr(), B, _stream_ptr(stream)))
        return sets_out, results

    def eval_root(self, states: torch.Tensor, stream=None) -> torch.Tensor:
        assert states.is_cuda and states.dtype == torch.int32 and states.is_contiguous()
        B = states.shape[0]
        truth = torch.empty((B,), dtype=torch.int32, device=states.device)
        check(load_library().csgpu_eval_batch(self._h, states.data_ptr(), truth.data_ptr(), B, _stream_ptr(stream)))
        return truth

    def eval_clauses(self, state: torch.Tensor, stream=None) -> torch.Tensor:
        assert state.is_cuda and state.dtype == torch.int32 and state.is_contiguous()
        out = torch.empty((max(1, self.n_clauses), 2), dtype=torch.int32, device=state.device)
        check(load_library().csgpu_eval_clauses(self._h, state.data_ptr(), out.data_ptr(), _stream_ptr(stream)))
        return out[: self.n_clauses]

    def propagate_one(self, state: np.ndarray, var: int, lo: int, hi: int):
        state = np.ascontiguousarray(state, dtype=np.int32)
        out = np.empty_like(state)
        res = Result()
        check(load_library().csgpu_propagate_one(self._h, state.ctypes.data, Node(var, lo, hi, 0),
                                                 out.ctypes.data, C.byref(res)))
        return res.status, res.props, out


    def propagate_one_causes(self, state: np.ndarray, var: int, lo: int, hi: int, cap: int = 4096):
        state = np.ascontiguousarray(state, dtype=np.int32)
        out = np.empty_like(state)
        res = Result()
        trace = np.empty((cap, 4), dtype=np.int32)
        cnt = C.c_int32()
        check(load_library().csgpu_propagate_one_causes(self._h, state.ctypes.data, Node(var, lo, hi, 0), out.ctypes.data,
                                                        C.byref(res), trace.ctypes.data, cap, C.byref(cnt)))
        if cnt.value > min(cap, 2048):
            raise OverflowError(f"{cnt.value} trace records, {min(cap, 2048)} kept")
        return res.status, res.props, (out if res.status >= 0 else None), trace[: cnt.value].copy()

    def propagate_one_chain(self, state: np.ndarray, var: int, lo: int, hi: int, cap: int = 4096):
        state = np.ascontiguousarray(state, dtype=np.int32)
        st, props, cnt = C.c_int32(), C.c_int32(), C.c_int32()
        bumps = np.empty(cap, dtype=np.int32)
        check(load_library().csgpu_propagate_one_chain(self._h, state.ctypes.data, Node(var, lo, hi, 0), C.byref(st),
                                                        C.byref(props), bumps.ctypes.data, cap, C.byref(cnt)))
        return st.value, props.value, bumps[: min(cap, cnt.value)].copy()

    def propagate_one_traced(self, state: np.ndarray, var: int, lo: int, hi: int, cap: int = 4096):
        state = np.ascontiguousarray(state, dtype=np.int32)
        out = np.empty_like(state)
        res = Result()
        trace = np.empty((cap, 4), dtype=np.int32)
        cnt = C.c_int32()
        check(load_library().csgpu_propagate_one_traced(self._h, state.ctypes.data, Node(var, lo, hi, 0), out.ctypes.data,
                                                        C.byref(res), trace.ctypes.data, cap, C.byref(cnt)))
        if cnt.value > cap:
            raise OverflowError(f"{cnt.value} trace records, room for {cap}")
        return res.status, res.props, (out if res.status >= 0 else None), trace[: cnt.value].copy()

    def propagate_values(self, state: np.ndarray, var: int, values):
        state = np.ascontiguousarray(state, dtype=np.int32)
        values = np.ascontiguousarray(values, dtype=np.int32)
        outs = np.empty((len(values),) + state.shape, dtype=np.int32)
        res = np.empty((len(values), 4), dtype=np.int32)
        check(load_library().csgpu_propagate_values(self._h, state.ctypes.data, var, values.ctypes.data, len(values),
                                                    outs.ctypes.data, res.ctypes.data))
        return res, outs

    def server_stats(self):
        seconds, calls, starts = (C.c_double * 4)(), C.c_uint64(), C.c_uint64()
        check(load_library().csgpu_debug_one_timing(self._h, seconds, C.byref(calls), C.byref(starts)))
        return calls.value, starts.value

    def root_propagate_limit(self, limit: int):
        st, rounds = C.c_int32(), C.c_int32()
        check(load_library().csgpu_model_root_propagate_limit(self._h, limit, C.byref(st), C.byref(rounds)))
        return st.value, rounds.value


class ManyCheckpoints:

    def __init__(self, model: Model, capacity: int, clauses: bool = False):
        self.model = model
        self.capacity = int(capacity)
        self.clauses = bool(clauses)
        self._h = C.c_void_p()
        L = load_library()
        create = L.csgpu_many_clause_checkpoints_create if self.clauses else L.csgpu_many_checkpoints_create
        check(create(model._h, self.capacity, C.byref(self._h)))

    def reset(self, stream=None):
        check(load_library().csgpu_many_checkpoints_reset(self._h, _stream_ptr(stream)))
        return self

    def close(self):
        if self._h:
            load_library().csgpu_many_checkpoints_free(self._h)
            self._h = None

    def __del__(self):
        try:
            self.close()
        except Exception:
            pass


class ManySolutionStream:

    def __init__(self, model: Model, rows: int):
        self.capacity = int(rows)
        cap = max(self.capacity, 1)
        self.rows = torch.empty((cap, model.n_vars), dtype=torch.int32, device="cuda")
        self.owner = torch.empty((cap,), dtype=torch.int32, device="cuda")
        self.count = torch.zeros((1,), dtype=torch.int64, device="cuda")

    def struct(self) -> ManyStream:
        return ManyStream(self.rows.data_ptr(), self.owner.data_ptr(), self.count.data_ptr(), self.capacity)

    def take(self):
        m = min(int(self.count.item()), max(self.capacity, 0))
        owner, rows = self.owner[:m].clone(), self.rows[:m].clone()
        self.count.zero_()
        return owner, rows


def set_linear_fast_paths(on: bool):
    load_library().csgpu_set_linear_fast_paths(1 if on else 0)


class Search:

    def __init__(self, model: Model, pool_capacity: int = 1 << 20, max_children: int = 1 << 16):
        self.model = model
        self._h = C.c_void_p()
        check(load_library().csgpu_search_create(model._h, pool_capacity, max_children, C.byref(self._h)))
        self.device = torch.device("cuda", torch.cuda.current_device())
        self.stats = None

    def close(self):
        if self._h:
            load_library().csgpu_search_free(self._h)
            self._h = None

    def __del__(self):
        try:
            self.close()
        except Exception:
            pass

    def reset(self):
        check(load_library().csgpu_search_reset(self._h))

    def put(self, states: torch.Tensor):
        if states.numel() == 0:
            return
        assert states.is_cuda and states.dtype == torch.int32 and states.is_contiguous()
        assert states.shape[-2:] == (self.model.n_vars, 2)
        check(load_library().csgpu_search_put(self._h, states.data_ptr(), states.shape[0]))

    def take(self, max_states: int) -> torch.Tensor:
        buf = torch.empty((max(1, max_states), self.model.n_vars, 2), dtype=torch.int32, device="cuda")
        cnt = C.c_int64()
        check(load_library().csgpu_search_take(self._h, buf.data_ptr(), max_states, C.byref(cnt)))
        return buf[: cnt.value]

    def set_parents(self, parents_per_iteration: int):
        check(load_library().csgpu_search_set_parents(self._h, int(parents_per_iteration)))

    def set_restart(self, iterations: int):
        check(load_library().csgpu_search_set_restart(self._h, int(iterations)))

    ORDERS = {"none": 0, "smallest-domain": 1, "largest-domain": 2, "smallest-value": 3, "largest-value": 4}

    def set_strategy(self, order="smallest-domain", prefer_failing: bool = False):
        o = self.ORDERS[order] if isinstance(order, str) else int(order)
        check(load_library().csgpu_search_set_strategy(self._h, o, int(bool(prefer_failing))))

    def set_restart_on_improvement(self, on: bool = True):
        check(load_library().csgpu_search_set_restart_on_improvement(self._h, int(bool(on))))

    def share_incumbent(self, other: "Search"):
        check(load_library().csgpu_search_share_incumbent(self._h, other._h))

    def set_best(self, best: int):
        check(load_library().csgpu_search_set_best(self._h, int(best)))

    def put_cost(self):
        sec, cnt = C.c_double(), C.c_int64()
        check(load_library().csgpu_search_put_cost(self._h, C.byref(sec), C.byref(cnt)))
        return sec.value, cnt.value

    def run(self, max_iterations: int = 1 << 62) -> dict:
        st = SearchStats()
        check(load_library().csgpu_search_run(self._h, max_iterations, C.byref(st)))
        return {k: getattr(st, k) for k, _ in SearchStats._fields_}

    def best_solution(self):
        out = np.empty(self.model.n_vars, dtype=np.int32)
        rc = check(load_library().csgpu_search_best_solution(self._h, out.ctypes.data))
        return out if rc == 1 else None

    def solutions(self, max_solutions: int = 1024) -> np.ndarray:
        out = np.empty((max(1, max_solutions), self.model.n_vars), dtype=np.int32)
        k = load_library().csgpu_search_solutions(self._h, out.ctypes.data, max_solutions)
        check(k)
        return out[:k]

    DEFAULT_STREAM_ROWS = 1 << 18

    def stream_solutions(self, rows: int | None = None):
        check(load_library().csgpu_search_set_solution_stream(self._h, int(rows or self.DEFAULT_STREAM_ROWS)))

    def pending_solutions(self):
        rows, room = C.c_int64(), C.c_int64()
        check(load_library().csgpu_search_pending_solutions(self._h, C.byref(rows), C.byref(room)))
        return rows.value, room.value

    def drain_solutions(self, max_rows: int | None = None) -> np.ndarray:
        rows, _ = self.pending_solutions()
        rows = rows if max_rows is None else min(rows, int(max_rows))
        out = np.empty((max(1, rows), self.model.n_vars), dtype=np.int32)
        cnt = C.c_int64()
        check(load_library().csgpu_search_drain_solutions(self._h, out.ctypes.data, rows, C.byref(cnt)))
        return out[: cnt.value]

    def drain_solutions_device(self, max_rows: int | None = None) -> torch.Tensor:
        rows, _ = self.pending_solutions()
        rows = rows if max_rows is None else min(rows, int(max_rows))
        out = torch.empty((max(1, rows), self.model.n_vars), dtype=torch.int32, device=self.device)
        cnt = C.c_int64()
        with torch.cuda.device(self.device):
            stream = torch.cuda.current_stream()
        check(load_library().csgpu_search_drain_solutions_device(self._h, out.data_ptr(), rows, C.byref(cnt),
                                                                 int(stream.cuda_stream)))
        return out[: cnt.value]

    def iter_solutions(self, slice_iterations: int = 64, device: bool = False):
        try:
            self.pending_solutions()
        except CsolveError:
            self.stream_solutions()
        drain = self.drain_solutions_device if device else self.drain_solutions
        while True:
            st = self.run(slice_iterations)
            batch = drain()
            if len(batch):
                yield batch
            if st["done"]:
                break
        self.stats = st


def solve_root(text: str, weights_on: bool = True) -> Model:
    m = Model.from_text(text, weights_on)
    if m.root_propagate() < 0:
        raise ValueError("INFEASIBLE PROBLEM")
    m.normalize()
    if m.root_propagate() < 0:
        raise ValueError("INFEASIBLE PROBLEM")
    return m.finalize()
```

Baseline: 21.36 billion.

## Draw next-level parents directly from staging buffers instead of compacting into pool

```diff
diff --git a/csolve_amd/_lib.py b/csolve_amd/_lib.py
--- a/csolve_amd/_lib.py
+++ b/csolve_amd/_lib.py
@@ -216,6 +216,9 @@
     L.csgpu_search_set_strategy.argtypes = [vp, C.c_int, C.c_int]
     L.csgpu_search_set_restart_on_improvement.argtypes = [vp, C.c_int]
     L.csgpu_internal_plan_symbol.argtypes = [vp, C.c_int, C.c_char_p, C.c_size_t]
+    if hasattr(L, "csgpu_internal_stage_map"):
+        L.csgpu_internal_stage_map.argtypes = [vp, i32, i32, i64, i64, i64, vp, vp]
+        L.csgpu_internal_search_direct_trace.argtypes = [vp, vp]
     L.csgpu_solve_many.argtypes = [vp, vp, i64, C.POINTER(ManyOptions), vp, vp, vp]
     L.csgpu_internal_many_symbol.argtypes = [vp, C.c_char_p, C.c_size_t]
     L.csgpu_internal_many_waves.argtypes = [vp, i64]
diff --git a/csolve_amd/csrc/cs_capi.hip b/csolve_amd/csrc/cs_capi.hip
--- a/csolve_amd/csrc/cs_capi.hip
+++ b/csolve_amd/csrc/cs_capi.hip
@@ -1306,6 +1306,7 @@
 
 static int launch_step_shave(const csgpu_model *m, const csgpu_step_launch *L, void *stream) {
   const cs_planned *k = &m->plan.step_shave;
+  if (L->direct || L->staged != 0) return set_err(CSGPU_E_ARG, "step kernel: no direct draw for models of more than 32 variables");
   const int n = m->host->n_vars, maxw = m->plan.max_width;
   int64_t waves = step_shave_waves(m, L->stage_rows);
   if (waves < k->waves || (int64_t)L->parents > csgpu_internal_step_parents_limit(m, L->stage_rows))
@@ -1330,6 +1331,11 @@
   io.max_solutions = (long long)L->max_solutions;
   io.store_open = L->store_open;
   io.stream_on = L->stream != NULL;
+  io.prev = NULL;
+  io.prev_prefix = NULL;
+  io.prev_waves = 0;
+  io.prev_K = 0;
+  io.staged = 0;
   int nn = n, slots = m->img->dense_slots, dmin_d = m->img->dense_dmin;
   const void *tab_d = m->d_dense_tab;
   const int *root_lo_d = m->d_root_lo, *sym_off = m->d_sym_off;
@@ -1341,18 +1347,21 @@
                      0 , (const unsigned *)L->ticket, (const unsigned long long *)L->wstat,
                      (unsigned long long *)L->out, (const unsigned long long *)L->stored,
                      L->stream, (long long)L->stream_base, (long long)L->stream_limit, (long long)L->stream_cap,
-                     (unsigned long long *)L->stream_err);
+                     (unsigned long long *)L->stream_err, 1);
   HIP_TRY(hipGetLastError());
   return CSGPU_OK;
 }
 
-extern "C" int csgpu_internal_step(const csgpu_model *m, const csgpu_step_launch *L, void *stream) {
+extern "C" int csgpu_internal_step(const csgpu_model *m, csgpu_step_launch *L, void *stream) {
   const int kind = csgpu_internal_step_kind(m);
   if (kind == 0 || L == NULL || L->parents < 1) return set_err(CSGPU_E_ARG, "bad argument");
   if (kind == 2) return launch_step_shave(m, L, stream);
   const int n = m->host->n_vars;
   const int G = m->plan.packed_nodes, maxw = m->plan.max_width;
   if (G * maxw > CS_STEP_QN) return set_err(CSGPU_E_LIMIT, "step kernel: interval too wide for the child queue");
+  if (L->staged < 0 || L->staged > 0x3fffffff || (L->direct && L->prefix == NULL) ||
+      (L->staged > 0 && (L->prev == NULL || L->prev_prefix == NULL || L->prev_waves < 1 || L->prev_K < 1 || L->prev_K > 0x7fffffff)))
+    return set_err(CSGPU_E_ARG, "step kernel: bad direct draw");
   int64_t waves = (int64_t)m->n_cus * 32;
   const int64_t by_stage = L->stage_rows / (2 * (int64_t)G * maxw);
   if (waves > by_stage) waves = by_stage;
@@ -1385,6 +1394,13 @@
   io.max_solutions = (long long)L->max_solutions;
   io.store_open = L->store_open;
   io.stream_on = L->stream != NULL;
+  io.prev = (const uint2 *)L->prev;
+  io.prev_prefix = L->prev_prefix;
+  io.prev_waves = L->prev_waves;
+  io.prev_K = (int)L->prev_K;
+  io.staged = (int)L->staged;
+  L->waves_used = (int32_t)waves;
+  L->K_used = io.K;
   int nn = n, slots = m->img->dense_slots, bias = m->packed_bias;
   const void *tab_d = m->d_packed_tab;
   const int *root_lo_d = m->d_root_lo, *sym_off = m->d_sym_off;
@@ -1392,13 +1408,53 @@
   void *args[] = { &nn, &tab_d, &slots, &root_lo_d, &sym_off, &bias, &tab_bytes, &io };
   HIP_TRY(hipLaunchKernel(m->plan.step_packed.fn, dim3((unsigned)grid), dim3((unsigned)(wg_waves * CS_WAVE)), args,
                           step_packed_lds(m, wg_waves), (hipStream_t)stream));
-  hipLaunchKernelGGL(cs_collect, dim3((unsigned)waves), dim3(256), 0, (hipStream_t)stream, (const unsigned *)L->fill, (int)waves,
-                     (const uint2 *)L->stage, io.K, n, (uint2 *)L->pool, (long long)L->first_row, (int)L->parents,
-                     (int)chunk, (const unsigned *)L->ticket, (const unsigned long long *)L->wstat,
-                     (unsigned long long *)L->out, (const unsigned long long *)L->stored,
-                     L->stream, (long long)L->stream_base, (long long)L->stream_limit, (long long)L->stream_cap,
-                     (unsigned long long *)L->stream_err);
+  if (L->direct)
+    hipLaunchKernelGGL(cs_level_book, dim3(1), dim3(1024), 0, (hipStream_t)stream, (const unsigned *)L->fill, (int)waves,
+                       (int)L->parents, (int)chunk, (const unsigned *)L->ticket, (const unsigned long long *)L->wstat,
+                       (unsigned long long *)L->out, (const unsigned long long *)L->stored, (unsigned *)L->prefix);
+  if (!L->direct || L->stream != NULL)
+    hipLaunchKernelGGL(cs_collect, dim3((unsigned)waves), dim3(256), 0, (hipStream_t)stream, (const unsigned *)L->fill, (int)waves,
+                       (const uint2 *)L->stage, io.K, n, (uint2 *)L->pool, (long long)L->first_row, (int)L->parents,
+                       (int)chunk, (const unsigned *)L->ticket, (const unsigned long long *)L->wstat,
+                       (unsigned long long *)L->out, (const unsigned long long *)L->stored,
+                       L->stream, (long long)L->stream_base, (long long)L->stream_limit, (long long)L->stream_cap,
+                       (unsigned long long *)L->stream_err, L->direct ? 0 : 1);
   HIP_TRY(hipGetLastError());
+  return CSGPU_OK;
+}
+
+extern "C" int csgpu_internal_stage_flush(const csgpu_model *m, const csgpu_val *stage, const uint32_t *prefix, int32_t waves,
+                                          int64_t K, csgpu_val *d_pool, int64_t pool_row, int64_t rows, void *stream) {
+  if (csgpu_internal_step_kind(m) != 1 || stage == NULL || prefix == NULL || d_pool == NULL || waves < 1 || K < 1 ||
+      K > 0x7fffffff || pool_row < 0 || rows < 0 || rows > 0x7fffffff)
+    return set_err(CSGPU_E_ARG, "bad argument");
+  if (rows == 0) return CSGPU_OK;
+  hipLaunchKernelGGL(cs_stage_flush, dim3((unsigned)waves), dim3(256), 0, (hipStream_t)stream, (const unsigned *)prefix,
+                     (const uint2 *)stage, (int)K, m->host->n_vars, (uint2 *)d_pool, (long long)pool_row, (unsigned)rows);
+  HIP_TRY(hipGetLastError());
+  return CSGPU_OK;
+}
+
+extern "C" int csgpu_internal_stage_map(const uint32_t *fill, int32_t waves, int32_t K, int64_t pool_top, int64_t first,
+                                        int64_t count, int64_t *rows, int32_t *in_stage) {
+  if (fill == NULL || waves < 1 || K < 1 || pool_top < 0 || first < 0 || count < 0 || (count > 0 && (rows == NULL || in_stage == NULL)))
+    return set_err(CSGPU_E_ARG, "bad argument");
+  unsigned *prefix = (unsigned *)malloc(((size_t)waves + 1) * sizeof *prefix);
+  if (prefix == NULL) return set_err(CSGPU_E_LIMIT, "out of memory");
+  prefix[0] = 0u;
+  for (int32_t w = 0; w < waves; w++) {
+    if (fill[w] > (uint32_t)K) { free(prefix); return set_err(CSGPU_E_ARG, "a region holds more rows than it has"); }
+    prefix[w + 1] = prefix[w] + fill[w];
+  }
+  const int64_t staged = prefix[waves];
+  if (first + count > staged + pool_top) { free(prefix); return set_err(CSGPU_E_ARG, "more parents than rows"); }
+  cs_stage_cursor c = { 0, 0u, 0u };
+  for (int64_t i = 0; i < count; i++) {
+    int st = 0;
+    rows[i] = cs_parent_row(first + i, staged, prefix, waves, K, pool_top, &c, &st);
+    in_stage[i] = st;
+  }
+  free(prefix);
   return CSGPU_OK;
 }
 
diff --git a/csolve_amd/csrc/cs_internal.h b/csolve_amd/csrc/cs_internal.h
--- a/csolve_amd/csrc/cs_internal.h
+++ b/csolve_amd/csrc/cs_internal.h
@@ -69,12 +69,26 @@
   int64_t stream_limit;
   int64_t stream_cap;
   uint64_t *stream_err;
+  int32_t direct;
+  uint32_t *prefix;
+  const csgpu_val *prev;
+  const uint32_t *prev_prefix;
+  int32_t prev_waves;
+  int64_t prev_K;
+  int64_t staged;
+  int32_t waves_used;
+  int64_t K_used;
 } csgpu_step_launch;
 int csgpu_internal_step_kind(const csgpu_model *m);
 int64_t csgpu_internal_step_parents_limit(const csgpu_model *m, int64_t stage_rows);
 int64_t csgpu_internal_step_stage_rows(const csgpu_model *m);
 int64_t csgpu_internal_step_waves(const csgpu_model *m);
-int csgpu_internal_step(const csgpu_model *m, const csgpu_step_launch *L, void *stream);
+int csgpu_internal_step(const csgpu_model *m, csgpu_step_launch *L, void *stream);
+int csgpu_internal_stage_flush(const csgpu_model *m, const csgpu_val *stage, const uint32_t *prefix, int32_t waves,
+                               int64_t K, csgpu_val *d_pool, int64_t pool_row, int64_t rows, void *stream);
+int csgpu_internal_stage_map(const uint32_t *fill, int32_t waves, int32_t K, int64_t pool_top, int64_t first,
+                             int64_t count, int64_t *rows, int32_t *in_stage);
+int csgpu_internal_search_direct_trace(const csgpu_search *s, int64_t *out);
 int csgpu_internal_step_import(const csgpu_model *m, csgpu_val *d_rows, int64_t first_row, int64_t count, void *stream);
 int csgpu_internal_step_export(const csgpu_model *m, csgpu_val *d_rows, int64_t first_row, int64_t count, void *stream);
 
diff --git a/csolve_amd/csrc/cs_search.hip b/csolve_amd/csrc/cs_search.hip
--- a/csolve_amd/csrc/cs_search.hip
+++ b/csolve_amd/csrc/cs_search.hip
@@ -22,6 +22,7 @@
   int holes_off;
   int sets_off;
   int fused_off;
+  int direct_off;
   int trace;
   int64_t parents_max;
   int64_t backlog_div;
@@ -46,6 +47,7 @@
   w.holes_off = env_is("CSGPU_SEARCH_HOLES", '0');
   w.sets_off = env_is("CSGPU_SEARCH_SETS", '0');
   w.fused_off = env_is("CSGPU_SEARCH_FUSED", '0');
+  w.direct_off = env_is("CSGPU_SEARCH_DIRECT", '0');
   w.trace = getenv("CSGPU_SEARCH_TRACE") != NULL;
   w.parents_max = env_count("CSGPU_SEARCH_PARENTS_MAX", 8192);
   w.backlog_div = env_count("CSGPU_SEARCH_BACKLOG_DIV", 4);
@@ -103,6 +105,11 @@
   int counted;
   int64_t stage_rows;
   uint32_t *d_fill, *d_ticket;
+  int direct;
+  int64_t staged, staged_K;
+  int32_t staged_waves, stage_cur;
+  uint32_t *d_prefix[2];
+  int64_t direct_trace[8];
   uint64_t *d_wstat, *d_step_out, *h_step_out;
   double surv_per_parent;
   uint64_t stored_seen;
@@ -192,6 +199,7 @@
   (void)hipFree(s->d_burst);
   (void)hipFree(s->d_prio);
   (void)hipFree(s->d_stream);
+  (void)hipFree(s->d_prefix[0]); (void)hipFree(s->d_prefix[1]);
   (void)hipFree(s->d_fill); (void)hipFree(s->d_ticket); (void)hipFree(s->d_wstat); (void)hipFree(s->d_step_out);
   if (s->h_step_out) (void)hipHostFree(s->h_step_out);
   if (s->h_burst) (void)hipHostFree(s->h_burst);
@@ -241,6 +249,11 @@
   if (levels) {
     const int64_t waves = csgpu_internal_step_waves(m);
     ALLOC(s->d_fill, sizeof(uint32_t) * (size_t)waves);
+    s->direct = csgpu_internal_step_kind(m) == 1 && !s->sw.direct_off;
+    if (s->direct) {
+      ALLOC(s->d_prefix[0], sizeof(uint32_t) * ((size_t)waves + 1));
+      ALLOC(s->d_prefix[1], sizeof(uint32_t) * ((size_t)waves + 1));
+    }
     ALLOC(s->d_wstat, sizeof(uint64_t) * 8 * (size_t)waves);
     ALLOC(s->d_ticket, 1024);
     ALLOC(s->d_step_out, sizeof(uint64_t) * 8);
@@ -349,7 +362,28 @@
   return CSGPU_OK;
 }
 
+static cs_val *stage_buffer(const csgpu_search *s, int b) {
+  return b == 0 ? s->d_child_states : s->pool + (size_t)(s->cap - s->stage_rows) * s->n;
+}
+
+static int flush_staged(csgpu_search *s) {
+  if (s->staged == 0) return CSGPU_OK;
+  TRY(csgpu_internal_stage_flush(s->m, (const csgpu_val *)stage_buffer(s, s->stage_cur),
+                                 s->d_prefix[s->stage_cur], s->staged_waves, s->staged_K, (csgpu_val *)s->pool,
+                                 s->top - s->staged, s->staged, NULL));
+  s->direct_trace[5]++;
+  s->staged = 0;
+  return CSGPU_OK;
+}
+
+extern "C" int csgpu_internal_search_direct_trace(const csgpu_search *s, int64_t *out) {
+  if (s == NULL || out == NULL) return CSGPU_E_ARG;
+  memcpy(out, s->direct_trace, sizeof s->direct_trace);
+  return CSGPU_OK;
+}
+
 static int search_put(csgpu_search *s, const csgpu_val *d_states, int64_t count) {
+  TRY(flush_staged(s));
   if (s->top + count > s->cap) return fail(CSGPU_E_LIMIT, "state pool is full");
   if (count > 0)
     HIP_OK(hipMemcpy(s->pool + (size_t)s->top * s->n, d_states, (size_t)count * s->n * sizeof(cs_val),
@@ -393,6 +427,8 @@
   if (hipSetDevice(s->device) != hipSuccess) return fail(CSGPU_E_HIP, "hipSetDevice");
   s->top = 0;
   s->peak = 0;
+  s->staged = 0;
+  memset(s->direct_trace, 0, sizeof s->direct_trace);
   memset(&s->st, 0, sizeof s->st);
   s->st.best = s->objective == CS_OBJ_MIN ? CS_DOM_MAX : (s->objective == CS_OBJ_MAX ? CS_DOM_MIN : 0);
   s->seed_count = 0;
@@ -468,6 +504,7 @@
 extern "C" int csgpu_search_take(csgpu_search *s, csgpu_val *d_states, int64_t max, int64_t *count) {
   if (s == NULL || d_states == NULL || count == NULL || max < 0) return fail(CSGPU_E_ARG, "bad argument");
   if (hipSetDevice(s->device) != hipSuccess) return fail(CSGPU_E_HIP, "hipSetDevice");
+  TRY(flush_staged(s));
   int64_t k = max < s->top ? max : s->top;
   *count = k;
   if (k == 0) return CSGPU_OK;
@@ -627,6 +664,16 @@
 }
 
 static int one_iteration_fused(csgpu_search *s) {
+  int direct = s->direct;
+  int32_t write_buf = 0;
+  if (direct && s->staged > 0) {
+    write_buf = 1 - s->stage_cur;
+    if (write_buf == 1 && s->cap - s->stage_rows - s->top < s->stage_rows) {
+      TRY(flush_staged(s));
+      direct = 0;
+      write_buf = 0;
+    }
+  }
   const int64_t reserve = pool_reserve(s);
   const double spp = s->surv_per_parent < 0.25 ? 0.25 : s->surv_per_parent;
   int64_t parents = s->top;
@@ -634,6 +681,7 @@
   if (parents > by_stage) parents = by_stage;
   const int64_t room = s->cap - s->top - reserve;
   const int64_t by_pool = room > 0 ? (int64_t)((double)room / (spp * (double)s->n)) : 0;
+  const int pool_limited = parents > by_pool;
   if (parents > by_pool) parents = by_pool;
   if (parents > 0x3fffffff) parents = 0x3fffffff;
   if (parents < 1) parents = 1;
@@ -643,8 +691,17 @@
   L.pool = (const csgpu_val *)s->pool;
   L.first_row = s->top - parents;
   L.parents = (int32_t)parents;
-  L.stage = (csgpu_val *)s->d_child_states;
+  L.stage = (csgpu_val *)stage_buffer(s, write_buf);
   L.stage_rows = s->stage_rows;
+  L.direct = direct;
+  L.prefix = direct ? s->d_prefix[write_buf] : NULL;
+  L.prev = (const csgpu_val *)stage_buffer(s, s->stage_cur);
+  L.prev_prefix = direct ? s->d_prefix[s->stage_cur] : NULL;
+  L.prev_waves = s->staged_waves;
+  L.prev_K = s->staged_K;
+  L.staged = s->staged;
+  L.waves_used = 0;
+  L.K_used = 0;
   if (L.stage_rows > s->cap - s->top) L.stage_rows = s->cap - s->top;
   {
     const int64_t limit = csgpu_internal_step_parents_limit(s->m, L.stage_rows);
@@ -675,6 +732,24 @@
   const uint64_t *h = s->h_step_out;
   const int64_t consumed = (int64_t)h[0], survivors = (int64_t)h[1];
   if (consumed < 1) return fail(CSGPU_E_LIMIT, "internal: a frontier of the fused search consumed no parent");
+  if (direct) {
+    int64_t *tr = s->direct_trace;
+    tr[0]++;
+    tr[s->staged > 0 ? 1 : 2]++;
+    tr[6] += survivors == 0;
+    tr[7] += pool_limited;
+    if (consumed < s->staged) {
+      const int64_t rest = s->staged - consumed;
+      TRY(csgpu_internal_stage_flush(s->m, L.prev, L.prev_prefix, L.prev_waves, L.prev_K, (csgpu_val *)s->pool,
+                                     s->top - s->staged, rest, NULL));
+      tr[3]++;
+      tr[4] += rest;
+    }
+    s->staged = survivors;
+    s->staged_waves = L.waves_used;
+    s->staged_K = L.K_used;
+    s->stage_cur = write_buf;
+  }
   s->top += survivors - consumed;
   if (s->top > s->peak) s->peak = s->top;
   s->st.iterations++;
@@ -969,6 +1044,7 @@
 static int restart_from_seeds(csgpu_search *s) {
   s->st.restarts++;
   s->top = 0;
+  s->staged = 0;
   const int keep_flag = s->restart_on_improvement;
   const int64_t keep = s->restart_base;
   s->restart_on_improvement = 0;
@@ -1015,6 +1091,7 @@
     }
   }
   TRY(flush_accept_results(s));
+  TRY(flush_staged(s));
   if (s->d_stream != NULL) {
     unsigned long long err = 0ull;
     HIP_OK(hipMemcpy(&err, s->d_counters + C_STREAM_ERR, sizeof err, hipMemcpyDeviceToHost));
diff --git a/csolve_amd/csrc/cs_stage_map.h b/csolve_amd/csrc/cs_stage_map.h
--- /dev/null
+++ b/csolve_amd/csrc/cs_stage_map.h
@@ -0,0 +1,44 @@
+#ifndef CS_STAGE_MAP_H
+#define CS_STAGE_MAP_H
+
+#if defined(__HIPCC__)
+#define CS_STAGE_HD __host__ __device__ __forceinline__
+#else
+#define CS_STAGE_HD static inline
+#endif
+
+typedef struct cs_stage_cursor {
+  int w;
+  unsigned lo, hi;
+} cs_stage_cursor;
+
+CS_STAGE_HD int cs_stage_region(const unsigned *prefix, int waves, unsigned f) {
+  int lo = 0, hi = waves;
+  while (hi - lo > 1) {
+    const int mid = (lo + hi) >> 1;
+    if (prefix[mid] <= f) lo = mid;
+    else hi = mid;
+  }
+  return lo;
+}
+
+CS_STAGE_HD long long cs_stage_row(const unsigned *prefix, int waves, int K, unsigned f, cs_stage_cursor *c) {
+  if (f - c->lo >= c->hi - c->lo) {
+    c->w = cs_stage_region(prefix, waves, f);
+    c->lo = prefix[c->w];
+    c->hi = prefix[c->w + 1];
+  }
+  return (long long)c->w * (long long)K + (long long)(f - c->lo);
+}
+
+CS_STAGE_HD long long cs_parent_row(long long i, long long staged, const unsigned *prefix, int waves, int K,
+                                    long long pool_top, cs_stage_cursor *c, int *in_stage) {
+  if (i < staged) {
+    *in_stage = 1;
+    return cs_stage_row(prefix, waves, K, (unsigned)(staged - 1 - i), c);
+  }
+  *in_stage = 0;
+  return pool_top - 1 - (i - staged);
+}
+
+#endif
diff --git a/csolve_amd/csrc/cs_step.hip.h b/csolve_amd/csrc/cs_step.hip.h
--- a/csolve_amd/csrc/cs_step.hip.h
+++ b/csolve_amd/csrc/cs_step.hip.h
@@ -3,6 +3,7 @@
 
 #include "cs_kernels.hip.h"
 #include "cs_shave.hip.h"
+#include "cs_stage_map.h"
 
 #define CS_STEP_QN 256
 #define CS_STEP_SHARDS 16
@@ -24,7 +25,34 @@
   long long max_solutions;
   int store_open;
   int stream_on;
+  const uint2 *prev;
+  const unsigned *prev_prefix;
+  int prev_waves, prev_K;
+  int staged;
 };
+
+template <int G>
+__device__ __forceinline__ const uint2 *cs_step_parent_rows(const cs_step_io &io, int n, int first, int end, int g, int &cw,
+                                                            unsigned &clo, unsigned &chi) {
+  const int pidx = first + g < end ? first + g : end - 1;
+  if (first >= io.staged)
+    return io.pool + (size_t)(io.first_row + (long long)io.parents - 1 - (long long)pidx) * n;
+  const int last = first + G - 1 < end ? first + G - 1 : end - 1;
+  if (last < io.staged) {
+    const unsigned f_hi = (unsigned)(io.staged - 1 - first), f_lo = (unsigned)(io.staged - 1 - last);
+    if (f_lo >= clo && f_hi < chi)
+      return io.prev + ((size_t)cw * (size_t)io.prev_K + (size_t)((unsigned)(io.staged - 1 - pidx) - clo)) * n;
+  }
+  cs_stage_cursor c;
+  c.w = cw; c.lo = clo; c.hi = chi;
+  int in_stage;
+  const long long row = cs_parent_row((long long)pidx, (long long)io.staged, io.prev_prefix, io.prev_waves, io.prev_K,
+                                      io.first_row + (long long)io.parents - (long long)io.staged, &c, &in_stage);
+  cw = __builtin_amdgcn_readlane(c.w, CS_WAVE - 1);
+  clo = (unsigned)__builtin_amdgcn_readlane((int)c.lo, CS_WAVE - 1);
+  chi = (unsigned)__builtin_amdgcn_readlane((int)c.hi, CS_WAVE - 1);
+  return (in_stage ? io.prev : io.pool) + (size_t)row * n;
+}
 
 template <int S>
 __device__ __forceinline__ unsigned cs_seg_bcast(unsigned x, int src, int lane) {
@@ -134,12 +162,10 @@
   int acc_nodes = 0, acc_skip = 0, acc_props = 0, acc_revs = 0;
   const size_t region = (size_t)wave_global * (size_t)io.K;
   uint2 pre = make_uint2(0u, 0u);
-
-  auto load_group = [&](int first, int end) -> uint2 {
-    const int pidx = first + g < end ? first + g : end - 1;
-    const long long prow = io.first_row + (long long)io.parents - 1 - (long long)pidx;
-    return io.pool[(size_t)prow * n + vcl];
-  };
+  int cw = 0;
+  unsigned clo = 0u, chi = 0u;
+
+#define CS_STEP_LOAD_GROUP(FIRST, END) (cs_step_parent_rows<G>(io, n, (FIRST), (END), g, cw, clo, chi)[vcl])
 #define CS_STEP_ASK_TICKET()                                                                                        \
   do {                                                                                                              \
     if (!exhausted && !tk_pending) {                                                                                \
@@ -168,6 +194,9 @@
     acc_fail = __builtin_amdgcn_readfirstlane(acc_fail);
     acc_sol = __builtin_amdgcn_readfirstlane(acc_sol);
     acc_parents = __builtin_amdgcn_readfirstlane(acc_parents);
+    cw = __builtin_amdgcn_readfirstlane(cw);
+    clo = (unsigned)__builtin_amdgcn_readfirstlane((int)clo);
+    chi = (unsigned)__builtin_amdgcn_readfirstlane((int)chi);
     int grp_live = 0;
     if (qlen > 0) {
       const unsigned d0 = s_q[qhead];
@@ -182,7 +211,7 @@
         if (first < (long long)io.parents) {
           c_cur = (int)first;
           c_end = first + io.chunk < (long long)io.parents ? (int)first + io.chunk : io.parents;
-          pre = load_group(c_cur, c_end);
+          pre = CS_STEP_LOAD_GROUP(c_cur, c_end);
         } else {
           exhausted = 1;
         }
@@ -193,7 +222,7 @@
         const uint2 e = pre;
         c_cur += had;
         acc_parents += had;
-        if (c_cur < c_end) pre = load_group(c_cur, c_end);
+        if (c_cur < c_end) pre = CS_STEP_LOAD_GROUP(c_cur, c_end);
         else CS_STEP_ASK_TICKET();
         int rl, rh;
         unsigned fb[2];
@@ -342,6 +371,7 @@
     st[5] = (unsigned long long)acc_parents;
   }
 #undef CS_STEP_ASK_TICKET
+#undef CS_STEP_LOAD_GROUP
 }
 
 template <int G, int NW, bool S3>
@@ -627,7 +657,8 @@
                                                   unsigned long long *__restrict__ out,
                                                   const unsigned long long *__restrict__ stored,
                                                   int32_t *__restrict__ stream, long long stream_base, long long stream_limit,
-                                                  long long stream_cap, unsigned long long *__restrict__ stream_err) {
+                                                  long long stream_cap, unsigned long long *__restrict__ stream_err,
+                                                  int copy) {
   __shared__ unsigned long long s_red[256];
   const int w = blockIdx.x, t = threadIdx.x;
   const unsigned long long drawn = chunk == 0 ? (unsigned long long)parents : (unsigned long long)*ticket * (unsigned long long)chunk;
@@ -642,7 +673,7 @@
   }
   before = s_red[0];
   __syncthreads();
-  const size_t count = (size_t)fill[w] * n;
+  const size_t count = copy ? (size_t)fill[w] * n : 0;
   const uint2 *src = stage + (size_t)w * K * n;
   uint2 *dst = pool + (size_t)(first_row + parents - consumed + (long long)before) * n;
   size_t e = t;
@@ -679,7 +710,7 @@
       }
     }
   }
-  if (w == 0) {
+  if (w == 0 && copy) {
     for (int k = 0; k < 6; k++) {
       unsigned long long x = 0ull;
       for (int i = t; i < waves; i += 256) x += k < 5 ? wstat[(size_t)i * CS_STEP_STATS + k] : (unsigned long long)fill[i];
@@ -699,4 +730,79 @@
   }
 }
 
+__global__ __launch_bounds__(1024) void cs_level_book(const unsigned *__restrict__ fill, int waves, int parents, int chunk,
+                                                      const unsigned *__restrict__ ticket,
+                                                      const unsigned long long *__restrict__ wstat,
+                                                      unsigned long long *__restrict__ out,
+                                                      const unsigned long long *__restrict__ stored,
+                                                      unsigned *__restrict__ prefix) {
+  __shared__ unsigned long long s_part[5][16];
+  __shared__ unsigned s_wsum[16];
+  const int t = threadIdx.x, lane = t & (CS_WAVE - 1), wv = t >> 6;
+  unsigned long long x[5] = { 0ull, 0ull, 0ull, 0ull, 0ull };
+  for (int i = t; i < waves; i += 1024) {
+    const unsigned long long *st = wstat + (size_t)i * CS_STEP_STATS;
+#pragma unroll
+    for (int k = 0; k < 5; k++) x[k] += st[k];
+  }
+#pragma unroll
+  for (int k = 0; k < 5; k++) {
+    for (int d = 32; d > 0; d >>= 1) x[k] += __shfl_down(x[k], d, CS_WAVE);
+    if (lane == 0) s_part[k][wv] = x[k];
+  }
+  const int per = (waves + 1023) / 1024;
+  const int w0 = t * per < waves ? t * per : waves, w1 = w0 + per < waves ? w0 + per : waves;
+  unsigned mine = 0u;
+  for (int i = w0; i < w1; i++) mine += fill[i];
+  unsigned incl = mine;
+  for (int d = 1; d < CS_WAVE; d <<= 1) {
+    const unsigned y = __shfl_up(incl, d, CS_WAVE);
+    if (lane >= d) incl += y;
+  }
+  if (lane == CS_WAVE - 1) s_wsum[wv] = incl;
+  __syncthreads();
+  unsigned base = 0u, total = 0u;
+  for (int j = 0; j < 16; j++) {
+    const unsigned ws = s_wsum[j];
+    base += j < wv ? ws : 0u;
+    total += ws;
+  }
+  unsigned at = base + incl - mine;
+  for (int i = w0; i < w1; i++) {
+    prefix[i] = at;
+    at += fill[i];
+  }
+  if (t < 5) {
+    unsigned long long sum = 0ull;
+    for (int j = 0; j < 16; j++) sum += s_part[t][j];
+    out[2 + t] = sum;
+  }
+  if (t == 0) {
+    const unsigned long long drawn = (unsigned long long)*ticket * (unsigned long long)chunk;
+    prefix[waves] = total;
+    out[0] = drawn < (unsigned long long)parents ? drawn : (unsigned long long)parents;
+    out[1] = (unsigned long long)total;
+    out[7] = *stored;
+  }
+}
+
+__global__ __launch_bounds__(256) void cs_stage_flush(const unsigned *__restrict__ prefix, const uint2 *__restrict__ stage,
+                                                      int K, int n, uint2 *__restrict__ pool, long long pool_row,
+                                                      unsigned rows) {
+  const int w = blockIdx.x, t = threadIdx.x;
+  const unsigned lo = prefix[w];
+  unsigned hi = prefix[w + 1];
+  hi = hi < rows ? hi : rows;
+  if (lo >= hi) return;
+  const size_t count = (size_t)(hi - lo) * n;
+  const uint2 *src = stage + (size_t)w * K * n;
+  uint2 *dst = pool + (size_t)(pool_row + (long long)lo) * n;
+  size_t e = t;
+  for (; e + 768 < count; e += 1024) {
+    const uint2 a = src[e], b = src[e + 256], c = src[e + 512], d = src[e + 768];
+    dst[e] = a; dst[e + 256] = b; dst[e + 512] = c; dst[e + 768] = d;
+  }
+  for (; e < count; e += 256) dst[e] = src[e];
+}
+
 #endif
diff --git a/csolve_amd/solver.py b/csolve_amd/solver.py
--- a/csolve_amd/solver.py
+++ b/csolve_amd/solver.py
@@ -1276,6 +1276,15 @@
     load_library().csgpu_set_linear_fast_paths(1 if on else 0)
 
 
+def stage_map(fill, region_rows: int, pool_top: int, first: int, count: int):
+    fill = np.ascontiguousarray(fill, dtype=np.uint32)
+    rows = np.zeros(max(1, count), dtype=np.int64)
+    in_stage = np.zeros(max(1, count), dtype=np.int32)
+    check(load_library().csgpu_internal_stage_map(fill.ctypes.data, len(fill), int(region_rows), int(pool_top), int(first),
+                                                  int(count), rows.ctypes.data, in_stage.ctypes.data))
+    return rows[:count], in_stage[:count]
+
+
 class Search:
 
     def __init__(self, model: Model, pool_capacity: int = 1 << 20, max_children: int = 1 << 16):
@@ -1332,6 +1341,14 @@
 
     def set_best(self, best: int):
         check(load_library().csgpu_search_set_best(self._h, int(best)))
+
+    DIRECT_TRACE = ("frontiers", "drew_staged", "pool_only", "left_undrawn", "rows_flushed_undrawn", "flushes_on_demand",
+                    "without_survivor", "pool_limited")
+
+    def direct_trace(self) -> dict:
+        out = np.zeros(8, dtype=np.int64)
+        check(load_library().csgpu_internal_search_direct_trace(self._h, out.ctypes.data))
+        return dict(zip(self.DIRECT_TRACE, (int(x) for x in out)))
 
     def put_cost(self):
         sec, cnt = C.c_double(), C.c_int64()
```

Result: no change. 21.28 billion (-0.4%).
